# matthiasverstraete/3d_recognizer

Measured on AMD Instinct MI355X. Metric: training clouds/sec, N=40960 pts, bs=8, at 1/2/4/8 GPUs; mIoU parity, higher is better.
Workload: dtype f32 storage/accumulate, bf16x3 MFMA in the wide GEMMs

## Files before the change

3d_recognizer_amd/csrc/gemm.hip:

```cpp
#include "rl_common.h"
#include <stdlib.h>
#include <string.h>

namespace {

typedef float f32x4 __attribute__((ext_vector_type(4)));

constexpr int GM_BM = 128;
constexpr int GM_BK = 16;
constexpr int GM_AS = 20;

struct AOperand {
    const float* A;
    long lda, a_bstride;
    int a_mode;
    RlLazy lazy;
    const float* xyz;
    long xyz_bstride;
    const int32_t* nbr_idx;
    const float* nbr_d2;
    int nbr_k;
    int n;
    int K;
    long M;
// ... 150 lines not shown
                int kk, c;
                if (p.w_ns == 1) { kk = e / BN; c = e - kk * BN; }
                else             { c = e / GM_BK; kk = e - c * GM_BK; }
                float v = 0.f;
                if (k0 + kk < K && col0 + c < N) v = p.W[(long)(k0 + kk) * p.w_ks + (long)(col0 + c) * p.w_ns];
                Ws[kk * WS + c] = v;
            }
            __syncthreads();
            const int ksteps = min(4, (K - k0 + 3) >> 2);
#pragma unroll
            for (int ks = 0; ks < 4; ++ks) {
                if (ks < ksteps) {
                    const int kc = ks * 4 + lq;
                    const float a0 = As[(wave * 32 + lr) * GM_AS + kc];
                    const float a1 = As[(wave * 32 + 16 + lr) * GM_AS + kc];
#pragma unroll
                    for (int nb = 0; nb < NT; ++nb) {
                        const float bv = Ws[kc * WS + nb * 16 + lr];
                        acc[0][nb] = __builtin_amdgcn_mfma_f32_16x16x4f32(a0, bv, acc[0][nb], 0, 0, 0);
                        acc[1][nb] = __builtin_amdgcn_mfma_f32_16x16x4f32(a1, bv, acc[1][nb], 0, 0, 0);
                    }
                }
            }
        }
#pragma unroll
        for (int rb = 0; rb < 2; ++rb) {
#pragma unroll
            for (int r = 0; r < 4; ++r) {
                const long R = row0 + wave * 32 + rb * 16 + lq * 4 + r;
                if (R < M) {
                    long yoff;
                    if (p.y_contig) yoff = R * p.ldy;
                    else {
                        const int b = (int)((unsigned)R / (unsigned)p.rows_per_batch);
                        const int i = (int)(R - (long)b * p.rows_per_batch);
                        yoff = ((long)b * p.y_bstride + i) * p.ldy;
                    }
#pragma unroll
                    for (int nb = 0; nb < NT; ++nb) {
                        const int c = col0 + nb * 16 + lr;
                        if (c < N) {
                            float v = acc[rb][nb][r];
                            if (p.bias) v += p.bias[c];
                            if (p.accumulate) v += p.Y[yoff + c];
                            p.Y[yoff + c] = v;
                            const float dv = v - piv[nb];
                            ssum[nb] += dv;
                            ssq[nb] += dv * dv;
                        }
                    }
                }
            }
        }
    }
    if (p.stats) {
#pragma unroll
        for (int nb = 0; nb < NT; ++nb) {
            float s = ssum[nb], q = ssq[nb];
            s += __shfl_xor(s, 16, 64); s += __shfl_xor(s, 32, 64);
            q += __shfl_xor(q, 16, 64); q += __shfl_xor(q, 32, 64);
            if (lane < 16) {
                red[wave][0][nb * 16 + lane] = (double)s;
                red[wave][1][nb * 16 + lane] = (double)q;
            }
        }
        __syncthreads();
        if (tid < BN && col0 + tid < N) {
            const double s = red[0][0][tid] + red[1][0][tid] + red[2][0][tid] + red[3][0][tid];
            const double q = red[0][1][tid] + red[1][1][tid] + red[2][1][tid] + red[3][1][tid];
            p.stats[((long)blockIdx.x * 2 + 0) * N + col0 + tid] = s;
            p.stats[((long)blockIdx.x * 2 + 1) * N + col0 + tid] = q;
            for (long slot = blockIdx.x + gridDim.x; slot < p.stat_slots; slot += gridDim.x) {
                p.stats[(slot * 2 + 0) * N + col0 + tid] = 0.0;
                p.stats[(slot * 2 + 1) * N + col0 + tid] = 0.0;
            }
        }
    }
}

constexpr int WG_RB = 32;
constexpr int WG_T = 64;
constexpr int WG_S = 80;

struct WgradParams {
    AOperand a;
    int N;
    const float* dY;
    long lddy, dy_bstride;
    int rows_per_batch;
    int dy_contig;
    float* slab;
    long rows_per_block;
    int has_bias;
};

__global__ __launch_bounds__(256) void wgrad_kernel(const WgradParams p) {
    __shared__ __attribute__((aligned(16))) float dYs[WG_RB * WG_S];
    __shared__ __attribute__((aligned(16))) float As[WG_RB * WG_S];
    const int tid = threadIdx.x, lane = tid & 63, wave = __builtin_amdgcn_readfirstlane(tid >> 6);
    const int lr = lane & 15, lq = lane >> 4;
    const int N = p.N, K = p.a.K;
    const int n0 = blockIdx.y * WG_T, k0 = blockIdx.z * WG_T;
    const int nvalid = min(WG_T, N - n0), kvalid = min(WG_T, K - k0);
    const int nkb = (kvalid + 15) >> 4;
    const bool wave_active = wave * 16 < nvalid;
    const long r_begin = (long)blockIdx.x * p.rows_per_block;
    const long r_end = min(p.a.M, r_begin + p.rows_per_block);

    f32x4 acc[4];
#pragma unroll
    for (int kb = 0; kb < 4; ++kb) acc[kb] = (f32x4){0.f, 0.f, 0.f, 0.f};
    float bsum = 0.f;

    for (long r0 = r_begin; r0 < r_end; r0 += WG_RB) {
        __syncthreads();
        for (int e = tid; e < WG_RB * WG_T; e += 256) {
            const int r = e >> 6, c = e & 63;
            const long R = r0 + r;
            float v = 0.f;
            if (R < r_end && c < nvalid) {
                long off;
                if (p.dy_contig) off = R * p.lddy;
                else {
                    const int b = (int)((unsigned)R / (unsigned)p.rows_per_batch);
                    const int i = (int)(R - (long)b * p.rows_per_batch);
                    off = ((long)b * p.dy_bstride + i) * p.lddy;
                }
                v = p.dY[off + n0 + c];
            }
            dYs[r * WG_S + c] = v;
        }
        stage_a(p.a, r0, WG_RB, r_end, k0, nkb * 16, As, WG_S);
        __syncthreads();
        if (p.has_bias && blockIdx.z == 0 && tid < WG_T) {
#pragma unroll 8
            for (int r = 0; r < WG_RB; ++r) bsum += dYs[r * WG_S + tid];
        }
        if (wave_active) {
#pragma unroll
            for (int rs = 0; rs < WG_RB / 4; ++rs) {
                const int rr = rs * 4 + lq;
                const float av = dYs[rr * WG_S + wave * 16 + lr];
#pragma unroll
                for (int kb = 0; kb < 4; ++kb) {
                    if (kb < nkb) {
                        const float bv = As[rr * WG_S + kb * 16 + lr];
                        acc[kb] = __builtin_amdgcn_mfma_f32_16x16x4f32(av, bv, acc[kb], 0, 0, 0);
                    }
                }
            }
        }
    }
    float* out = p.slab + (long)blockIdx.x * ((long)N * K + N);
    if (wave_active) {
#pragma unroll
        for (int kb = 0; kb < 4; ++kb) {
            if (kb < nkb) {
                const int k = k0 + kb * 16 + lr;
#pragma unroll
                for (int r = 0; r < 4; ++r) {
                    const int n = n0 + wave * 16 + lq * 4 + r;
                    if (n < N && k < K) out[(long)n * K + k] = acc[kb][r];
                }
            }
        }
    }
    if (p.has_bias && blockIdx.z == 0 && tid < nvalid) out[(long)N * K + n0 + tid] = bsum;
}
// ... 1829 lines not shown
                v.w = actf(v.w * sc[i].w + sh[i].w);
            }
            float* dd = dYt + ucol[i] * PW2_S + urow[i];
            dd[0] = rd[i].x; dd[PW2_S] = rd[i].y; dd[2 * PW2_S] = rd[i].z; dd[3 * PW2_S] = rd[i].w;
            float* da = At + ucol[i] * PW2_S + urow[i];
            da[0] = v.x; da[PW2_S] = v.y; da[2 * PW2_S] = v.z; da[3 * PW2_S] = v.w;
        }
    };

    const float* n_frag = dYt + (wave * 32 + lr) * PW2_S + lq * 8;
    const float* k_frag = At + lr * PW2_S + lq * 8;
    if (r_begin < r_end) fetch(r_begin);
    for (long r0 = r_begin; r0 < r_end; r0 += PW2_RB) {
        __syncthreads();
        commit(r0);
        __syncthreads();
        if (r0 + PW2_RB < r_end) fetch(r0 + PW2_RB);
        if (p.has_bias && blockIdx.z == 0 && tid < PW2_T) {
#pragma unroll
            for (int j = 0; j < PW2_RB / 4; ++j) {
                const float4 t = *reinterpret_cast<const float4*>(dYt + tid * PW2_S + j * 4);
                bsum += (t.x + t.y) + (t.z + t.w);
            }
        }
        float4 af[2][2], bf[2][2];
#pragma unroll
        for (int h = 0; h < 2; ++h) {
            af[h][0] = *reinterpret_cast<const float4*>(n_frag + h * 4);
            af[h][1] = *reinterpret_cast<const float4*>(n_frag + 16 * PW2_S + h * 4);
        }
#pragma unroll
        for (int j = 0; j < 2; ++j) bf[0][j] = *reinterpret_cast<const float4*>(k_frag + j * 16 * PW2_S);
#pragma unroll
        for (int g = 0; g < 8; ++g) {
            const int h = g / 4, kb0 = (g % 4) * 2;
            if (g + 1 < 8) {
                const int h1 = (g + 1) / 4, kb1 = ((g + 1) % 4) * 2;
#pragma unroll
                for (int j = 0; j < 2; ++j)
                    bf[(g + 1) & 1][j] = *reinterpret_cast<const float4*>(k_frag + (kb1 + j) * 16 * PW2_S + h1 * 4);
            }
            __builtin_amdgcn_sched_barrier(0);
            const float a0[4] = {af[h][0].x, af[h][0].y, af[h][0].z, af[h][0].w};
            const float a1[4] = {af[h][1].x, af[h][1].y, af[h][1].z, af[h][1].w};
#pragma unroll
            for (int s2 = 0; s2 < 4; ++s2) {
#pragma unroll
                for (int j = 0; j < 2; ++j) {
                    const float4 b4 = bf[g & 1][j];
                    const float bv = s2 == 0 ? b4.x : s2 == 1 ? b4.y : s2 == 2 ? b4.z : b4.w;
                    acc[0][kb0 + j] = __builtin_amdgcn_mfma_f32_16x16x4f32(a0[s2], bv, acc[0][kb0 + j], 0, 0, 0);
                    acc[1][kb0 + j] = __builtin_amdgcn_mfma_f32_16x16x4f32(a1[s2], bv, acc[1][kb0 + j], 0, 0, 0);
                }
            }
        }
    }
    float* out = p.slab + (long)blockIdx.x * ((long)N * K + N);
#pragma unroll
    for (int i = 0; i < 2; ++i) {
#pragma unroll
        for (int kb = 0; kb < 8; ++kb) {
            const int k = k0 + kb * 16 + lr;
#pragma unroll
            for (int r = 0; r < 4; ++r) {
                const int n = n0 + (2 * wave + i) * 16 + lq * 4 + r;
                if (n < N && k < K) out[(long)n * K + k] = acc[i][kb][r];
            }
        }
    }
    if (p.has_bias && blockIdx.z == 0 && tid < nvalid) out[(long)N * K + n0 + tid] = bsum;
}

typedef __attribute__((ext_vector_type(4))) short s16x4g;
template <int TERMS, bool RB = false>
__device__ __forceinline__ void pwgrad128w_body(const WgradParams& p, const int bx, const int by, const int bz) {
    constexpr int RP = 144;
    constexpr int NSPL = TERMS == 3 ? 2 : 1;
    __shared__ __attribute__((aligned(16))) __bf16 lds_d[PW2_RB * RP * NSPL];
    __shared__ __attribute__((aligned(16))) __bf16 lds_a[PW2_RB * RP * NSPL];
    __bf16* Dh = lds_d;
    __bf16* Dl = Dh + PW2_RB * RP;
    __bf16* Xh = lds_a;
    __bf16* Xl = Xh + PW2_RB * RP;
    __shared__ __attribute__((aligned(16))) float lz[2][PW2_T];
    const int tid = threadIdx.x, lane = tid & 63, wave = tid >> 6;
    const int lr = lane & 15, lq = lane >> 4;
    const int N = p.N, K = p.a.K;
    const int n0 = by * PW2_T, k0 = bz * PW2_T;
    const int nvalid = min(PW2_T, N - n0), kvalid = min(PW2_T, K - k0);
    const long r_begin = (long)bx * p.rows_per_block;
    const long r_end = min(p.a.M, r_begin + p.rows_per_block);
    const bool lazy = p.a.lazy.scale != nullptr;
    const bool relu = p.a.lazy.act == RL_ACT_RELU;
    const float nslope = p.a.lazy.act == RL_ACT_NONE ? 1.f : p.a.lazy.slope;
    auto actf = [&](float z) {
        const float neg = relu ? 0.f : z * nslope;
        return z > 0.f ? z : neg;
    };
    int ucol[2], urow[2];
#pragma unroll
    for (int i = 0; i < 2; ++i) {
        const int u = i * 8 + wave;
        ucol[i] = (u & 7) * 16 + (lane & 3) * 4;
        urow[i] = (u >> 3) * 16 + (lane >> 2);
    }
    if (tid < PW2_T) {
        const bool in = lazy && tid < kvalid;
        lz[0][tid] = in ? p.a.lazy.scale[k0 + tid] : 1.f;
        lz[1][tid] = in ? p.a.lazy.shift[k0 + tid] : 0.f;
    }
    const int nh = wave >> 2, kw = wave & 3;
    f32x4 acc[4][2];
#pragma unroll
    for (int nb = 0; nb < 4; ++nb)
#pragma unroll
        for (int kb = 0; kb < 2; ++kb) acc[nb][kb] = (f32x4){0.f, 0.f, 0.f, 0.f};
    const bool want_bias = p.has_bias && bz == 0;
    f32x4 bs = {0.f, 0.f, 0.f, 0.f};
    float4 rd[2], ra[2];

    auto fetch = [&](long r0) {
#pragma unroll
        for (int i = 0; i < 2; ++i) {
            const long R = r0 + urow[i];
            rd[i] = make_float4(0.f, 0.f, 0.f, 0.f);
            ra[i] = make_float4(0.f, 0.f, 0.f, 0.f);
            if (R < r_end) {
                if (ucol[i] < nvalid) {
                    long off;
                    if (p.dy_contig) off = R * p.lddy;
                    else {
                        const int b = (int)((unsigned)R / (unsigned)p.rows_per_batch);
                        const int ii = (int)(R - (long)b * p.rows_per_batch);
                        off = ((long)b * p.dy_bstride + ii) * p.lddy;
                    }
                    rd[i] = rl_ldx4<RB>(p.dY, off + n0 + ucol[i]);
                }
                if (ucol[i] < kvalid) ra[i] = rl_ldx4<RB>(p.a.A, a_row_offset(p.a, R) + k0 + ucol[i]);
            }
        }
    };
    auto commit = [&](long r0) {
#pragma unroll
        for (int i = 0; i < 2; ++i) {
            float4 v = ra[i];
            if (lazy && r0 + urow[i] < r_end && ucol[i] < kvalid) {
                const float4 sc = *reinterpret_cast<const float4*>(&lz[0][ucol[i]]);
                const float4 sh = *reinterpret_cast<const float4*>(&lz[1][ucol[i]]);
                v.x = actf(v.x * sc.x + sh.x);
                v.y = actf(v.y * sc.y + sh.y);
                v.z = actf(v.z * sc.z + sh.z);
                v.w = actf(v.w * sc.w + sh.w);
            }
            bf16x4 dh, dl, xh, xl;
            if (want_bias) bs += (f32x4){rd[i].x, rd[i].y, rd[i].z, rd[i].w};
            split_bf16(rd[i], dh, dl);
            split_bf16(v, xh, xl);
            const int o = urow[i] * RP + ucol[i];
            *reinterpret_cast<bf16x4*>(Dh + o) = dh;
            *reinterpret_cast<bf16x4*>(Xh + o) = xh;
            if constexpr (TERMS == 3) {
                *reinterpret_cast<bf16x4*>(Dl + o) = dl;
                *reinterpret_cast<bf16x4*>(Xl + o) = xl;
            }
        }
    };

    const int tr_off = (lq * 8 + (lr >> 2)) * RP + 4 * (lr & 3);
    const __bf16* dh_frag = Dh + tr_off + nh * 64;
    const __bf16* xh_frag = Xh + tr_off + kw * 32;
    constexpr int LO = PW2_RB * RP;
    auto frag = [&](const __bf16* q) {
        const bf16x4 r0 = __builtin_bit_cast(bf16x4, __builtin_amdgcn_ds_read_tr16_b64_v4i16((__attribute__((address_space(3))) s16x4g*)q));
        const bf16x4 r1 = __builtin_bit_cast(bf16x4, __builtin_amdgcn_ds_read_tr16_b64_v4i16((__attribute__((address_space(3))) s16x4g*)(q + 4 * RP)));
        return __builtin_shufflevector(r0, r1, 0, 1, 2, 3, 4, 5, 6, 7);
    };
    if (r_begin < r_end) fetch(r_begin);
    for (long r0 = r_begin; r0 < r_end; r0 += PW2_RB) {
        __syncthreads();
        commit(r0);
        __syncthreads();
        if (r0 + PW2_RB < r_end) fetch(r0 + PW2_RB);
        bf16x8 b_h[2], b_l[2];
#pragma unroll
        for (int kb = 0; kb < 2; ++kb) {
            b_h[kb] = frag(xh_frag + kb * 16);
            if constexpr (TERMS == 3) b_l[kb] = frag(xh_frag + LO + kb * 16);
        }
#pragma unroll
        for (int nb = 0; nb < 4; ++nb) {
            bf16x8 a_h, a_l;
            a_h = frag(dh_frag + nb * 16);
            if constexpr (TERMS == 3) a_l = frag(dh_frag + LO + nb * 16);
#pragma unroll
            for (int kb = 0; kb < 2; ++kb)
                acc[nb][kb] = __builtin_amdgcn_mfma_f32_16x16x32_bf16(a_h, b_h[kb], acc[nb][kb], 0, 0, 0);
            if constexpr (TERMS == 3) {
#pragma unroll
                for (int kb = 0; kb < 2; ++kb)
                    acc[nb][kb] = __builtin_amdgcn_mfma_f32_16x16x32_bf16(a_h, b_l[kb], acc[nb][kb], 0, 0, 0);
#pragma unroll
                for (int kb = 0; kb < 2; ++kb)
                    acc[nb][kb] = __builtin_amdgcn_mfma_f32_16x16x32_bf16(a_l, b_h[kb], acc[nb][kb], 0, 0, 0);
            }
        }
    }
    float* out = p.slab + (long)bx * ((long)N * K + N);
#pragma unroll
    for (int nb = 0; nb < 4; ++nb) {
#pragma unroll
        for (int kb = 0; kb < 2; ++kb) {
            const int k = k0 + kw * 32 + kb * 16 + lr;
#pragma unroll
            for (int r = 0; r < 4; ++r) {
                const int n = n0 + nh * 64 + nb * 16 + lq * 4 + r;
                if (n < N && k < K) out[(long)n * K + k] = acc[nb][kb][r];
            }
        }
    }
    if (want_bias) {
#pragma unroll
        for (int o = 4; o < 64; o <<= 1)
#pragma unroll
            for (int j = 0; j < 4; ++j) bs[j] += __shfl_xor(bs[j], o, 64);
        if (lane < 4 && ucol[0] < nvalid) {
#pragma unroll
            for (int j = 0; j < 4; ++j) out[(long)N * K + n0 + ucol[0] + j] = bs[j];
        }
    }
}

template <int TERMS, bool RB = false>
__global__ __launch_bounds__(512, 4) void pwgrad128w_kernel(const WgradParams p) {
    pwgrad128w_body<TERMS, RB>(p, blockIdx.x, blockIdx.y, blockIdx.z);
}

struct WBItem {
    const float* A; const float* dY; const float* sc; const float* sh; float* slab;
    long lda, a_bstride, lddy, dy_bstride, rows_per_block, M;
    int N, K, n, rows_per_batch, act;
    float slope;
    int first_block;
    int nsplit;
    unsigned short gy, gz;
    unsigned char a_contig, dy_contig, has_bias, pad;
};
constexpr int WB_MAX = 24;
struct WgradBatch {
    WBItem item[WB_MAX];
    int count, pad;
};
template <int TERMS>
__global__ __launch_bounds__(512, 4) void pwgrad128w_batch_kernel(const WgradBatch b) {
    int i = 0;
    while (i + 1 < b.count && (int)blockIdx.x >= b.item[i + 1].first_block) ++i;
    const WBItem& it = b.item[i];
    const int local = (int)blockIdx.x - it.first_block;
    const int per = (int)it.gy * (int)it.gz;
    int bx, t = 0;
    if (per > 1) {
        const int grp = local / (8 * per), rem = local - grp * 8 * per;
        t = rem >> 3;
        bx = grp * 8 + (rem & 7);
    } else bx = local;
    if (bx >= it.nsplit) return;
    const int by = t / (int)it.gz, bz = t - by * (int)it.gz;
    WgradParams p;
    p.a.A = it.A; p.a.lda = it.lda; p.a.a_bstride = it.a_bstride; p.a.a_mode = 0;
    p.a.lazy.scale = it.sc; p.a.lazy.shift = it.sh; p.a.lazy.act = it.act; p.a.lazy.slope = it.slope;
    p.a.xyz = nullptr; p.a.xyz_bstride = 0; p.a.nbr_idx = nullptr; p.a.nbr_d2 = nullptr; p.a.nbr_k = 0;
    p.a.n = it.n; p.a.K = it.K; p.a.M = it.M; p.a.contig = it.a_contig; p.a.vec4 = 1; p.a.vec4p = 1;
    p.N = it.N; p.dY = it.dY; p.lddy = it.lddy; p.dy_bstride = it.dy_bstride; p.rows_per_batch = it.rows_per_batch;
    p.dy_contig = it.dy_contig; p.slab = it.slab; p.rows_per_block = it.rows_per_block; p.has_bias = it.has_bias;
    pwgrad128w_body<TERMS, false>(p, bx, by, bz);
}

__global__ __launch_bounds__(256) void swgrad_batch_kernel(const WgradBatch b) {
    __shared__ float red[4 * 4 * 4 * 64 + 8 * 64];
    int i = 0;
    while (i + 1 < b.count && (int)blockIdx.x >= b.item[i + 1].first_block) ++i;
    const WBItem& it = b.item[i];
    WgradParams p;
    p.a.A = it.A; p.a.lda = it.lda; p.a.a_bstride = it.a_bstride; p.a.a_mode = 0;
    p.a.lazy.scale = it.sc; p.a.lazy.shift = it.sh; p.a.lazy.act = it.act; p.a.lazy.slope = it.slope;
    p.a.xyz = nullptr; p.a.xyz_bstride = 0; p.a.nbr_idx = nullptr; p.a.nbr_d2 = nullptr; p.a.nbr_k = 0;
    p.a.n = it.n; p.a.K = it.K; p.a.M = it.M; p.a.contig = it.a_contig; p.a.vec4 = 0; p.a.vec4p = 0;
    p.N = it.N; p.dY = it.dY; p.lddy = it.lddy; p.dy_bstride = it.dy_bstride; p.rows_per_batch = it.rows_per_batch;
    p.dy_contig = it.dy_contig; p.slab = it.slab; p.rows_per_block = it.rows_per_block; p.has_bias = it.has_bias;
    const int bx = (int)blockIdx.x - it.first_block;
    if (bx >= it.nsplit) return;
    switch (it.gy) {
        case swgrad_body_index(1, 1): swgrad_body<1, 1>(p, bx, red); break;
        case swgrad_body_index(1, 2): swgrad_body<1, 2>(p, bx, red); break;
        case swgrad_body_index(1, 4): swgrad_body<1, 4>(p, bx, red); break;
        case swgrad_body_index(1, 8): swgrad_body<1, 8>(p, bx, red); break;
        case swgrad_body_index(2, 1): swgrad_body<2, 1>(p, bx, red); break;
        case swgrad_body_index(2, 2): swgrad_body<2, 2>(p, bx, red); break;
        case swgrad_body_index(2, 4): swgrad_body<2, 4>(p, bx, red); break;
        case swgrad_body_index(4, 1): swgrad_body<4, 1>(p, bx, red); break;
        case swgrad_body_index(4, 2): swgrad_body<4, 2>(p, bx, red); break;
        default: swgrad_body<4, 4>(p, bx, red); break;
    }
}

inline bool pwgrad_ok(const WgradParams& p) {
    if (p.a.a_mode != 0 || !p.a.vec4) return false;
    if ((p.N % 4) || (p.lddy % 4) || (((uintptr_t)p.dY) & 15)) return false;
    if (p.a.lazy.scale && ((((uintptr_t)p.a.lazy.scale) | ((uintptr_t)p.a.lazy.shift)) & 15)) return false;
    return true;
}


typedef void (*GemmFn)(const GemmParams);
typedef void (*WgradFn)(const WgradParams);
enum GemmKernel { GK_NONE, GK_SGEMM, GK_PGEMM, GK_WGEMM, GK_WGEMM2, GK_GEMM };

struct GemmFacts {
    long M; int N, K;
    bool streamable;
    bool pgemm, wgemm, wgemm2;
    bool split, stats, bnb;
    int64_t kslab_floats;
};

struct GemmPlan {
    GemmKernel kernel;
    GemmFn fn;
    int threads; dim3 grid;
    WidePlan wide;
    int gx, ny, ksplit, kchunk;
    GemmFn reduce;
    dim3 reduce_grid;
    const char* name;
    const char* refusal;
};

template <int KC, bool BNB>
GemmFn sgemm_fn(int N) {
    if constexpr (KC == 1 && !BNB) if (N > 64) return sgemm_kernel<1, 8>;
    return N <= 16 ? sgemm_kernel<KC, 1, BNB> : N <= 32 ? sgemm_kernel<KC, 2, BNB> : sgemm_kernel<KC, 4, BNB>;
}
template <int NT>
GemmFn pgemm_fn(int terms) { return terms == 0 ? pgemm_kernel<NT, 0> : terms == 1 ? pgemm_kernel<NT, 1> : pgemm_kernel<NT, 3>; }
template <int TERMS, bool STATS>
GemmFn wide_inst(bool dma, WidePlan w) {
    if (!dma) return wgemm_kernel<TERMS, STATS>;
    return w.bm == 128 ? wgemm2_kernel<TERMS, STATS, W2_AS, W2_WS, 128, 128>
         : w.bn == 128 ? wgemm2_kernel<TERMS, STATS, W2_AS, W2_WS, 64, 128> : wgemm2_kernel<TERMS, STATS, W2_AS, W2_WS, 64, 64>;
}
inline GemmFn wide_fn(bool stats, bool dma, WidePlan w) {
    if (wide_gemm_terms() == 1) return stats ? wide_inst<1, true>(dma, w) : wide_inst<1, false>(dma, w);
    return stats ? wide_inst<3, true>(dma, w) : wide_inst<3, false>(dma, w);
}

inline dim3 xcd_grid(int gx, int ny, int z) { return dim3(ny > 1 ? (unsigned)(8 * rl_cdiv(gx, 8) * ny) : (unsigned)gx, 1, z); }

inline void persistent_grid(GemmPlan& pl, long M, int ny, int z) {
    int cap = cu_count() / ny / 8 * 8;
    if (cap < 8) cap = 8;
    pl.gx = rl_cdiv(M, pl.wide.bm);
    if (pl.gx > cap) pl.gx = cap;
    pl.ny = ny;
    pl.grid = xcd_grid(pl.gx, ny, z);
}

inline void plan_wide(GemmPlan& pl, const GemmFacts& f, int z, bool splitk) {
    const bool dma = f.wgemm2;
    pl.fn = wide_fn(f.stats && pl.ksplit <= 1, dma, pl.wide);
    pl.kernel = dma ? GK_WGEMM2 : GK_WGEMM;
    pl.threads = dma ? W2_THREADS : 512;
    if (dma) persistent_grid(pl, f.M, rl_cdiv(f.N, pl.wide.bn), z);
// ... 12 lines not shown
    const bool streams = !f.split && f.streamable && stream_ok(N, K);
    if (!f.split && f.bnb && !(streams && N <= 64)) {
        pl.refusal = "rl_gemm: the BatchNorm-backward sums are a by-product of the streaming kernel only (K, N <= 64; ask rl_gemm_streams)";
        return pl;
    }
    if (streams) {
        int sg = pl.gx;
        if ((long)K * N >= 2048) sg = sg > 512 ? 512 : (sg > 256 ? 256 : sg);
        if (g_sgemm_grid_div > 1) sg = sg / g_sgemm_grid_div > 0 ? sg / g_sgemm_grid_div : 1;
        if (f.bnb) pl.fn = K <= 16 ? sgemm_fn<1, true>(N) : K <= 32 ? sgemm_fn<2, true>(N) : sgemm_fn<4, true>(N);
        else       pl.fn = K <= 16 ? sgemm_fn<1, false>(N) : K <= 32 ? sgemm_fn<2, false>(N) : sgemm_fn<4, false>(N);
        pl.kernel = GK_SGEMM;
        pl.grid = dim3(sg);
        pl.name = "sgemm_kernel";
        return pl;
    }
    if (f.pgemm) pl.wide = wide_plan(f.M, N, K, N > 64 && f.wgemm && f.wgemm2);
    const int terms = wide_gemm_terms();
    if (!f.split && f.pgemm && N > 64 && pl.wide.ksplit > 1 && f.kslab_floats >= (int64_t)pl.wide.ksplit * f.M * N) {
        pl.kchunk = ((K + pl.wide.ksplit - 1) / pl.wide.ksplit + 31) / 32 * 32;
        pl.ksplit = (K + pl.kchunk - 1) / pl.kchunk;
        const bool cb64 = (long)pl.gx * rl_cdiv(N, 64) >= 256;
        pl.reduce = cb64 ? gemm_splitk_reduce_kernel<64> : gemm_splitk_reduce_kernel<16>;
        pl.reduce_grid = dim3(pl.gx, rl_cdiv(N, cb64 ? 64 : 16));
        if (f.wgemm) {
            plan_wide(pl, f, pl.ksplit, true);
        } else {
            pl.kernel = GK_PGEMM;
            pl.fn = pgemm_fn<8>(terms);
            pl.grid = xcd_grid(pl.gx, pl.ny, pl.ksplit);
            pl.name = "pgemm_kernel<8>+splitk";
        }
    } else if (!f.split && f.pgemm && N > 16 && N <= 64 && wgemm_small_tiles() && f.wgemm && f.wgemm2) {
        pl.wide = WidePlan{64, 64, 1};
        plan_wide(pl, f, 1, false);
    } else if (!f.pgemm) {
        pl.kernel = GK_GEMM;
        pl.fn = nt == 1 ? gemm_kernel<1> : nt == 2 ? gemm_kernel<2> : nt == 4 ? gemm_kernel<4> : gemm_kernel<8>;
        pl.grid = dim3(pl.gx, pl.ny);
        pl.name = "gemm_kernel";
    } else if (N > 64 && f.wgemm) {
        plan_wide(pl, f, 1, false);
    } else {
        pl.kernel = GK_PGEMM;
        pl.fn = nt == 1 ? pgemm_fn<1>(terms) : nt == 2 ? pgemm_fn<2>(terms) : nt == 4 ? pgemm_fn<4>(terms) : pgemm_fn<8>(terms);
        pl.grid = xcd_grid(pl.gx, pl.ny, 1);
        pl.name = N > 64 ? "pgemm_kernel<8>" : f.split ? "pgemm_kernel" : nt == 1 ? "pgemm_kernel<1>" : nt == 2 ? "pgemm_kernel<2>" : "pgemm_kernel<4>";
    }
    return pl;
}

inline GemmFacts aligned_facts(long M, int N, int K, bool dma) {
    return GemmFacts{M, N, K, true, true, wide_gemm_terms() != 0 && K % 8 == 0,
                     dma && wgemm_staging() == 1 && K % PG_BK == 0 && K <= W2_KMAX, false, true, false, 0};
}

int launch_gemm(const GemmPlan& pl, hipStream_t st, GemmParams p, const char* who) {
    p.gx = pl.gx; p.ny = pl.ny; p.ksplit = pl.ksplit; p.kchunk = pl.kchunk;
    hipLaunchKernelGGL(pl.fn, pl.grid, dim3(pl.threads), 0, st, p);
    rl_note_kernel(pl.name);
    RL_LAUNCH_CHECK(who);
    if (!pl.reduce) return RL_OK;
    hipLaunchKernelGGL(pl.reduce, pl.reduce_grid, dim3(256), 0, st, p);
    RL_LAUNCH_CHECK("rl_gemm(split-K reduce)");
    return RL_OK;
}

struct WgradPlan {
    WgradFn fn;
    int threads; dim3 grid;
    int nsplit; long rows_per_block;
    int batch;
    int body;
    const char* name;
    const char* refusal;
};

template <int KT>
WgradFn swgrad_fn(int N) {
    if constexpr (KT == 1) if (N > 64) return swgrad_kernel<1, 8>;
    return N <= 16 ? swgrad_kernel<KT, 1> : N <= 32 ? swgrad_kernel<KT, 2> : swgrad_kernel<KT, 4>;
}

WgradPlan plan_wgrad(long M, int N, int K, int a_mode, bool pwgrad, bool rows_bf16) {
    WgradPlan pl{};
    pl.threads = 256;
    const int terms = wide_gemm_terms();
    if (stream_ok(N, K)) {
        swgrad_split(M, &pl.nsplit, &pl.rows_per_block);
        if (!rows_bf16) pl.fn = K <= 16 ? swgrad_fn<1>(N) : K <= 32 ? swgrad_fn<2>(N) : swgrad_fn<4>(N);
        pl.refusal = "rl_wgrad: bf16 rows are supported by the wide weight-gradient kernel only";
        pl.grid = dim3(pl.nsplit);
        pl.batch = a_mode == 0 && !rows_bf16 ? 2 : 0;
        pl.body = swgrad_body_index(K <= 16 ? 1 : K <= 32 ? 2 : 4, N <= 16 ? 1 : N <= 32 ? 2 : N <= 64 ? 4 : 8);
        pl.name = "swgrad_kernel";
        return pl;
    }
    wgrad_split(M, N, K, &pl.nsplit, &pl.rows_per_block);
    const int T = pwgrad ? wgrad_tile(N, K) : WG_T;
    const bool wide = pwgrad && T == 128;
    pl.grid = dim3(pl.nsplit, rl_cdiv(N, T), rl_cdiv(K, T));
    if (rows_bf16)  pl.fn = wide && terms != 0 ? pwgrad128w_kernel<1, true> : nullptr;
    else if (wide)  pl.fn = terms == 0 ? pwgrad128_kernel : terms == 1 ? pwgrad128w_kernel<1> : pwgrad128w_kernel<3>;
    else            pl.fn = pwgrad ? pwgrad_kernel : wgrad_kernel;
    pl.threads = wide && terms != 0 ? 512 : 256;
    pl.refusal = "rl_wgrad: bf16 rows are supported by the wide (128 x 128 tile) weight-gradient kernel only";
    pl.batch = !rows_bf16 && wide && terms != 0 && rl_cdiv(N, 128) < 65536 && rl_cdiv(K, 128) < 65536 ? 1 : 0;
    pl.name = wide ? (terms != 0 ? "pwgrad128w_kernel" : "pwgrad128_kernel") : pwgrad ? "pwgrad_kernel" : "wgrad_kernel";
    return pl;
}

void launch_wgrad_batch(int batch, long blocks, hipStream_t st, const WgradBatch& b) {
    if (batch == 2)                   hipLaunchKernelGGL(swgrad_batch_kernel, dim3((unsigned)blocks), dim3(256), 0, st, b);
    else if (wide_gemm_terms() == 1)  hipLaunchKernelGGL(pwgrad128w_batch_kernel<1>, dim3((unsigned)blocks), dim3(512), 0, st, b);
    else                              hipLaunchKernelGGL(pwgrad128w_batch_kernel<3>, dim3((unsigned)blocks), dim3(512), 0, st, b);
}

}

int rl_wide_terms() { return wide_gemm_terms(); }

extern "C" int rl_set_wide_gemm(const char* mode) {
    const int t = parse_wide(mode);
    RL_REQUIRE(mode != nullptr && t >= 0, RL_ERR_ARGS, "rl_set_wide_gemm: mode must be \"fp32\", \"bf16x3\" or \"bf16\"");
    g_wide_terms = t;
    return RL_OK;
}
extern "C" int rl_set_wgemm_staging(const char* how) {
    RL_REQUIRE(how != nullptr && (!strcmp(how, "registers") || !strcmp(how, "dma")), RL_ERR_ARGS,
               "rl_set_wgemm_staging: \"registers\" or \"dma\"");
    g_wgemm_staging = !strcmp(how, "dma");
    return RL_OK;
}
extern "C" int rl_set_wgemm_tile(const char* how) {
    RL_REQUIRE(how && (!strcmp(how, "auto") || !strcmp(how, "128") || !strcmp(how, "64x128") || !strcmp(how, "64x64")), RL_ERR_ARGS,
               "rl_set_wgemm_tile: expected auto | 128 | 64x128 | 64x64");
    g_wgemm_force = !strcmp(how, "64x128") ? 1 : !strcmp(how, "64x64") ? 2 : 0;
    g_wgemm_small = strcmp(how, "128") ? 1 : 0;
    return RL_OK;
}
extern "C" int rl_set_gemm_ksplit(int enable) {
    g_gemm_no_ksplit = enable ? 0 : 1;
    return RL_OK;
}
extern "C" int rl_set_sgemm_grid_div(int div) {
    RL_REQUIRE(div >= 1 && div <= 64, RL_ERR_ARGS, "rl_set_sgemm_grid_div: 1 .. 64");
    g_sgemm_grid_div = div;
    return RL_OK;
}
extern "C" const char* rl_get_wide_gemm(void) {
    const int t = wide_gemm_terms();
    return t == 0 ? "fp32" : t == 1 ? "bf16" : "bf16x3";
}

extern "C" int rl_gemm(const rl_gemm_desc* d, void* stream) {
    RL_REQUIRE(d != nullptr, RL_ERR_ARGS, "rl_gemm: null descriptor");
    GemmParams p{};
    int rc = fill_a(&p.a, "rl_gemm", d->A, d->lda, d->a_bstride, d->a_mode, d->in_act, d->in_slope,
                    d->in_scale, d->in_shift, d->xyz, d->xyz_bstride, d->nbr_idx, d->nbr_d2, d->nbr_k,
                    d->B, d->n, d->K);
    if (rc) return rc;
    RL_REQUIRE(d->N > 0 && d->W && d->Y && d->ldy > 0, RL_ERR_ARGS, "rl_gemm: bad W/Y");
    p.N = d->N; p.W = d->W; p.w_ks = d->w_ks; p.w_ns = d->w_ns; p.bias = d->bias;
    p.Y = d->Y; p.ldy = d->ldy; p.y_bstride = d->y_bstride;
    p.rows_per_batch = (d->a_mode == 1) ? d->n * d->nbr_k : d->n;
    RL_REQUIRE(d->y_bstride >= p.rows_per_batch, RL_ERR_ARGS, "rl_gemm: y_bstride smaller than rows per cloud");
    p.y_contig = (d->y_bstride == p.rows_per_batch);
// ... 39 lines not shown
static bool gemm_pair_fits(const rl_gemm_desc* a, const rl_gemm_desc* b) {
    if (!a || !b) return false;
    if (a->A != b->A || a->lda != b->lda || a->a_bstride != b->a_bstride || a->a_mode != 0 || b->a_mode != 0) return false;
    if (a->B != b->B || a->n != b->n || a->K != b->K) return false;
    if (a->in_scale != b->in_scale || a->in_shift != b->in_shift || a->in_act != b->in_act || a->in_slope != b->in_slope) return false;
    if (!a->W_split || !b->W_split || wide_gemm_terms() == 0 || wgemm_staging() != 1) return false;
    if (a->K % PG_BK || a->K > W2_KMAX || a->N <= 0 || b->N <= 0) return false;
    if ((a->K <= 64 && a->N <= 64) || (b->K <= 64 && b->N <= 64)) return false;
    if (a->bias || b->bias || a->accumulate || b->accumulate || a->addend || b->addend || a->out2 || b->out2) return false;
    if ((a->stats == nullptr) != (b->stats == nullptr)) return false;
    if (a->ldy != a->N || b->ldy != b->N || a->y_bstride != a->n || b->y_bstride != b->n || !a->Y || !b->Y) return false;
    if ((((uintptr_t)a->A | (uintptr_t)(a->lda * 4) | (uintptr_t)a->W_split | (uintptr_t)b->W_split | (uintptr_t)a->Y | (uintptr_t)b->Y) & 15) != 0)
        return false;
    if (a->N % 4 || b->N % 4) return false;
    return true;
}
extern "C" int rl_gemm_pair_supported(const rl_gemm_desc* a, const rl_gemm_desc* b) { return gemm_pair_fits(a, b) ? 1 : 0; }
extern "C" int rl_gemm_pair(const rl_gemm_desc* a, const rl_gemm_desc* b, void* stream) {
    RL_REQUIRE(gemm_pair_fits(a, b), RL_ERR_UNSUPPORTED,
               "rl_gemm_pair: needs one plain A' (K %% 32 == 0, K <= 1024) for both, pre-split weights in a bf16 arithmetic mode, the "
               "dense outputs, statistics for both or none, no bias / accumulate / split epilogue");
    GemmParams p{};
    int rc = fill_a(&p.a, "rl_gemm_pair", a->A, a->lda, a->a_bstride, 0, a->in_act, a->in_slope, a->in_scale, a->in_shift,
                    nullptr, 0, nullptr, nullptr, 0, a->B, a->n, a->K);
    if (rc) return rc;
    p.N = a->N; p.W = a->W; p.w_ks = a->w_ks; p.w_ns = a->w_ns; p.bias = nullptr;
    p.Y = a->Y; p.ldy = a->ldy; p.y_bstride = a->y_bstride; p.rows_per_batch = a->n; p.y_contig = 1;
    p.accumulate = 0; p.stats = a->stats;
    p.piv_mean = a->stats ? a->stats_pivot_mean : nullptr; p.piv_bias = a->stats ? a->stats_pivot_bias : nullptr;
    p.split_col = a->N; p.wsplit = reinterpret_cast<const __bf16*>(a->W_split);
    p.stat_slots = rl_row_blocks_host(p.a.M, GM_BM);
    p.N2 = b->N; p.Y2 = b->Y; p.stats2 = b->stats; p.wsplit2 = reinterpret_cast<const __bf16*>(b->W_split);
    p.piv_mean2 = b->stats ? b->stats_pivot_mean : nullptr; p.piv_bias2 = b->stats ? b->stats_pivot_bias : nullptr;
    p.pair_ny1 = rl_cdiv(a->N, 128);
    RL_REQUIRE(wgemm2_usable(p), RL_ERR_UNSUPPORTED, "rl_gemm_pair: the LDS-DMA kernel does not take this operand");
    GemmPlan pl{};
    pl.kernel = GK_WGEMM2; pl.wide = WidePlan{128, 128, 1}; pl.threads = W2_THREADS; pl.ksplit = 1; pl.name = "wgemm2_kernel";
    pl.fn = wide_fn(p.stats != nullptr, true, pl.wide);
    persistent_grid(pl, p.a.M, p.pair_ny1 + rl_cdiv(b->N, 128), 1);
    return launch_gemm(pl, (hipStream_t)stream, p, "rl_gemm_pair");
}

extern "C" int rl_split_weights(const rl_wsplit_item* items, int count, void* stream) {
    RL_REQUIRE(items != nullptr && count >= 0, RL_ERR_ARGS, "rl_split_weights: bad arguments");
    hipStream_t st = (hipStream_t)stream;
    for (int base = 0; base < count; base += WS_MAX) {
        SplitBatch b;
        b.count = count - base < WS_MAX ? count - base : WS_MAX;
        long blocks = 0;
        for (int i = 0; i < b.count; ++i) {
            const rl_wsplit_item& it = items[base + i];
            RL_REQUIRE(it.W && it.out && it.K > 0 && it.N > 0, RL_ERR_ARGS, "rl_split_weights: bad item %d", base + i);
            RL_REQUIRE(((uintptr_t)it.out & 15) == 0, RL_ERR_ARGS, "rl_split_weights: item %d: out must be 16-byte aligned", base + i);
            RL_REQUIRE(it.K % 8 == 0 && (long)it.N * it.K < (1l << 31), RL_ERR_ARGS, "rl_split_weights: item %d: K %% 8 == 0, N * K < 2^31", base + i);
            b.item[i] = it;
            b.first_block[i] = (int)blocks;
            blocks += rl_cdiv((long)it.N * (it.K / 8), 256);
        }
        b.first_block[b.count] = (int)blocks;
        if (blocks > 0) hipLaunchKernelGGL(split_weights_kernel, dim3((unsigned)blocks), dim3(256), 0, st, b);
        RL_LAUNCH_CHECK("rl_split_weights");
    }
    rl_note_kernel("split_weights_kernel");
    return RL_OK;
}

extern "C" int64_t rl_gemm_stat_slots(int64_t M, int N, int K) {
    const GemmPlan pl = plan_gemm(aligned_facts(M, N, K, true));
    return rl_row_blocks_host(M, pl.kernel == GK_WGEMM2 ? pl.wide.bm : GM_BM);
}

extern "C" int64_t rl_gemm_kslab_floats(int64_t M, int N, int K) {
    const int ks = plan_gemm(aligned_facts(M, N, K, false)).wide.ksplit;
    return ks > 1 ? (int64_t)ks * M * N : 0;
}

extern "C" int64_t rl_wgrad_slab_floats(int64_t M, int N, int K) {
    return (int64_t)plan_wgrad(M, N, K, 0, true, false).nsplit * ((int64_t)N * K + N);
}

static int wgrad_fill(const rl_wgrad_desc* d, WgradParams* pp, WgradPlan* plan) {
    RL_REQUIRE(d != nullptr, RL_ERR_ARGS, "rl_wgrad: null descriptor");
    WgradParams& p = *pp;
    int rc = fill_a(&p.a, "rl_wgrad", d->A, d->lda, d->a_bstride, d->a_mode, d->in_act, d->in_slope,
                    d->in_scale, d->in_shift, d->xyz, d->xyz_bstride, d->nbr_idx, d->nbr_d2, d->nbr_k,
                    d->B, d->n, d->K);
    if (rc) return rc;
    RL_REQUIRE(d->N > 0 && d->dY && d->dW && d->slab && d->lddy >= d->N, RL_ERR_ARGS, "rl_wgrad: bad dY/dW/slab");
    p.N = d->N; p.dY = d->dY; p.lddy = d->lddy; p.dy_bstride = d->dy_bstride;
    p.rows_per_batch = (d->a_mode == 1) ? d->n * d->nbr_k : d->n;
    RL_REQUIRE(d->dy_bstride >= p.rows_per_batch, RL_ERR_ARGS, "rl_wgrad: dy_bstride smaller than rows per cloud");
    p.dy_contig = (d->dy_bstride == p.rows_per_batch);
    p.slab = d->slab; p.has_bias = d->dbias != nullptr;
    const WgradPlan pl = plan_wgrad(p.a.M, d->N, d->K, d->a_mode, pwgrad_ok(p), d->rows_bf16 != 0);
    RL_REQUIRE(pl.fn != nullptr, RL_ERR_UNSUPPORTED, "%s", pl.refusal);
    RL_REQUIRE(d->slab_floats >= (int64_t)pl.nsplit * ((int64_t)d->N * d->K + d->N), RL_ERR_ARGS,
               "rl_wgrad: slab too small (%ld floats)", (long)d->slab_floats);
    RL_REQUIRE(!d->rows_bf16 || (d->lda % 4 == 0 && d->lddy % 4 == 0), RL_ERR_ARGS,
               "rl_wgrad: bf16 rows need leading dimensions that are multiples of 4");
    p.rows_per_block = pl.rows_per_block;
    *plan = pl;
    return RL_OK;
}

extern "C" int rl_wgrad_batchable(const rl_wgrad_desc* d) {
    WgradParams p;
    WgradPlan pl;
    return wgrad_fill(d, &p, &pl) == RL_OK ? pl.batch : 0;
}

extern "C" int rl_wgrad_batch(const rl_wgrad_desc* descs, int count, void* stream) {
    RL_REQUIRE(descs != nullptr && count >= 0, RL_ERR_ARGS, "rl_wgrad_batch: bad arguments");
    hipStream_t st = (hipStream_t)stream;
    bool any[3] = {false, false, false};
    for (int kind = 1; kind <= 2; ++kind) {
        WgradBatch b;
        b.count = 0; b.pad = 0;
        long blocks = 0;
        auto flush = [&]() -> int {
            if (b.count == 0 || blocks == 0) { b.count = 0; blocks = 0; return RL_OK; }
            launch_wgrad_batch(kind, blocks, st, b);
            RL_LAUNCH_CHECK("rl_wgrad_batch");
            b.count = 0; blocks = 0;
            return RL_OK;
        };
        for (int i = 0; i < count; ++i) {
            const rl_wgrad_desc* d = descs + i;
            WgradParams p;
            WgradPlan pl;
            int rc = wgrad_fill(d, &p, &pl);
            if (rc) return rc;
            RL_REQUIRE(pl.batch != 0, RL_ERR_UNSUPPORTED,
                       "rl_wgrad_batch: layer %d (N = %d, K = %d) cannot join a grouped launch - check rl_wgrad_batchable first", i, d->N, d->K);
            RL_REQUIRE(d->defer_reduce, RL_ERR_ARGS, "rl_wgrad_batch: the layers' slabs are summed by rl_wgrad_reduce_batch (defer_reduce must be set)");
            if (pl.batch != kind) continue;
            any[kind] = true;
            WBItem& it = b.item[b.count];
            it.A = p.a.A; it.dY = p.dY; it.sc = p.a.lazy.scale; it.sh = p.a.lazy.shift; it.slab = p.slab;
            it.lda = p.a.lda; it.a_bstride = p.a.a_bstride; it.lddy = p.lddy; it.dy_bstride = p.dy_bstride;
            it.rows_per_block = p.rows_per_block; it.M = p.a.M;
            it.N = p.N; it.K = p.a.K; it.n = p.a.n; it.rows_per_batch = p.rows_per_batch; it.act = p.a.lazy.act; it.slope = p.a.lazy.slope;
            it.nsplit = pl.nsplit;
            if (kind == 2) {
                it.gy = (unsigned short)pl.body; it.gz = 1;
                it.first_block = (int)blocks;
                blocks += pl.nsplit;
            } else {
                it.gy = (unsigned short)pl.grid.y; it.gz = (unsigned short)pl.grid.z;
                const int per = (int)it.gy * (int)it.gz;
                if (per > 1) blocks = (blocks + 7) / 8 * 8;
                it.first_block = (int)blocks;
                blocks += per > 1 ? (long)((pl.nsplit + 7) / 8 * 8) * per : (long)pl.nsplit;
            }
            it.a_contig = (unsigned char)p.a.contig; it.dy_contig = (unsigned char)p.dy_contig; it.has_bias = (unsigned char)p.has_bias; it.pad = 0;
            RL_REQUIRE(blocks < (1l << 30), RL_ERR_ARGS, "rl_wgrad_batch: too many workgroups");
            if (++b.count == WB_MAX) {
                rc = flush();
                if (rc) return rc;
            }
        }
        const int rc = flush();
        if (rc) return rc;
    }
    rl_note_kernel(any[2] && !any[1] ? "swgrad_batch_kernel" : "pwgrad128w_batch_kernel");
    return RL_OK;
}

extern "C" int rl_wgrad(const rl_wgrad_desc* d, void* stream) {
    WgradParams p;
    WgradPlan pl;
    int rc = wgrad_fill(d, &p, &pl);
    if (rc) return rc;
    hipStream_t st = (hipStream_t)stream;
    hipLaunchKernelGGL(pl.fn, pl.grid, dim3(pl.threads), 0, st, p);
    rl_note_kernel(pl.name);
    RL_LAUNCH_CHECK("rl_wgrad");
    if (d->defer_reduce) return RL_OK;
    const long per = (long)d->N * d->K + d->N;
    hipLaunchKernelGGL(wgrad_reduce_kernel, dim3(rl_cdiv(per, WR_E)), dim3(256), 0, st, d->slab, pl.nsplit,
                       d->N, d->K, d->dW, (long)d->w_ks, (long)d->w_ns, d->dbias);
    RL_LAUNCH_CHECK("rl_wgrad_reduce");
    return RL_OK;
}

extern "C" int rl_wgrad_nsplit(int64_t M, int N, int K) { return plan_wgrad(M, N, K, 0, true, false).nsplit; }

extern "C" int rl_wgrad_reduce_batch(const rl_wgrad_reduce_item* items, int count, void* stream) {
    RL_REQUIRE(items != nullptr && count >= 0, RL_ERR_ARGS, "rl_wgrad_reduce_batch: bad arguments");
    hipStream_t st = (hipStream_t)stream;
    for (int base = 0; base < count; base += RB_MAX) {
        ReduceBatch b;
        b.count = count - base < RB_MAX ? count - base : RB_MAX;
        long tiles = 0;
        for (int i = 0; i < b.count; ++i) {
            const rl_wgrad_reduce_item& it = items[base + i];
            RL_REQUIRE(it.slab && it.dW && it.nsplit > 0 && it.N > 0 && it.K > 0, RL_ERR_ARGS,
                       "rl_wgrad_reduce_batch: bad item %d", base + i);
            b.item[i] = it;
            b.first_tile[i] = (int)tiles;
            tiles += rl_cdiv((long)it.N * it.K + it.N, WR_E);
            RL_REQUIRE(tiles < (1l << 30), RL_ERR_ARGS, "rl_wgrad_reduce_batch: too many tiles");
        }
        b.first_tile[b.count] = (int)tiles;
        hipLaunchKernelGGL(wgrad_reduce_batch_kernel, dim3((unsigned)tiles), dim3(256), 0, st, b);
        RL_LAUNCH_CHECK("rl_wgrad_reduce_batch");
    }
    rl_note_kernel("wgrad_reduce_batch_kernel");
    return RL_OK;
}
```

3d_recognizer_amd/csrc/pool.hip:

```cpp
#include "rl_common.h"
#include <stdlib.h>

namespace {

#ifdef RL_POOL_PLAIN_STORES
#define RL_ST1 rl_stx
#define RL_ST4 rl_stx4
#else
#define RL_ST1 rl_stx_nt
#define RL_ST4 rl_stx4_nt
#endif

typedef float f32x4 __attribute__((ext_vector_type(4)));
typedef __attribute__((ext_vector_type(4))) __bf16 bf16x4;
typedef __attribute__((ext_vector_type(8))) __bf16 bf16x8;
typedef __attribute__((ext_vector_type(4))) short s16x4;

typedef float f32x2 __attribute__((ext_vector_type(2)));
typedef __attribute__((ext_vector_type(2))) __bf16 bf16x2;
__device__ __forceinline__ void split2(const f32x2 x, unsigned& hi, unsigned& lo) {
    const unsigned hb = __builtin_bit_cast(unsigned, __builtin_convertvector(x, bf16x2));
    const f32x2 hf = {__uint_as_float(hb << 16), __uint_as_float(hb & 0xffff0000u)};
    const f32x2 l = x - hf;
    lo = __builtin_bit_cast(unsigned, __builtin_convertvector(l, bf16x2));
    hi = hb;
}
__device__ __forceinline__ void split4(const float4 v, bf16x4& hi, bf16x4& lo) {
    unsigned h0, h1, l0, l1;
    split2((f32x2){v.x, v.y}, h0, l0);
    split2((f32x2){v.z, v.w}, h1, l1);
    typedef unsigned u2 __attribute__((ext_vector_type(2)));
    hi = __builtin_bit_cast(bf16x4, (u2){h0, h1});
    lo = __builtin_bit_cast(bf16x4, (u2){l0, l1});
}
__device__ __forceinline__ bf16x8 cat8(const bf16x4 a, const bf16x4 b) {
    bf16x8 r;
#pragma unroll
    for (int i = 0; i < 4; ++i) { r[i] = a[i]; r[4 + i] = b[i]; }
    return r;
}
__device__ __forceinline__ f32x4 mfma16(const bf16x4 a, const bf16x4 b, const f32x4 c) {
    return __builtin_amdgcn_mfma_f32_16x16x16bf16_1k(__builtin_bit_cast(s16x4, a), __builtin_bit_cast(s16x4, b), c, 0, 0, 0);
}

__device__ __forceinline__ void loads_issued() { __builtin_amdgcn_sched_barrier(0); }
__device__ __forceinline__ void loads_landed() {
    asm volatile("" ::: "memory");
    __builtin_amdgcn_s_waitcnt(0x0F70);
    asm volatile("" ::: "memory");
}
__device__ __forceinline__ f32x4 splat(float v) { return (f32x4){v, v, v, v}; }
__device__ __forceinline__ f32x4 v4(const float4 a) { return (f32x4){a.x, a.y, a.z, a.w}; }
__device__ __forceinline__ float4 f4(const f32x4 a) { return make_float4(a[0], a[1], a[2], a[3]); }
__device__ __forceinline__ float sum4(const f32x4 a) { return (a[0] + a[1]) + (a[2] + a[3]); }
__device__ __forceinline__ f32x4 vbn(const f32x4 raw, float s, float h) { return __builtin_elementwise_fma(raw, splat(s), splat(h)); }
__device__ __forceinline__ f32x4 vrelu(const f32x4 z) { return __builtin_elementwise_max(z, splat(0.f)); }
__device__ __forceinline__ float eff_slope(const RlLazy& t) {
    if (t.scale == nullptr || t.act == RL_ACT_NONE) return 1.f;
    return t.act == RL_ACT_RELU ? 0.f : t.slope;
}
__device__ __forceinline__ f32x4 vact(const f32x4 z, float e) { return __builtin_elementwise_max(z, z * splat(e)); }

struct PoolParams {
    const float* U;
    RlLazy ulazy;
    const float* G;
    long g_bstride;
    RlLazy glazy;
    const int32_t* idx;
    const float* W;
    long P;
    int n;
    int d;
    float* Pout;
    const float* dP;
    float* GU;
    int gu_accumulate;
    float* DG;
    float* slab;
    long slab_stride;
    float* X_out;
    float* dS_out;
    int src;
    const float* xyz;
    long xyz_bstride;
    int xyz_w;
    const float* nbr_d2;
    const float* W1; const float* b1; const float* sc1; const float* sh1;
    const float* W2; const float* b2; const float* sc2; const float* sh2;
    const float* mu1; const float* is1; const float* mu2; const float* is2;
    const float* piv1; const float* piv2;
    double* fstats2;
    double* bstats;
    int xcd_chunk;
};

template <int DT>
struct Tile {
    static constexpr int D = 16 * DT;
    static constexpr int H = D / 2;
    static constexpr int XS = D + 4;
    static constexpr int XSB = D + 8;
};

template <int DT>
__device__ __forceinline__ void lane_lazy(const PoolParams& p, int lj, f32x4 (&sc)[DT], f32x4 (&sh)[DT]) {
    constexpr int H = Tile<DT>::H;
#pragma unroll
    for (int c = 0; c < DT; ++c)
#pragma unroll
        for (int s = 0; s < 4; ++s) {
            const int k = 16 * c + 4 * lj + s;
            if (k < H) {
                sc[c][s] = p.ulazy.scale ? p.ulazy.scale[k] : 1.f;
                sh[c][s] = p.ulazy.scale ? p.ulazy.shift[k] : 0.f;
            } else {
                sc[c][s] = p.glazy.scale ? p.glazy.scale[k - H] : 1.f;
                sh[c][s] = p.glazy.scale ? p.glazy.shift[k - H] : 0.f;
            }
        }
}
template <int DT>
__device__ __forceinline__ float chunk_slope(int c, int lj, float es_u, float es_g) {
    if constexpr (DT == 1) return lj < 2 ? es_u : es_g;
    else return 16 * c < Tile<DT>::H ? es_u : es_g;
}

template <int DT>
struct LFold {
    static constexpr int D = 16 * DT;
    static constexpr bool INLDS = DT >= 8;
    static constexpr int LDS_FLOATS = INLDS ? 2 * D : 4;
    f32x4 rsc[INLDS ? 1 : DT], rsh[INLDS ? 1 : DT];
    const float* lds;
    __device__ __forceinline__ void init(const PoolParams& p, int lj, float* mem) {
        if constexpr (INLDS) {
            constexpr int H = D / 2;
            for (int k = threadIdx.x; k < D; k += blockDim.x) {
                const RlLazy& t = k < H ? p.ulazy : p.glazy;
                mem[k] = t.scale ? t.scale[k < H ? k : k - H] : 1.f;
                mem[D + k] = t.scale ? t.shift[k < H ? k : k - H] : 0.f;
            }
            lds = mem + 4 * lj;
        } else lane_lazy<DT>(p, lj, rsc, rsh);
    }
    __device__ __forceinline__ f32x4 sc(int c) const {
        if constexpr (INLDS) return *reinterpret_cast<const f32x4*>(lds + 16 * c);
        else return rsc[c];
    }
    __device__ __forceinline__ f32x4 sh(int c) const {
        if constexpr (INLDS) return *reinterpret_cast<const f32x4*>(lds + D + 16 * c);
        else return rsh[c];
    }
};

struct Cursor {
    long pt;
    int b, i;
    __device__ __forceinline__ void start(long pt0, int n) {
        pt = pt0;
        b = (int)((unsigned)pt0 / (unsigned)n);
        i = (int)(pt0 - (long)b * n);
    }
    __device__ __forceinline__ Cursor next(long pstep, int n) const {
        Cursor c;
        c.pt = pt + pstep;
        c.b = b;
        c.i = i + (int)pstep;
        while (c.i >= n) { c.i -= n; ++c.b; }
        return c;
    }
};

struct PointSpan { int first, step, end; };
template <int NW>
__device__ __forceinline__ PointSpan point_span(const PoolParams& p, int wave) {
    PointSpan s;
    if (p.xcd_chunk > 0) {
        const int x = (int)blockIdx.x & 7, slot = (int)blockIdx.x >> 3;
        const int lo = x * p.xcd_chunk, hi = lo + p.xcd_chunk;
        s.end = hi < (int)p.P ? hi : (int)p.P;
        s.first = lo + slot * NW + wave;
        s.step = ((int)gridDim.x >> 3) * NW;
    } else {
        s.end = (int)p.P;
        s.first = (int)blockIdx.x * NW + wave;
        s.step = (int)gridDim.x * NW;
    }
    return s;
}

template <int DT>
__device__ __forceinline__ void fetch_x(const PoolParams& p, const Cursor& cu, int li, int lj, int my_idx, float4 (&raw)[DT]) {
    constexpr int H = Tile<DT>::H;
    const long row = cu.pt * 16 + li;
    const long b = cu.b;
#pragma unroll
    for (int c = 0; c < DT; ++c) {
        const int k = 16 * c + 4 * lj;
        if (k < H) {
            if (p.src == 0) raw[c] = *reinterpret_cast<const float4*>(p.U + row * H + k);
        } else raw[c] = *reinterpret_cast<const float4*>(p.G + (b * p.g_bstride + my_idx) * H + (k - H));
    }
}
template <int DT>
__device__ __forceinline__ void finish_x(const PoolParams& p, int li, int lj, const float4 (&raw)[DT],
                                         const LFold<DT>& lf, float4 (&xa)[DT], float* Xs) {
    constexpr int XS = Tile<DT>::XS;
    const float es_u = eff_slope(p.ulazy), es_g = eff_slope(p.glazy);
#pragma unroll
    for (int c = 0; c < DT; ++c) {
        const int k = 16 * c + 4 * lj;
        const float4 v = f4(vact(v4(raw[c]) * lf.sc(c) + lf.sh(c), chunk_slope<DT>(c, lj, es_u, es_g)));
        xa[c] = v;
        *reinterpret_cast<float4*>(Xs + li * XS + k) = v;
    }
}

template <int DT>
__device__ __forceinline__ void tile_gemm(const float4 (&a)[DT], const float* Bt, int li, int lj, f32x4 (&acc)[DT]) {
    constexpr int XS = Tile<DT>::XS;
    const float* base = Bt + li * XS + 4 * lj;
#pragma unroll
    for (int c = 0; c < DT; ++c) {
        float4 b[DT];
#pragma unroll
        for (int nb = 0; nb < DT; ++nb) b[nb] = *reinterpret_cast<const float4*>(base + nb * 16 * XS + 16 * c);
        const float av[4] = {a[c].x, a[c].y, a[c].z, a[c].w};
#pragma unroll
        for (int s = 0; s < 4; ++s) {
#pragma unroll
            for (int nb = 0; nb < DT; ++nb) {
                const float bv = s == 0 ? b[nb].x : s == 1 ? b[nb].y : s == 2 ? b[nb].z : b[nb].w;
                acc[nb] = __builtin_amdgcn_mfma_f32_16x16x4f32(av[s], bv, acc[nb], 0, 0, 0);
            }
        }
    }
}

template <int DT>
__device__ __forceinline__ void tile_gemm_bf(const float4 (&a)[DT], const __bf16* Bh, const __bf16* Bl, int li, int lj,
                                             f32x4 (&acc)[DT]) {
    constexpr int XSB = Tile<DT>::XSB;
    const int off = li * XSB + 4 * lj;
    if constexpr (DT == 1) {
        bf16x4 ah, al;
        split4(a[0], ah, al);
        const bf16x4 bh = *reinterpret_cast<const bf16x4*>(Bh + off);
        const bf16x4 bl = *reinterpret_cast<const bf16x4*>(Bl + off);
        acc[0] = mfma16(ah, bh, acc[0]);
        acc[0] = mfma16(ah, bl, acc[0]);
        acc[0] = mfma16(al, bh, acc[0]);
    } else {
#pragma unroll
        for (int b = 0; b < DT / 2; ++b) {
            bf16x4 h0, l0, h1, l1;
            split4(a[2 * b], h0, l0);
            split4(a[2 * b + 1], h1, l1);
            const bf16x8 ah = cat8(h0, h1), al = cat8(l0, l1);
            constexpr int NG = DT < 4 ? DT : 4;
#pragma unroll
            for (int n0 = 0; n0 < DT; n0 += NG) {
                bf16x8 bh[NG], bl[NG];
#pragma unroll
                for (int j = 0; j < NG; ++j) {
                    const int o = off + (n0 + j) * 16 * XSB + 32 * b;
                    bh[j] = cat8(*reinterpret_cast<const bf16x4*>(Bh + o), *reinterpret_cast<const bf16x4*>(Bh + o + 16));
                    bl[j] = cat8(*reinterpret_cast<const bf16x4*>(Bl + o), *reinterpret_cast<const bf16x4*>(Bl + o + 16));
                }
#pragma unroll
                for (int j = 0; j < NG; ++j) acc[n0 + j] = __builtin_amdgcn_mfma_f32_16x16x32_bf16(ah, bh[j], acc[n0 + j], 0, 0, 0);
#pragma unroll
                for (int j = 0; j < NG; ++j) acc[n0 + j] = __builtin_amdgcn_mfma_f32_16x16x32_bf16(ah, bl[j], acc[n0 + j], 0, 0, 0);
#pragma unroll
                for (int j = 0; j < NG; ++j) acc[n0 + j] = __builtin_amdgcn_mfma_f32_16x16x32_bf16(al, bh[j], acc[n0 + j], 0, 0, 0);
            }
        }
    }
}


typedef unsigned u32x2 __attribute__((ext_vector_type(2)));
__device__ __forceinline__ float vsqrt(float x) { return __builtin_amdgcn_sqrtf(x); }

__device__ __forceinline__ float lg_sum(float v) {
    u32x2 r = __builtin_amdgcn_permlane16_swap(__float_as_uint(v), __float_as_uint(v), false, false);
    v = __uint_as_float(r[0]) + __uint_as_float(r[1]);
    r = __builtin_amdgcn_permlane32_swap(__float_as_uint(v), __float_as_uint(v), false, false);
    return __uint_as_float(r[0]) + __uint_as_float(r[1]);
}
__device__ __forceinline__ void lg_sum2(float& a, float& b) {
    u32x2 r = __builtin_amdgcn_permlane32_swap(__float_as_uint(a), __float_as_uint(b), false, false);
    float z = __uint_as_float(r[0]) + __uint_as_float(r[1]);
    r = __builtin_amdgcn_permlane16_swap(__float_as_uint(z), __float_as_uint(z), false, false);
    z = __uint_as_float(r[0]) + __uint_as_float(r[1]);
    r = __builtin_amdgcn_permlane32_swap(__float_as_uint(z), __float_as_uint(z), false, false);
// ... 230 lines not shown
                v.x = Xs[(4 * lj + 0) * XS + kb * 16 + li]; v.y = Xs[(4 * lj + 1) * XS + kb * 16 + li];
                v.z = Xs[(4 * lj + 2) * XS + kb * 16 + li]; v.w = Xs[(4 * lj + 3) * XS + kb * 16 + li];
                split4(v, xh[kb], xl[kb]);
            }
#pragma unroll
            for (int nb = 0; nb < DT; ++nb) {
                bf16x4 dh, dl;
                split4(f4(dsr[nb]), dh, dl);
#pragma unroll
                for (int kb = 0; kb < DT; ++kb) accw[nb][kb] = mfma16(dh, xh[kb], accw[nb][kb]);
#pragma unroll
                for (int kb = 0; kb < DT; ++kb) accw[nb][kb] = mfma16(dh, xl[kb], accw[nb][kb]);
#pragma unroll
                for (int kb = 0; kb < DT; ++kb) accw[nb][kb] = mfma16(dl, xh[kb], accw[nb][kb]);
            }
        }
        loads_landed();
#pragma unroll
        for (int r = 0; r < 4; ++r) {
            const int rowi = lj * 4 + r;
#pragma unroll
            for (int nb = 0; nb < DT; ++nb) {
                const int col = nb * 16 + li;
                float v = dx[nb][r];
                if (col < H) {
                    if (nb < NGU) v += gacc[nb][r];
                }
                if constexpr (DT <= 2) Ds[rowi * XS + col] = v;
                else {
                    const long urow = (pt * 16 + rowi) * H;
                    if (col < H) RL_ST1<GUB>(p.GU, urow + col, v);
                    else RL_ST1<GB>(p.DG, urow + (col - H), v);
                }
            }
        }
        if constexpr (DT <= 2) {
            __builtin_amdgcn_wave_barrier();
            const long orow = (pt * 16 + li) * H;
#pragma unroll
            for (int c = 0; c < DT; ++c) {
                const int k = 16 * c + 4 * lj;
                const float4 v = *reinterpret_cast<const float4*>(Ds + li * XS + k);
                if (k < H) RL_ST4<GUB>(p.GU, orow + k, v);
                else RL_ST4<GB>(p.DG, orow + (k - H), v);
            }
        }
#pragma unroll
        for (int nb = 0; nb < DT; ++nb) gp[nb] = gp_nxt[nb];
        __builtin_amdgcn_wave_barrier();
    }
    __syncthreads();
    float* red = Wmem;
    for (int w = 1; w < NW; ++w) {
        __syncthreads();
        if (wave == w) {
#pragma unroll
            for (int nb = 0; nb < DT; ++nb)
#pragma unroll
                for (int kb = 0; kb < DT; ++kb)
#pragma unroll
                    for (int r = 0; r < 4; ++r) red[((nb * DT + kb) * 4 + r) * 64 + lane] = accw[nb][kb][r];
        }
        __syncthreads();
        if (wave == 0) {
#pragma unroll
            for (int nb = 0; nb < DT; ++nb)
#pragma unroll
                for (int kb = 0; kb < DT; ++kb)
#pragma unroll
                    for (int r = 0; r < 4; ++r) accw[nb][kb][r] += red[((nb * DT + kb) * 4 + r) * 64 + lane];
        }
    }
    if (wave == 0) {
        float* out = p.slab + (long)blockIdx.x * p.slab_stride;
#pragma unroll
        for (int nb = 0; nb < DT; ++nb)
#pragma unroll
            for (int kb = 0; kb < DT; ++kb)
#pragma unroll
                for (int r = 0; r < 4; ++r) out[(long)(nb * 16 + lj * 4 + r) * D + kb * 16 + li] = accw[nb][kb][r];
    }
}

template <bool GB>
__global__ __launch_bounds__(512) void pool128_bwd_kernel(const PoolParams p) {
    __shared__ __attribute__((aligned(16))) float lfm[LFold<8>::LDS_FLOATS];
    constexpr int NW = 8;
    constexpr int TERMS = 3;
    constexpr int DT = 8, D = 128, H = 64, XS = Tile<DT>::XS, XSB = Tile<DT>::XSB;
    __shared__ __attribute__((aligned(16))) __bf16 Wh[D * XSB];
    __shared__ __attribute__((aligned(16))) __bf16 Wl[D * XSB];
    __shared__ __attribute__((aligned(16))) float Tiles[NW][16 * XS];
    const int lane = threadIdx.x & 63, wave = __builtin_amdgcn_readfirstlane(threadIdx.x >> 6);
    const int li = lane & 15, lj = lane >> 4;
    for (int e = threadIdx.x; e < D * D; e += 64 * NW) {
        const int o = e / D, i = e - o * D;
        const float w = p.W[e];
        const __bf16 h = (__bf16)w;
        Wh[o * XSB + i] = h;
        if constexpr (TERMS == 3) Wl[o * XSB + i] = (__bf16)(w - (float)h);
    }
    LFold<DT> lf;
    lf.init(p, lj, lfm);
    __syncthreads();
    float* Xs = Tiles[wave];
    float* Ds = Tiles[wave];

    const PointSpan span = point_span<NW>(p, wave);
    const long pstep = span.step, Pend = span.end;
    long pt = span.first;
    int idx_cur = pt < Pend ? p.idx[pt * 16 + li] : 0;
    int idx_nxt = pt + pstep < Pend ? p.idx[(pt + pstep) * 16 + li] : 0;
    float4 raw[DT];
    Cursor cu;
    cu.start(pt, p.n);
    float gp[DT], gp_nxt[DT];
#pragma unroll
    for (int nb = 0; nb < DT; ++nb) gp[nb] = gp_nxt[nb] = 0.f;
    if (pt < Pend) {
        fetch_x<DT>(p, cu, li, lj, idx_cur, raw);
#pragma unroll
        for (int nb = 0; nb < DT; ++nb) gp[nb] = p.dP[pt * D + nb * 16 + li];
    }
    loads_landed();
    for (; pt < Pend; pt += pstep) {
        const Cursor cn = cu.next(pstep, p.n);
        float4 xa[DT];
        finish_x<DT>(p, li, lj, raw, lf, xa, Xs);
        const int idx_n2 = pt + 2 * pstep < Pend ? p.idx[(pt + 2 * pstep) * 16 + li] : 0;
        const Cursor cf = pt + pstep < Pend ? cn : cu;
        fetch_x<DT>(p, cf, li, lj, pt + pstep < Pend ? idx_nxt : idx_cur, raw);
#pragma unroll
        for (int nb = 0; nb < DT; ++nb) gp_nxt[nb] = p.dP[cf.pt * D + nb * 16 + li];
        loads_issued();
        cu = cn;
        idx_cur = idx_nxt; idx_nxt = idx_n2;
#pragma unroll
        for (int c = 0; c < DT; ++c) rl_stx4<GB>(p.X_out, (pt * 16 + li) * D + 16 * c + 4 * lj, xa[c]);
        f32x4 a[DT];
#pragma unroll
        for (int nb = 0; nb < DT; ++nb) a[nb] = (f32x4){0.f, 0.f, 0.f, 0.f};
        tile_gemm_bf<DT>(xa, Wh, Wl, li, lj, a);
        softmax_rows<DT>(a);
        __builtin_amdgcn_wave_barrier();
        f32x4 dx[DT];
#pragma unroll
        for (int nb = 0; nb < DT; ++nb) {
            const int col = nb * 16 + li;
            f32x4 xc;
#pragma unroll
            for (int r = 0; r < 4; ++r) xc[r] = Xs[(lj * 4 + r) * XS + col];
            float pool = sum4(a[nb] * xc);
            pool = lg_sum(pool);
            dx[nb] = a[nb] * splat(gp[nb]);
            const f32x4 ds = dx[nb] * (xc - splat(pool));
#pragma unroll
            for (int r = 0; r < 4; ++r) Ds[(lj * 4 + r) * XS + col] = ds[r];
        }
        __builtin_amdgcn_wave_barrier();
#pragma unroll
        for (int c = 0; c < DT; ++c) {
            const float4 da = *reinterpret_cast<const float4*>(Ds + li * XS + 16 * c + 4 * lj);
            rl_stx4<GB>(p.dS_out, (pt * 16 + li) * D + 16 * c + 4 * lj, da);
            bf16x4 ah, al;
            split4(da, ah, al);
            const int tq = li >> 2, tp = li & 3;
            const __bf16* trh = Wh + (16 * c + 4 * lj + tq) * XSB + 4 * tp;
            const __bf16* trl = Wl + (16 * c + 4 * lj + tq) * XSB + 4 * tp;
#pragma unroll
            for (int n0 = 0; n0 < DT; n0 += 4) {
                bf16x4 bh[4], bl[4];
#pragma unroll
                for (int j4 = 0; j4 < 4; ++j4) {
                    bh[j4] = __builtin_bit_cast(bf16x4, __builtin_amdgcn_ds_read_tr16_b64_v4i16(
                        (__attribute__((address_space(3))) s16x4*)(trh + (n0 + j4) * 16)));
                    if constexpr (TERMS == 3)
                        bl[j4] = __builtin_bit_cast(bf16x4, __builtin_amdgcn_ds_read_tr16_b64_v4i16(
                            (__attribute__((address_space(3))) s16x4*)(trl + (n0 + j4) * 16)));
                }
#pragma unroll
                for (int j4 = 0; j4 < 4; ++j4) dx[n0 + j4] = mfma16(ah, bh[j4], dx[n0 + j4]);
                if constexpr (TERMS == 3) {
#pragma unroll
                    for (int j4 = 0; j4 < 4; ++j4) dx[n0 + j4] = mfma16(ah, bl[j4], dx[n0 + j4]);
#pragma unroll
                    for (int j4 = 0; j4 < 4; ++j4) dx[n0 + j4] = mfma16(al, bh[j4], dx[n0 + j4]);
                }
            }
        }
        loads_landed();
        __builtin_amdgcn_wave_barrier();
#pragma unroll
        for (int nb = 0; nb < DT; ++nb)
#pragma unroll
            for (int r = 0; r < 4; ++r) Ds[(lj * 4 + r) * XS + nb * 16 + li] = dx[nb][r];
        __builtin_amdgcn_wave_barrier();
        const long orow = (pt * 16 + li) * H;
        float4 gold[DT / 2];
        if (p.gu_accumulate) {
#pragma unroll
            for (int c = 0; c < DT / 2; ++c) gold[c] = *reinterpret_cast<const float4*>(p.GU + orow + 16 * c + 4 * lj);
        }
#pragma unroll
        for (int c = DT / 2; c < DT; ++c)
            rl_stx4<GB>(p.DG, orow + 16 * c + 4 * lj - H, *reinterpret_cast<const float4*>(Ds + li * XS + 16 * c + 4 * lj));
#pragma unroll
        for (int c = 0; c < DT / 2; ++c) {
            f32x4 v = *reinterpret_cast<const f32x4*>(Ds + li * XS + 16 * c + 4 * lj);
            if (p.gu_accumulate) v += v4(gold[c]);
            *reinterpret_cast<float4*>(p.GU + orow + 16 * c + 4 * lj) = f4(v);
        }
#pragma unroll
        for (int nb = 0; nb < DT; ++nb) gp[nb] = gp_nxt[nb];
        __builtin_amdgcn_wave_barrier();
    }
}

struct RpeBwdParams {
    PoolParams pp;
    const float* G;
    double* stats;
    const float* coef;
    float* slab;
    float* GU1;
    int g_bf16;
// ... 1354 lines not shown
        __syncthreads();
        if (wave == 0) {
#pragma unroll
            for (int nb = 0; nb < NCH; ++nb)
#pragma unroll
                for (int kb = 0; kb < KB; ++kb)
#pragma unroll
                    for (int r = 0; r < 4; ++r) accw[nb][kb][r] += red[((nb * KB + kb) * 4 + r) * 64 + lane];
        }
    }
    __syncthreads();
    float* out = q.slab + (long)blockIdx.x * ((long)H * Kin + H);
    if (wave == 0) {
#pragma unroll
        for (int nb = 0; nb < NCH; ++nb) {
            if constexpr (SRC == 1) {
#pragma unroll
                for (int r = 0; r < 4; ++r) {
                    const int n = nb * 16 + lj * 4 + r;
                    const float v = accw[nb][0][r], o = __shfl_xor(v, 1, 64);
                    const int c = li >> 1;
                    if (n < H && li < 8) {
                        if ((li & 1) == 0) {
                            if (c < 3) { out[(long)n * 10 + c] = v; out[(long)n * 10 + 3 + c] = v - o; }
                        } else {
                            out[(long)n * 10 + (c < 3 ? 6 + c : 9)] = v;
                        }
                    }
                }
            } else {
#pragma unroll
                for (int kb = 0; kb < KB; ++kb) {
                    const int k = kb * 16 + li;
#pragma unroll
                    for (int r = 0; r < 4; ++r) {
                        const int n = nb * 16 + lj * 4 + r;
                        if (n < H && k < Kin) out[(long)n * Kin + k] = accw[nb][kb][r];
                    }
                }
            }
        }
    }
    if (threadIdx.x < H) {
        const int n = threadIdx.x;
        out[(long)H * Kin + n] = ((rb[0 * HP + n] + rb[1 * HP + n]) + rb[2 * HP + n]) + rb[3 * HP + n];
    }
}

__global__ __launch_bounds__(256) void pool_dw_reduce_kernel(const float* __restrict__ slab, int nsplit, int count,
                                                             float* __restrict__ dW) {
    __shared__ float red[16][17];
    const int ex = threadIdx.x & 15, sy = threadIdx.x >> 4;
    const int e = blockIdx.x * 16 + ex;
    float s0 = 0.f, s1 = 0.f, s2 = 0.f, s3 = 0.f;
    if (e < count) {
        const float* src = slab + e;
        int i = sy;
        for (; i + 48 < nsplit; i += 64) {
            s0 += src[(long)i * count];
            s1 += src[(long)(i + 16) * count];
            s2 += src[(long)(i + 32) * count];
            s3 += src[(long)(i + 48) * count];
        }
        for (; i < nsplit; i += 16) s0 += src[(long)i * count];
    }
    red[sy][ex] = (s0 + s1) + (s2 + s3);
    __syncthreads();
    if (sy == 0 && e < count) {
        float t = 0.f;
#pragma unroll
        for (int j = 0; j < 16; ++j) t += red[j][ex];
        dW[e] = t;
    }
}

enum PoolEntry { PE_FWD, PE_BWD, PE_STATS, PE_BN_REDUCE, PE_WGRAD };

struct PoolFacts {
    PoolEntry entry;
    int d, stage;
    int terms;
    bool rows_bf16, gu_accumulate, fwd_stats2;
    long points;
};

typedef void (*PoolFn)();
struct PoolPlan {
    PoolFn fn;
    int grid, threads;
    int xcd_chunk;
    int dw_count;
    const char* name;
    const char* refusal;
};

constexpr int pool_wavefronts(bool virtual_bwd, int d) { return d == 128 || (virtual_bwd && d == 64) ? 8 : 4; }

template <template <int, int> class Pick, class... A>
PoolFn by_width(int d, int terms, A... a) {
    if (terms == 0) return d == 16 ? Pick<1, 0>::fn(a...) : d == 32 ? Pick<2, 0>::fn(a...) : Pick<4, 0>::fn(a...);
    return d == 16 ? Pick<1, 3>::fn(a...) : d == 32 ? Pick<2, 3>::fn(a...) : Pick<4, 3>::fn(a...);
}
template <int DT, int T> struct PoolFwd { static PoolFn fn() { return (PoolFn)pool_fwd_kernel<DT, T>; } };
template <int DT, int T> struct PoolBwd {
    static PoolFn fn(bool gb) {
        if constexpr (T == 3) if (gb) return (PoolFn)pool_bwd_kernel<DT, 3, false, 4, true>;
        return (PoolFn)pool_bwd_kernel<DT, T>;
    }
};
template <int DT, int T> struct VPoolFwd {
    static PoolFn fn(bool s2, bool fst) {
        return s2 ? (PoolFn)vpool_fwd_kernel<DT, T, 2, false> : fst ? (PoolFn)vpool_fwd_kernel<DT, T, 1, true> : (PoolFn)vpool_fwd_kernel<DT, T, 1, false>;
    }
};
template <int DT, int T> struct VPoolBwd {
    template <int SRC, bool GB> static PoolFn at(bool acc) {
        constexpr int NW = pool_wavefronts(true, 16 * DT);
        return acc ? (PoolFn)vpool_bwd_kernel<DT, T, SRC, NW, GB, true> : (PoolFn)vpool_bwd_kernel<DT, T, SRC, NW, GB, false>;
    }
    static PoolFn fn(bool s2, bool gb, bool acc) {
        if constexpr (T == 3) if (gb) return s2 ? at<2, true>(acc) : at<1, true>(acc);
        return s2 ? at<2, false>(acc) : at<1, false>(acc);
    }
};
template <int DT, int T> struct RpeStats { static PoolFn fn(bool s2) { return s2 ? (PoolFn)vrpe_stats_kernel<DT, T, 2> : (PoolFn)vrpe_stats_kernel<DT, T, 1>; } };
template <int DT, int T> struct RpeBwd {
    template <int SRC, bool GB> static PoolFn at(bool wgrad) { return wgrad ? (PoolFn)vrpe_wgrad_kernel<DT, T, SRC, GB> : (PoolFn)vrpe_bn_reduce_kernel<DT, T, SRC, GB>; }
    static PoolFn fn(bool s2, bool gb, bool wgrad) {
        if constexpr (T == 3) if (gb) return s2 ? at<2, true>(wgrad) : at<1, true>(wgrad);
        return s2 ? at<2, false>(wgrad) : at<1, false>(wgrad);
    }
};

PoolPlan plan_pool(const PoolFacts& f) {
    const bool rpe = f.entry >= PE_STATS, fwd = f.entry == PE_FWD, virt = f.stage > 0, s2 = f.stage == 2;
    const int d = f.d, nw = rpe ? 4 : pool_wavefronts(f.entry == PE_BWD && virt, d);
    PoolPlan pl{};
    pl.threads = 64 * nw;
    const long per = 4 * nw;
    const long cap = rpe ? RL_MAX_SLOTS : nw == 8 ? 256 : (fwd && d <= 16) ? 1280 : (fwd && d == 64) ? 768 : 1024;
    const long g = (f.points + per - 1) / per;
    pl.grid = (int)(g < 1 ? 1 : g < cap ? g : cap);
    if (((fwd && virt) || f.entry == PE_STATS) && pl.grid >= 8 && pl.grid % 8 == 0 && f.points < (1l << 30))
        pl.xcd_chunk = (int)((f.points + 7) / 8);

    if (!(d == 16 || d == 32 || d == 64 || (d == 128 && !virt && !rpe && f.terms != 0))) {
        pl.refusal = "d must be 16, 32 or 64, or 128 with a stored U outside the fp32 arithmetic mode";
        return pl;
    }
    const bool gb = f.rows_bf16 && !fwd && f.entry != PE_STATS;
    if (gb && f.terms != 3 && d != 128) { pl.refusal = "bf16 gradient rows need the bf16x3 arithmetic mode"; return pl; }
    switch (f.entry) {
    case PE_FWD:
        pl.name = virt ? "vpool_fwd_kernel" : d == 16 ? "pool_fwd_kernel<1>" : d == 32 ? "pool_fwd_kernel<2>" : d == 64 ? "pool_fwd_kernel<4>" : "pool_fwd_kernel<8>";
        pl.fn = virt ? by_width<VPoolFwd>(d, f.terms, s2, f.fwd_stats2)
              : d == 128 ? (PoolFn)pool_fwd_kernel<8, 3, pool_wavefronts(false, 128)> : by_width<PoolFwd>(d, f.terms);
        break;
    case PE_BWD:
        pl.name = virt ? "vpool_bwd_kernel" : d == 16 ? "pool_bwd_kernel<1>" : d == 32 ? "pool_bwd_kernel<2>" : d == 64 ? "pool_bwd_kernel<4>" : "pool128_bwd_kernel";
        pl.fn = virt ? by_width<VPoolBwd>(d, f.terms, s2, gb, f.gu_accumulate)
              : d == 128 ? (gb ? (PoolFn)pool128_bwd_kernel<true> : (PoolFn)pool128_bwd_kernel<false>) : by_width<PoolBwd>(d, f.terms, gb);
        pl.dw_count = d == 128 ? 0 : d * d;
        break;
    case PE_STATS:
        pl.name = "vrpe_stats_kernel";
        pl.fn = by_width<RpeStats>(d, f.terms, s2);
        break;
    case PE_BN_REDUCE:
    case PE_WGRAD:
        pl.name = f.entry == PE_WGRAD ? "vrpe_wgrad_kernel" : "vrpe_bn_reduce_kernel";
        pl.fn = by_width<RpeBwd>(d, f.terms, s2, gb, f.entry == PE_WGRAD);
        break;
    }
    return pl;
}

template <class... Args>
int launch_pool(const PoolPlan& pl, const char* who, void* stream, const float* slab, float* dW, Args... args) {
    hipStream_t st = (hipStream_t)stream;
    void (*fn)(Args...) = (void (*)(Args...))pl.fn;
    hipLaunchKernelGGL(fn, dim3(pl.grid), dim3(pl.threads), 0, st, args...);
    rl_note_kernel(pl.name);
    RL_LAUNCH_CHECK(who);
    if (dW) {
        hipLaunchKernelGGL(pool_dw_reduce_kernel, dim3(rl_cdiv(pl.dw_count, 16)), dim3(256), 0, st, slab, pl.grid, pl.dw_count, dW);
        RL_LAUNCH_CHECK(who);
    }
    return RL_OK;
}

enum BnNeed {
    BN_BELOW,
    BN_FOLDED,
    BN_FOLDED_SAVED,
    BN_ALL
};

int fill_branch(PoolParams* p, const rl_pool_desc* d, const char* who, BnNeed need) {
    RL_REQUIRE(d && d->idx && d->points > 0 && d->n > 0 && d->points % d->n == 0, RL_ERR_ARGS, "%s: bad descriptor (null, idx, points, n)", who);
    RL_REQUIRE(d->nbr_k == 16, RL_ERR_UNSUPPORTED, "%s: the fused kernels need 16 neighbours (got %d)", who, d->nbr_k);
    RL_REQUIRE((int64_t)d->points * 16 < (1l << 31), RL_ERR_ARGS, "%s: too many neighbourhood rows", who);
    const int s = d->u_source;
    RL_REQUIRE(s >= 0 && s <= 2, RL_ERR_ARGS, "%s: u_source must be 0, 1 or 2", who);
    *p = PoolParams{};
    p->idx = d->idx; p->P = d->points; p->n = d->n; p->d = d->d; p->src = s;
    p->xyz = d->xyz; p->xyz_bstride = d->xyz_bstride; p->nbr_d2 = d->nbr_d2;
    p->xyz_w = d->xyz_width == 4 ? 4 : 3;
    p->W1 = d->W1; p->b1 = d->b1; p->sc1 = d->scale1; p->sh1 = d->shift1;
    p->W2 = d->W2; p->b2 = d->b2; p->sc2 = d->scale2; p->sh2 = d->shift2;
    p->mu1 = d->mean1; p->is1 = d->invstd1; p->mu2 = d->mean2; p->is2 = d->invstd2;
    p->piv1 = d->pivot_mean1; p->piv2 = d->pivot_mean2;
    if (s == 0) return RL_OK;
    RL_REQUIRE(d->xyz && d->nbr_d2 && d->xyz_bstride >= d->n && d->W1 && d->b1, RL_ERR_ARGS, "%s: incomplete virtual rpe branch (xyz, nbr_d2, xyz_bstride, W1, b1)", who);
    RL_REQUIRE(s < 2 || (d->W2 && d->b2 && d->scale1 && d->shift1), RL_ERR_ARGS, "%s: stage 2 needs W2 / b2 and BatchNorm 1", who);
    const int64_t B = d->points / d->n, h = d->d / 2, lim = (int64_t)1 << 31;
    RL_REQUIRE(d->n < (1 << 24), RL_ERR_UNSUPPORTED, "%s: a virtual rpe branch needs fewer than 2^24 points per cloud", who);
    RL_REQUIRE((int64_t)d->points * 16 * h * 4 < lim && (int64_t)d->points * d->d * 4 < lim, RL_ERR_UNSUPPORTED,
               "%s: a virtual rpe branch needs (points*16) x d/2 row tensors below 2 GB", who);
    RL_REQUIRE(B * d->xyz_bstride * 16 < lim && (d->g_bstride == 0 || B * d->g_bstride * h * 4 < lim), RL_ERR_UNSUPPORTED,
               "%s: a virtual rpe branch needs coordinate / feature tables below 2 GB", who);
    RL_REQUIRE(d->xyz_width == 0 || d->xyz_width == 3 || d->xyz_width == 4, RL_ERR_ARGS, "%s: xyz_width must be 3 or 4", who);
    RL_REQUIRE(d->xyz_width != 4 || ((uintptr_t)d->xyz & 15) == 0, RL_ERR_ARGS, "%s: padded xyz must be 16-byte aligned", who);
    RL_REQUIRE(need == BN_BELOW || (d->scale1 && d->shift1 && (s < 2 || (d->scale2 && d->shift2))), RL_ERR_ARGS,
               "%s: the virtual rpe branch needs its folded BatchNorm(s)", who);
    RL_REQUIRE(need != BN_ALL || (d->mean1 && d->invstd1 && (s < 2 || (d->mean2 && d->invstd2))), RL_ERR_ARGS,
               "%s: the backward of a virtual stage needs the saved mean / invstd up to it", who);
    RL_REQUIRE(need != BN_FOLDED_SAVED || (s == 1 ? (d->mean1 && d->invstd1) : (d->mean2 && d->invstd2)), RL_ERR_ARGS,
               "%s: bn_bwd_stats needs the stage's saved mean / invstd", who);
    return RL_OK;
}

int fill(PoolParams* p, const rl_pool_desc* d, const char* who, bool backward) {
    int rc = fill_branch(p, d, who, backward && d && d->bn_bwd_stats ? BN_FOLDED_SAVED : BN_FOLDED);
    if (rc) return rc;
    RL_REQUIRE(d->G && d->W && (p->src > 0 || d->U) && d->g_bstride >= d->n, RL_ERR_ARGS, "%s: null G / W / U, or g_bstride < n", who);
    RL_REQUIRE((p->src > 0 || ((uintptr_t)d->U & 15) == 0) && ((uintptr_t)d->G & 15) == 0, RL_ERR_ARGS, "%s: U/G must be 16-byte aligned", who);
    RL_REQUIRE((d->u_scale == nullptr) == (d->u_shift == nullptr) && (d->g_scale == nullptr) == (d->g_shift == nullptr),
               RL_ERR_ARGS, "%s: scale/shift must come together", who);
    p->U = d->U; p->ulazy.scale = d->u_scale; p->ulazy.shift = d->u_shift; p->ulazy.act = d->u_act; p->ulazy.slope = d->u_slope;
    p->G = d->G; p->g_bstride = d->g_bstride;
    p->glazy.scale = d->g_scale; p->glazy.shift = d->g_shift; p->glazy.act = d->g_act; p->glazy.slope = d->g_slope;
    p->W = d->W;
    p->Pout = d->Pout; p->dP = d->dP; p->GU = d->GU; p->gu_accumulate = d->gu_accumulate; p->DG = d->DG; p->slab = d->slab;
    p->slab_stride = (long)d->d * d->d + (d->dW ? 0 : d->d);
    if (backward) p->piv1 = p->piv2 = nullptr;
    p->fstats2 = backward ? nullptr : d->bn_fwd_stats2;
    RL_REQUIRE(!p->fstats2 || (p->src == 1 && d->W2 && d->b2), RL_ERR_ARGS, "%s: bn_fwd_stats2 needs virtual stage 1 and W2 / b2", who);
    p->bstats = backward ? d->bn_bwd_stats : nullptr;
    RL_REQUIRE(!p->bstats || p->src > 0, RL_ERR_ARGS, "%s: bn_bwd_stats needs a virtual rpe stage", who);
    RL_REQUIRE(backward ? (d->dP && d->GU && d->DG) : d->Pout != nullptr, RL_ERR_ARGS, "%s: null output / gradient buffers", who);
    return RL_OK;
}

int plan_grid(PoolEntry entry, int64_t points, int d, int stage) { return plan_pool({entry, d, stage, rl_wide_terms(), false, false, false, points}).grid; }

}

extern "C" int rl_pool_supported(int d, int nbr_k) { return nbr_k == 16 && !plan_pool({PE_FWD, d, 0, rl_wide_terms(), false, false, false, 1}).refusal; }

extern "C" int64_t rl_pool_slab_floats(int64_t points, int d) {
    const int stored = plan_grid(PE_BWD, points, d, 0), virt = plan_grid(PE_BWD, points, d, 1);
    return (int64_t)(stored > virt ? stored : virt) * (d * d + d);
}
extern "C" int rl_pool_bwd_slots(int64_t points, int d) { return plan_grid(PE_BWD, points, d, 1); }
extern "C" int rl_pool_bwd_grid(int64_t points, int d, int virt) { return plan_grid(PE_BWD, points, d, virt != 0); }
extern "C" int rl_pool_fwd_slots(int64_t points, int d) { return plan_grid(PE_FWD, points, d, 0); }
extern "C" int rl_rpe_stats_slots(int64_t points) { return plan_grid(PE_STATS, points, 16, 1); }
extern "C" int64_t rl_rpe_wgrad_slab_floats(int64_t points, int d, int stage) {
    const int h = d / 2;
    return (int64_t)plan_grid(PE_WGRAD, points, d, stage) * ((int64_t)h * (stage == 1 ? 10 : h) + h);
}

extern "C" int rl_pool_fwd(const rl_pool_desc* d, void* stream) {
    PoolParams p;
    int rc = fill(&p, d, "rl_pool_fwd", false);
    if (rc) return rc;
    const PoolPlan pl = plan_pool({PE_FWD, p.d, p.src, rl_wide_terms(), false, false, p.fstats2 != nullptr, p.P});
    RL_REQUIRE(!pl.refusal, RL_ERR_UNSUPPORTED, "rl_pool_fwd: %s (d %d, u_source %d)", pl.refusal, p.d, p.src);
    p.xcd_chunk = pl.xcd_chunk;
    return launch_pool(pl, "rl_pool_fwd", stream, nullptr, nullptr, p);
}

extern "C" int rl_pool_bwd(const rl_pool_desc* d, void* stream) {
    PoolParams p;
    int rc = fill(&p, d, "rl_pool_bwd", true);
    if (rc) return rc;
    const PoolPlan pl = plan_pool({PE_BWD, p.d, p.src, rl_wide_terms(), d->rows_bf16 != 0, p.gu_accumulate != 0, false, p.P});
    RL_REQUIRE(!pl.refusal, RL_ERR_UNSUPPORTED, "rl_pool_bwd: %s (d %d, u_source %d)", pl.refusal, p.d, p.src);
    if (p.d == 128) {
        RL_REQUIRE(d->X_out && d->dS_out, RL_ERR_ARGS, "rl_pool_bwd: d = 128 needs X_out and dS_out");
        RL_REQUIRE((((uintptr_t)d->X_out | (uintptr_t)d->dS_out) & 15) == 0, RL_ERR_ARGS, "rl_pool_bwd: X_out / dS_out must be 16-byte aligned");
        p.X_out = d->X_out; p.dS_out = d->dS_out;
        return launch_pool(pl, "rl_pool_bwd", stream, nullptr, nullptr, p);
    }
    RL_REQUIRE(d->slab, RL_ERR_ARGS, "rl_pool_bwd: null gradient buffers");
    RL_REQUIRE(d->slab_floats >= (int64_t)pl.grid * p.slab_stride, RL_ERR_ARGS, "rl_pool_bwd: slab too small");
    return launch_pool(pl, "rl_pool_bwd", stream, p.slab, d->dW, p);
}

extern "C" int rl_rpe_stats(const rl_pool_desc* d, double* stats, void* stream) {
    PoolParams p;
    int rc = fill_branch(&p, d, "rl_rpe_stats", BN_BELOW);
    if (rc) return rc;
    RL_REQUIRE(p.src > 0 && stats, RL_ERR_ARGS, "rl_rpe_stats: needs u_source 1 or 2 and a stats buffer");
    const PoolPlan pl = plan_pool({PE_STATS, p.d, p.src, rl_wide_terms(), false, false, false, p.P});
    RL_REQUIRE(!pl.refusal, RL_ERR_UNSUPPORTED, "rl_rpe_stats: %s (d %d, u_source %d)", pl.refusal, p.d, p.src);
    p.xcd_chunk = pl.xcd_chunk;
    return launch_pool(pl, "rl_rpe_stats", stream, nullptr, nullptr, p, stats);
}

static int rpe_bwd_plan(RpeBwdParams* q, PoolPlan* pl, PoolEntry entry, const rl_pool_desc* d, const float* G, const char* who) {
    int rc = fill_branch(&q->pp, d, who, BN_ALL);
    if (rc) return rc;
    RL_REQUIRE(q->pp.src > 0 && G, RL_ERR_ARGS, "%s: needs u_source 1 or 2 and the stage's gradient G", who);
    q->pp.piv1 = q->pp.piv2 = nullptr;
    q->G = G; q->stats = nullptr; q->coef = nullptr; q->slab = nullptr; q->GU1 = nullptr;
    q->g_bf16 = d->rows_bf16 ? 1 : 0;
    *pl = plan_pool({entry, d->d, d->u_source, rl_wide_terms(), d->rows_bf16 != 0, false, false, d->points});
    RL_REQUIRE(!pl->refusal, RL_ERR_UNSUPPORTED, "%s: %s (d %d, u_source %d)", who, pl->refusal, d->d, d->u_source);
    return RL_OK;
}

extern "C" int rl_rpe_bn_reduce(const rl_pool_desc* d, const float* G, double* stats, void* stream) {
    RpeBwdParams q;
    PoolPlan pl;
    int rc = rpe_bwd_plan(&q, &pl, PE_BN_REDUCE, d, G, "rl_rpe_bn_reduce");
    if (rc) return rc;
    RL_REQUIRE(stats, RL_ERR_ARGS, "rl_rpe_bn_reduce: null stats");
    q.stats = stats;
    return launch_pool(pl, "rl_rpe_bn_reduce", stream, nullptr, nullptr, q);
}

extern "C" int rl_rpe_wgrad(const rl_pool_desc* d, const float* G, const float* coef, float* slab, int64_t slab_floats,
                            float* GU1, void* stream) {
    RpeBwdParams q;
    PoolPlan pl;
    int rc = rpe_bwd_plan(&q, &pl, PE_WGRAD, d, G, "rl_rpe_wgrad");
    if (rc) return rc;
    RL_REQUIRE(coef && slab, RL_ERR_ARGS, "rl_rpe_wgrad: null coef / slab");
    RL_REQUIRE(slab_floats >= rl_rpe_wgrad_slab_floats(d->points, d->d, d->u_source), RL_ERR_ARGS, "rl_rpe_wgrad: slab too small");
    RL_REQUIRE(d->u_source == 1 || GU1, RL_ERR_ARGS, "rl_rpe_wgrad: stage 2 needs the stage-1 gradient output");
    q.coef = coef; q.slab = slab; q.GU1 = GU1;
    return launch_pool(pl, "rl_rpe_wgrad", stream, nullptr, nullptr, q);
}
```

3d_recognizer_amd/csrc/rl_common.h:

```cpp
#pragma once
#include <hip/hip_runtime.h>
#include <stdarg.h>
#include <stdint.h>
#include <stdio.h>

#include "../../include/rl_randlanet.h"

void rl_set_error(const char* fmt, ...);
void rl_note_kernel(const char* name);

#define RL_REQUIRE(cond, code, ...)      \
    do {                                 \
        if (!(cond)) {                   \
            rl_set_error(__VA_ARGS__);   \
            return (code);               \
        }                                \
    } while (0)

#define RL_LAUNCH_CHECK(name)                                                        \
    do {                                                                             \
        hipError_t e_ = hipGetLastError();                                           \
        if (e_ != hipSuccess) {                                                      \
            rl_set_error("%s: launch failed: %s", name, hipGetErrorString(e_));      \
            return RL_ERR_LAUNCH;                                                    \
        }                                                                            \
    } while (0)

void rl_count_launch();
#undef hipLaunchKernelGGL
#define hipLaunchKernelGGL(kernelName, numBlocks, numThreads, memPerBlock, streamId, ...)                         \
    do {                                                                                                         \
        rl_count_launch();                                                                                       \
        kernelName<<<(numBlocks), (numThreads), (memPerBlock), (streamId)>>>(__VA_ARGS__);                       \
    } while (0)

int rl_wide_terms();

static inline int rl_cdiv(long a, long b) { return (int)((a + b - 1) / b); }

#include <stdlib.h>
static inline bool rl_float_atomics_allowed() {
    const char* e = getenv("RL_ALLOW_FLOAT_ATOMICS");
    return e && e[0] == '1';
}

static inline int rl_row_blocks_host(long rows, int rows_per_tile) {
    long tiles = (rows + rows_per_tile - 1) / rows_per_tile;
    if (tiles < 1) tiles = 1;
    return (int)(tiles < RL_MAX_SLOTS ? tiles : RL_MAX_SLOTS);
}

constexpr size_t al256(size_t x) { return (x + 255) & ~(size_t)255; }

struct RlCarve {
    size_t at = 0;
    size_t take(size_t bytes) {
        const size_t off = at;
        at += al256(bytes);
        return off;
    }
};

template <class T>
static inline T* rl_at(const void* ws, size_t off) { return (T*)((char*)ws + off); }

static inline int rl_ws_check(const char* who, const void* ws, int64_t ws_bytes, int64_t need) {
    RL_REQUIRE(ws_bytes >= need, RL_ERR_ARGS, "%s: workspace of %lld bytes, %lld needed", who, (long long)ws_bytes,
               (long long)need);
    RL_REQUIRE(ws, RL_ERR_ARGS, "%s: null pointer", who);
    RL_REQUIRE(((uintptr_t)ws & 255) == 0, RL_ERR_ARGS, "%s: workspace not 256-byte aligned", who);
    return RL_OK;
}

static inline int rl_bits_of(int64_t x) {
    int b = 0;
    while (x > 0) ++b, x >>= 1;
    return b < 1 ? 1 : b;
}

#define RL_ACT_NONE 0
#define RL_ACT_RELU 1
#define RL_ACT_LRELU 2

__device__ __forceinline__ float rl_act(float z, int act, float slope) {
    if (act == RL_ACT_RELU) return z > 0.f ? z : 0.f;
    if (act == RL_ACT_LRELU) return z > 0.f ? z : z * slope;
    return z;
}
__device__ __forceinline__ float rl_act_grad(float z, int act, float slope) {
    if (act == RL_ACT_RELU) return z > 0.f ? 1.f : 0.f;
    if (act == RL_ACT_LRELU) return z > 0.f ? 1.f : slope;
    return 1.f;
}

struct RlLazy {
    const float* scale;
    const float* shift;
    int act;
    float slope;
};
__device__ __forceinline__ float rl_lazy(const RlLazy& t, float raw, int c) {
    if (t.scale == nullptr) return raw;
    return rl_act(raw * t.scale[c] + t.shift[c], t.act, t.slope);
}

typedef __bf16 rl_bf16x4 __attribute__((ext_vector_type(4)));
template <bool BF>
__device__ __forceinline__ float rl_ldx(const float* p, long i) {
    if constexpr (BF) return (float)reinterpret_cast<const __bf16*>(p)[i];
    else return p[i];
}
template <bool BF>
__device__ __forceinline__ void rl_stx(float* p, long i, float v) {
    if constexpr (BF) reinterpret_cast<__bf16*>(p)[i] = (__bf16)v;
    else p[i] = v;
}
template <bool BF>
__device__ __forceinline__ float4 rl_ldx4(const float* p, long i) {
    if constexpr (BF) {
        const rl_bf16x4 h = *reinterpret_cast<const rl_bf16x4*>(reinterpret_cast<const __bf16*>(p) + i);
        return make_float4((float)h[0], (float)h[1], (float)h[2], (float)h[3]);
    } else return *reinterpret_cast<const float4*>(p + i);
}
template <bool BF>
__device__ __forceinline__ void rl_stx4(float* p, long i, const float4 v) {
    if constexpr (BF) {
        rl_bf16x4 h;
        h[0] = (__bf16)v.x; h[1] = (__bf16)v.y; h[2] = (__bf16)v.z; h[3] = (__bf16)v.w;
        *reinterpret_cast<rl_bf16x4*>(reinterpret_cast<__bf16*>(p) + i) = h;
    } else *reinterpret_cast<float4*>(p + i) = v;
}
template <bool BF>
__device__ __forceinline__ void rl_stx_nt(float* p, long i, float v) {
    if constexpr (BF) __builtin_nontemporal_store((__bf16)v, reinterpret_cast<__bf16*>(p) + i);
    else __builtin_nontemporal_store(v, p + i);
}
template <bool BF>
__device__ __forceinline__ void rl_stx4_nt(float* p, long i, const float4 v) {
    typedef float rl_f32x4 __attribute__((ext_vector_type(4)));
    if constexpr (BF) {
        rl_bf16x4 h;
        h[0] = (__bf16)v.x; h[1] = (__bf16)v.y; h[2] = (__bf16)v.z; h[3] = (__bf16)v.w;
        __builtin_nontemporal_store(h, reinterpret_cast<rl_bf16x4*>(reinterpret_cast<__bf16*>(p) + i));
    } else {
        const rl_f32x4 w = {v.x, v.y, v.z, v.w};
        __builtin_nontemporal_store(w, reinterpret_cast<rl_f32x4*>(p + i));
    }
}
__device__ __forceinline__ float4 rl_ld4(const float* p, long i, int bf) { return bf ? rl_ldx4<true>(p, i) : rl_ldx4<false>(p, i); }
__device__ __forceinline__ float rl_ld1(const float* p, long i, int bf) { return bf ? rl_ldx<true>(p, i) : rl_ldx<false>(p, i); }
__device__ __forceinline__ void rl_st4(float* p, long i, const float4 v, int bf) {
    if (bf) rl_stx4<true>(p, i, v);
    else rl_stx4<false>(p, i, v);
}
__device__ __forceinline__ void rl_st1(float* p, long i, float v, int bf) {
    if (bf) rl_stx<true>(p, i, v);
    else rl_stx<false>(p, i, v);
}

__device__ __forceinline__ double rl_wave_sum(double v) {
#pragma unroll
    for (int o = 32; o > 0; o >>= 1) v += __shfl_xor(v, o, 64);
    return v;
}
__device__ __forceinline__ float rl_wave_sum(float v) {
#pragma unroll
    for (int o = 32; o > 0; o >>= 1) v += __shfl_xor(v, o, 64);
    return v;
}
```

3d_recognizer_amd/randlanet/_hip.py:

```python
import ctypes as C
import os
from typing import Optional

import torch

_LIB: Optional[C.CDLL] = None
_LIB_PATH = os.path.join(os.path.dirname(os.path.dirname(os.path.abspath(__file__))), "csrc",
                         "librandla_hip.so")
_LIB_PATH = os.environ.get("RL_HIP_LIB", _LIB_PATH)

ABI_VERSION = 110
MAX_SLOTS = 1024
KNN_MAX_K = 64
ACT_NONE, ACT_RELU, ACT_LRELU = 0, 1, 2

ERR_ARGS, ERR_FEW_SUPPORT, ERR_LAUNCH, ERR_UNSUPPORTED = -1, -2, -3, -4


class HipKernelError(RuntimeError):
    pass


class GemmDesc(C.Structure):
    _fields_ = [
        ("A", C.c_void_p), ("lda", C.c_int64), ("a_bstride", C.c_int64),
        ("a_mode", C.c_int32), ("in_act", C.c_int32), ("in_slope", C.c_float),
        ("in_scale", C.c_void_p), ("in_shift", C.c_void_p),
        ("xyz", C.c_void_p), ("xyz_bstride", C.c_int64),
        ("nbr_idx", C.c_void_p), ("nbr_d2", C.c_void_p), ("nbr_k", C.c_int32),
        ("B", C.c_int32), ("n", C.c_int32), ("N", C.c_int32), ("K", C.c_int32),
        ("W", C.c_void_p), ("w_ks", C.c_int64), ("w_ns", C.c_int64),
        ("bias", C.c_void_p),
        ("Y", C.c_void_p), ("ldy", C.c_int64), ("y_bstride", C.c_int64),
        ("accumulate", C.c_int32),
        ("stats", C.c_void_p),
        ("kslab", C.c_void_p), ("kslab_floats", C.c_int64),
        ("addend", C.c_void_p), ("out2", C.c_void_p), ("out2_index", C.c_void_p), ("out2_bstride", C.c_int64),
        ("split_col", C.c_int32),
        ("W_split", C.c_void_p),
        ("stats_pivot_mean", C.c_void_p), ("stats_pivot_bias", C.c_void_p),
        ("bnb_Y", C.c_void_p), ("bnb_scale", C.c_void_p), ("bnb_shift", C.c_void_p), ("bnb_mean", C.c_void_p),
        ("bnb_invstd", C.c_void_p), ("bnb_act", C.c_int32), ("bnb_slope", C.c_float),
    ]


class WsplitItem(C.Structure):
    _fields_ = [("W", C.c_void_p), ("w_ks", C.c_int64), ("w_ns", C.c_int64), ("K", C.c_int32), ("N", C.c_int32),
                ("out", C.c_void_p)]


class WgradDesc(C.Structure):
    _fields_ = [
        ("A", C.c_void_p), ("lda", C.c_int64), ("a_bstride", C.c_int64),
        ("a_mode", C.c_int32), ("in_act", C.c_int32), ("in_slope", C.c_float),
        ("in_scale", C.c_void_p), ("in_shift", C.c_void_p),
        ("xyz", C.c_void_p), ("xyz_bstride", C.c_int64),
        ("nbr_idx", C.c_void_p), ("nbr_d2", C.c_void_p), ("nbr_k", C.c_int32),
        ("B", C.c_int32), ("n", C.c_int32), ("N", C.c_int32), ("K", C.c_int32),
        ("dY", C.c_void_p), ("lddy", C.c_int64), ("dy_bstride", C.c_int64),
        ("dW", C.c_void_p), ("w_ks", C.c_int64), ("w_ns", C.c_int64),
        ("dbias", C.c_void_p),
        ("slab", C.c_void_p), ("slab_floats", C.c_int64),
        ("defer_reduce", C.c_int32), ("rows_bf16", C.c_int32),
    ]


class WgradReduceItem(C.Structure):
    _fields_ = [
        ("slab", C.c_void_p), ("dW", C.c_void_p), ("dbias", C.c_void_p),
        ("w_ks", C.c_int64), ("w_ns", C.c_int64),
        ("nsplit", C.c_int32), ("N", C.c_int32), ("K", C.c_int32), ("reserved", C.c_int32),
    ]


class CloudJob(C.Structure):
    _fields_ = [
        ("xyz", C.c_void_p), ("features", C.c_void_p), ("labels", C.c_void_p), ("n_points", C.c_int64),
        ("xyz_f64", C.c_int32), ("normalization", C.c_int32), ("augment", C.c_int32), ("normal_col", C.c_int32),
        ("jitter_variance", C.c_double), ("jitter_limit", C.c_double), ("scale", C.c_double),
        ("R", C.c_double * 9), ("shift", C.c_double * 3),
    ]


class HeadDesc(C.Structure):
    _fields_ = [
        ("X", C.c_void_p), ("scale", C.c_void_p), ("shift", C.c_void_p), ("act", C.c_int32), ("slope", C.c_float),
        ("mean", C.c_void_p), ("invstd", C.c_void_p), ("W", C.c_void_p), ("bias", C.c_void_p),
        ("perm", C.c_void_p), ("labels", C.c_void_p), ("B", C.c_int32), ("N", C.c_int32), ("C", C.c_int32),
        ("loss_kind", C.c_int32), ("alpha", C.c_float), ("gamma", C.c_float), ("neglect_background", C.c_int32),
        ("drop_p", C.c_float), ("drop_key", C.c_void_p), ("drop_seed", C.c_uint64), ("drop_first_row", C.c_int64),
        ("work", C.c_void_p), ("G", C.c_void_p), ("bn_bwd_stats", C.c_void_p), ("slab", C.c_void_p),
        ("slab_floats", C.c_int64), ("grad_scale", C.c_float), ("reserved", C.c_int32), ("drop_mask", C.c_void_p), ("perm_bstride", C.c_int64),
        ("class_weight", C.c_void_p), ("masked", C.c_int32),
    ]


class BnBwdDesc(C.Structure):
    _fields_ = [
        ("G", C.c_void_p), ("Y", C.c_void_p), ("ld", C.c_int64), ("bstride", C.c_int64),
        ("B", C.c_int32), ("n", C.c_int32), ("C", C.c_int32), ("act", C.c_int32),
        ("slope", C.c_float),
        ("scale", C.c_void_p), ("shift", C.c_void_p), ("mean", C.c_void_p), ("invstd", C.c_void_p),
        ("stats", C.c_void_p), ("coef", C.c_void_p),
    ]


class KnnTask(C.Structure):
    _fields_ = [
        ("support", C.c_void_p), ("support_bstride", C.c_int64), ("query", C.c_void_p), ("query_bstride", C.c_int64),
        ("Ns", C.c_int32), ("Nq", C.c_int32), ("k", C.c_int32),
        ("idx_out", C.c_void_p), ("d2_out", C.c_void_p),
    ]


KNN_MAX_TASKS = 8


class PoolDesc(C.Structure):
    _fields_ = [
        ("U", C.c_void_p), ("u_scale", C.c_void_p), ("u_shift", C.c_void_p), ("u_act", C.c_int32),
        ("u_slope", C.c_float),
        ("G", C.c_void_p), ("g_bstride", C.c_int64), ("g_scale", C.c_void_p), ("g_shift", C.c_void_p),
        ("g_act", C.c_int32), ("g_slope", C.c_float),
        ("idx", C.c_void_p), ("W", C.c_void_p), ("points", C.c_int64),
        ("n", C.c_int32), ("d", C.c_int32), ("nbr_k", C.c_int32),
        ("Pout", C.c_void_p), ("dP", C.c_void_p), ("GU", C.c_void_p), ("gu_accumulate", C.c_int32),
        ("DG", C.c_void_p), ("dW", C.c_void_p), ("slab", C.c_void_p), ("slab_floats", C.c_int64),
        ("X_out", C.c_void_p), ("dS_out", C.c_void_p),
        ("u_source", C.c_int32), ("xyz", C.c_void_p), ("xyz_bstride", C.c_int64), ("nbr_d2", C.c_void_p),
        ("W1", C.c_void_p), ("b1", C.c_void_p), ("scale1", C.c_void_p), ("shift1", C.c_void_p),
        ("W2", C.c_void_p), ("b2", C.c_void_p), ("scale2", C.c_void_p), ("shift2", C.c_void_p),
        ("mean1", C.c_void_p), ("invstd1", C.c_void_p), ("mean2", C.c_void_p), ("invstd2", C.c_void_p),
        ("xyz_width", C.c_int32), ("bn_bwd_stats", C.c_void_p), ("bn_fwd_stats2", C.c_void_p),
        ("rows_bf16", C.c_int32),
        ("pivot_mean1", C.c_void_p), ("pivot_mean2", C.c_void_p),
    ]


class ResidBnBwdDesc(C.Structure):
    _fields_ = [
        ("G", C.c_void_p), ("G2", C.c_void_p), ("O", C.c_void_p), ("slope", C.c_float), ("rows", C.c_int64), ("C", C.c_int32),
        ("Y1", C.c_void_p), ("scale1", C.c_void_p), ("mean1", C.c_void_p), ("invstd1", C.c_void_p),
        ("Y2", C.c_void_p), ("scale2", C.c_void_p), ("mean2", C.c_void_p), ("invstd2", C.c_void_p),
        ("stats1", C.c_void_p), ("stats2", C.c_void_p), ("coef1", C.c_void_p), ("coef2", C.c_void_p),
    ]


class CsrTask(C.Structure):
    _fields_ = [
        ("idx", C.c_void_p), ("n_src", C.c_int32), ("k", C.c_int32), ("n_dst", C.c_int32),
        ("offsets", C.c_void_p), ("entries", C.c_void_p),
    ]


CSR_MAX_TASKS = 8


class BnFinalizeItem(C.Structure):
    _fields_ = [
        ("stats", C.c_void_p), ("count", C.c_int64), ("gamma", C.c_void_p), ("beta", C.c_void_p),
        ("running_mean", C.c_void_p), ("running_var", C.c_void_p), ("num_batches_tracked", C.c_void_p),
        ("scale", C.c_void_p), ("shift", C.c_void_p), ("save_mean", C.c_void_p), ("save_invstd", C.c_void_p),
        ("folded_bias", C.c_void_p), ("nslots", C.c_int32), ("C", C.c_int32), ("training", C.c_int32),
        ("momentum", C.c_float), ("eps", C.c_float), ("pivoted", C.c_int32), ("pivot", C.c_void_p),
    ]


class BnBwdFinalizeItem(C.Structure):
    _fields_ = [
        ("stats", C.c_void_p), ("count", C.c_int64), ("dgamma", C.c_void_p), ("dbeta", C.c_void_p), ("coef", C.c_void_p),
        ("nslots", C.c_int32), ("C", C.c_int32),
    ]


class SegsumDesc(C.Structure):
    _fields_ = [
        ("src", C.c_void_p), ("lds", C.c_int64), ("src_bstride", C.c_int64),
        ("dst", C.c_void_p), ("ldd", C.c_int64), ("dst_bstride", C.c_int64),
        ("offsets", C.c_void_p), ("entries", C.c_void_p), ("entries_per_cloud", C.c_int64),
        ("B", C.c_int32), ("n_dst", C.c_int32), ("C", C.c_int32), ("accumulate", C.c_int32),
        ("src_bf16", C.c_int32),
    ]


class RowsDesc(C.Structure):
    _fields_ = [
        ("src", C.c_void_p), ("lds", C.c_int64), ("src_bstride", C.c_int64),
        ("dst", C.c_void_p), ("ldd", C.c_int64),
        ("rows", C.c_int64), ("rows_per_batch", C.c_int64),
        ("C", C.c_int32),
        ("index32", C.c_void_p), ("index64", C.c_void_p),
        ("index_shared", C.c_int32), ("accumulate", C.c_int32), ("act", C.c_int32),
        ("slope", C.c_float),
        ("scale", C.c_void_p), ("shift", C.c_void_p),
    ]


_vp, _i, _l, _f = C.c_void_p, C.c_int, C.c_int64, C.c_float
_SIGNATURES = {
    "rl_last_error": (C.c_char_p, []),
    "rl_last_kernel": (C.c_char_p, []),
    "rl_version": (_i, []),
    "rl_spin_us": (_i, [_i, _vp]),
    "rl_launch_count": (_l, []),
    "rl_row_blocks": (_i, [_l, _i]),
    "rl_knn_workspace_bytes": (_l, [_i, _i, _i, _i]),
    "rl_knn_f32": (_i, [_vp, _vp, _i, _i, _i, _i, _vp, _vp, _vp, _l, _vp]),
    "rl_knn_f32_cpu": (_i, [_vp, _vp, _i, _i, _i, _i, _vp, _vp]),
    "rl_knn_i32": (_i, [_vp, _l, _vp, _l, _i, _i, _i, _i, _vp, _vp, _vp, _l, _vp]),
    "rl_knn_multi_workspace_bytes": (_l, [C.POINTER(KnnTask), _i, _i]),
    "rl_knn_multi": (_i, [C.POINTER(KnnTask), _i, _i, _vp, _l, _vp]),
    "rl_gemm_streams": (_i, [C.POINTER(GemmDesc)]),
    "rl_gemm_pair_supported": (_i, [C.POINTER(GemmDesc), C.POINTER(GemmDesc)]),
    "rl_gemm_pair": (_i, [C.POINTER(GemmDesc), C.POINTER(GemmDesc), _vp]),
    "rl_gemm_kslab_floats": (_l, [_l, _i, _i]),
    "rl_gemm_stat_slots": (_l, [_l, _i, _i]),
    "rl_gemm": (_i, [C.POINTER(GemmDesc), _vp]),
    "rl_split_weights": (_i, [C.POINTER(WsplitItem), _i, _vp]),
    "rl_wgrad_slab_floats": (_l, [_l, _i, _i]),
    "rl_set_wide_gemm": (_i, [C.c_char_p]),
    "rl_get_wide_gemm": (C.c_char_p, []),
    "rl_set_wgemm_staging": (_i, [C.c_char_p]),
    "rl_set_wgemm_tile": (_i, [C.c_char_p]),
    "rl_set_gemm_ksplit": (_i, [_i]),
    "rl_set_sgemm_grid_div": (_i, [_i]),
    "rl_wgrad": (_i, [C.POINTER(WgradDesc), _vp]),
    "rl_wgrad_nsplit": (_i, [_l, _i, _i]),
    "rl_wgrad_batchable": (_i, [C.POINTER(WgradDesc)]),
    "rl_wgrad_batch": (_i, [C.POINTER(WgradDesc), _i, _vp]),
    "rl_wgrad_reduce_batch": (_i, [C.POINTER(WgradReduceItem), _i, _vp]),
    "rl_bn_finalize": (_i, [_vp, _i, _l, _i, _vp, _vp, _vp, _vp, _vp, _f, _f, _i, _vp, _vp, _vp, _vp, _vp, _i, _vp, _vp]),
    "rl_bn_finalize_batch": (_i, [C.POINTER(BnFinalizeItem), _i, _vp]),
    "rl_bn_bwd_finalize_batch": (_i, [C.POINTER(BnBwdFinalizeItem), _i, _vp]),
    "rl_head_supported": (_i, [_i, _i]),
    "rl_head_grid": (_i, [_l]),
    "rl_head_fwd": (_i, [C.POINTER(HeadDesc), _vp, _vp]),
    "rl_head_bwd": (_i, [C.POINTER(HeadDesc), _vp]),
    "rl_bn_bwd_finalize_pair": (_i, [_vp, _vp, _i, _l, _i, _vp, _vp, _vp, _vp, _vp, _vp, _vp]),
    "rl_bn_reduce_slots": (_i, [_vp, _i, _i, _vp, _vp]),
    "rl_bn_bwd_slots": (_i, [_l]),
    "rl_bn_bwd_reduce": (_i, [C.POINTER(BnBwdDesc), _vp]),
    "rl_bn_bwd_finalize": (_i, [_vp, _i, _l, _i, _vp, _vp, _vp, _vp]),
    "rl_bn_bwd_apply": (_i, [C.POINTER(BnBwdDesc), _vp]),
    "rl_bn_bwd_fused_supported": (_i, [_l, _i, _l]),
    "rl_bn_bwd_fused": (_i, [C.POINTER(BnBwdDesc), _l, _vp, _vp, _vp, _vp]),
    "rl_resid_bn_bwd_supported": (_i, [_l, _i]),
    "rl_resid_bn_bwd_reduce": (_i, [C.POINTER(ResidBnBwdDesc), _vp]),
    "rl_resid_bn_bwd_apply": (_i, [C.POINTER(ResidBnBwdDesc), _vp]),
    "rl_resid_bn_bwd_fused_supported": (_i, [_l, _i]),
    "rl_resid_bn_bwd_fused": (_i, [C.POINTER(ResidBnBwdDesc), _vp, _vp, _vp, _vp, _vp]),
    "rl_copy_rows": (_i, [C.POINTER(RowsDesc), _vp]),
    "rl_copy_rows_pair": (_i, [C.POINTER(RowsDesc), C.POINTER(RowsDesc), _vp]),
    "rl_scatter_add_rows": (_i, [C.POINTER(RowsDesc), _vp]),
    "rl_csr_workspace_bytes": (_l, [C.POINTER(CsrTask), _i, _i]),
    "rl_csr_build": (_i, [C.POINTER(CsrTask), _i, _i, _vp, _l, _vp]),
    "rl_segment_sum_rows": (_i, [C.POINTER(SegsumDesc), _vp]),
    "rl_pool_supported": (_i, [_i, _i]),
    "rl_pool_slab_floats": (_l, [_l, _i]),
    "rl_pool_bwd_slots": (_i, [_l, _i]),
    "rl_pool_bwd_grid": (_i, [_l, _i, _i]),
    "rl_pool_fwd_slots": (_i, [_l, _i]),
    "rl_pool_fwd": (_i, [C.POINTER(PoolDesc), _vp]),
    "rl_rpe_stats_slots": (_i, [_l]),
    "rl_rpe_stats": (_i, [C.POINTER(PoolDesc), _vp, _vp]),
    "rl_rpe_bn_reduce": (_i, [C.POINTER(PoolDesc), _vp, _vp, _vp]),
    "rl_rpe_wgrad_slab_floats": (_l, [_l, _i, _i]),
    "rl_rpe_wgrad": (_i, [C.POINTER(PoolDesc), _vp, _vp, _vp, _l, _vp, _vp]),
    "rl_pool_bwd": (_i, [C.POINTER(PoolDesc), _vp]),
    "rl_attpool_fwd": (_i, [_vp, _vp, _l, _i, _i, _vp, _vp]),
    "rl_attpool_bwd": (_i, [_vp, _vp, _vp, _vp, _l, _i, _i, _vp, _vp, _vp]),
    "rl_add_act_fwd": (_i, [_vp, _vp, _vp, _vp, _vp, _vp, _l, _i, _f, _vp, _vp]),
    "rl_add_act_bwd": (_i, [_vp, _vp, _l, _i, _f, _vp]),
    "rl_rpe_build": (_i, [_vp, _l, _vp, _vp, _i, _i, _i, _vp, _vp]),
    "rl_rpe_build_dist": (_i, [_vp, _l, _vp, _vp, _i, _i, _i, _vp, _vp]),
    "rl_batch_assemble": (_i, [_vp, _i, _i, _i, _vp, _vp, _vp, _vp, _vp, _vp]),
    "rl_batch_assemble_scratch_doubles": (_l, [_i, _i]),
    "rl_batch_assemble_flag_u32": (_l, [_i, _i, _i]),
    "rl_batch_draw": (_i, [_vp, _i, _i, C.c_uint64, _vp, _vp, _vp]),
    "rl_scale_mask": (_i, [_vp, _vp, _f, _l, _vp]),
    "rl_dropout_tick": (_i, [_vp, _vp, _vp]),
    "rl_dropout_fwd": (_i, [_vp, _vp, _vp, _i, _f, _vp, _l, _l, _i, _vp, C.c_uint64, _f, _vp]),
    "rl_dropout_bwd": (_i, [_vp, _l, _l, _i, _vp, C.c_uint64, _f, _vp]),
    "rl_upsample_cf": (_i, [_vp, _vp, _vp, _i, _i, _i, _i, _i, _i, _vp, _vp]),
    "rl_logits_unpermute": (_i, [_vp, _vp, _i, _i, _i, _vp, _vp]),
    "rl_logits_permute_grad": (_i, [_vp, _vp, _i, _i, _i, _vp, _vp]),
    "rl_logits_unpermute_b": (_i, [_vp, _vp, C.c_int64, _i, _i, _i, _vp, _vp]),
    "rl_logits_permute_grad_b": (_i, [_vp, _vp, C.c_int64, _i, _i, _i, _vp, _vp]),
    "rl_band_sort_workspace_bytes": (C.c_int64, [_i, _i, _vp, _i]),
    "rl_band_sort": (_i, [_vp, C.c_int64, _vp, _i, _i, _vp, _i, _vp, _vp, C.c_int64, _vp]),
    "rl_loss_max_classes": (_i, []),
    "rl_loss_work_doubles": (_l, [_l, _i]),
    "rl_loss_forward": (_i, [_vp, _vp, _i, _i, _i, _i, _f, _f, _i, _vp, _vp, _vp]),
    "rl_loss_backward": (_i, [_vp, _vp, _i, _i, _i, _i, _f, _f, _i, _vp, _f, _vp, _vp]),
    "rl_loss_forward_masked": (_i, [_vp, _vp, _i, _i, _i, _i, _f, _f, _i, _vp, _i, _vp, _vp, _vp]),
    "rl_loss_backward_masked": (_i, [_vp, _vp, _i, _i, _i, _i, _f, _f, _i, _vp, _f, _vp, _i, _vp, _vp]),
    "rl_loss_partials": (_i, [_vp, _vp, _i, _i, _i, _i, _f, _vp, _vp]),
    "rl_loss_totals_offset": (_l, [_i]),
    "rl_loss_from_totals": (_i, [_l, _i, _i, _f, _f, _i, _vp, _vp, _vp]),
    "rl_loss_backward_global": (_i, [_vp, _vp, _i, _i, _i, _i, _f, _f, _i, _vp, _f, _l, _vp, _vp]),
    "rl_lovasz_workspace_bytes": (_l, [_i, _i, _i]),
    "rl_lovasz_coef_offset": (_l, [_i, _i, _i]),
    "rl_lovasz_forward": (_i, [_vp, _vp, _i, _i, _i, _i, _vp, _vp, _l, _vp, _vp]),
    "rl_lovasz_backward": (_i, [_vp, _vp, _i, _i, _i, _i, _vp, _vp, _l, _f, _vp, _vp]),
    "rl_softmax_cf": (_i, [_vp, _i, _i, _i, _vp, _vp]),
    "rl_adam_step": (_i, [_vp, _vp, _vp, _vp, _l, _vp, _f, _f, _f, _f, _vp, _vp]),
    "rl_scene_workspace_bytes": (_l, [_l, _i]),
    "rl_scene_crop": (_i, [_vp, _l, _i, _vp, _i, _vp, _l, _vp, _vp, _l, _vp]),
    "rl_scene_accumulate": (_i, [_vp, _i, _i, _vp, _f, _f, _vp, _vp, _l, _vp]),
    "rl_scene_min_count": (_i, [_vp, _l, _vp, _vp, _vp]),
    "rl_scene_crop_padded": (_i, [_vp, _l, _i, _vp, _i, _vp, _l, _vp, _vp, _l, _vp]),
    "rl_scene_accumulate_first": (_i, [_vp, _i, _i, _vp, _f, _f, _vp, _vp, _l, _l, _i, _vp]),
    "rl_scenes_workspace_bytes": (_l, [_i, _l, _i]),
    "rl_scenes_init": (_i, [_vp, _i, _l, _vp, _vp, _l, _vp]),
    "rl_scenes_crop": (_i, [_vp, _i, _i, _l, _vp, _i, _i, _vp, _vp, _vp, _vp, _l, _vp]),
    "rl_scenes_crop_padded": (_i, [_vp, _i, _i, _l, _vp, _i, _i, _vp, _vp, _vp, _vp, _l, _vp]),
    "rl_scenes_vote_crop": (_i, [_vp, _i, _i, _l, _vp, _vp, _vp, _i, _i, _i, _i, _vp, _l, _l, _vp, _vp, _vp, _vp, _vp, _l, _vp]),
    "rl_scenes_vote_accumulate": (_i, [_vp, _i, _i, _l, _l, _i, _vp, _vp, _f, _f, _vp, _l, _vp]),
    "rl_grid_workspace_bytes": (_l, [_l, _i]),
    "rl_grid_bounds": (_i, [_vp, _l, _i, _f, _vp, _vp, _l, _vp]),
    "rl_grid_sort": (_i, [_vp, _l, _i, _i, _vp, _l, _vp]),
    "rl_grid_heads": (_i, [_l, _i, _vp, _vp, _vp, _l, _vp]),
    "rl_grid_reduce": (_i, [_vp, _l, _i, _vp, _i, _l, _vp, _vp, _vp, _vp, _l, _vp]),
    "rl_scene_confusion": (_i, [_vp, _l, _i, _vp, _l, _vp, _vp, _vp]),
    "rl_cluster_workspace_bytes": (_l, [_l]),
    "rl_cluster_cells": (_i, [_vp, _l, _f, _vp, _vp, _l, _vp]),
    "rl_cluster_union": (_i, [_vp, _vp, _l, _f, _vp, _i, _i, _l, _vp, _vp, _vp, _l, _vp]),
    "rl_cluster_smooth_workspace_bytes": (_l, [_l]),
    "rl_cluster_union_smooth": (_i, [_vp, _vp, _l, _f, _vp, _i, _i, _l, _vp, _vp, _f, _f, _vp, _vp, _vp, _l, _vp]),
    "rl_cluster_reduce": (_i, [_vp, _vp, _vp, _l, _l, _vp, _vp, _vp, _vp, _vp, _vp, _vp, _l, _vp]),
    "rl_scene_labels": (_i, [_vp, _l, _i, _f, _vp, _vp, _vp]),
    "rl_keypoints_workspace_bytes": (_l, [_l]),
    "rl_keypoints_cells": (_i, [_vp, _l, _f, _vp, _vp, _l, _vp]),
    "rl_keypoints_sort": (_i, [_vp, _vp, _vp, _l, _f, _vp, _i, _i, _vp, _l, _vp]),
    "rl_keypoints_support": (_i, [_vp, _l, _f, _vp, _l, _vp]),
    "rl_keypoints_peaks": (_i, [_vp, _l, _f, _l, _vp, _vp, _l, _vp]),
    "rl_keypoints_refine": (_i, [_vp, _l, _l, _f, _l, _vp, _vp, _vp, _vp, _vp, _vp, _vp, _l, _vp]),
    "rl_normals": (_i, [_vp, _l, _vp, _l, _l, _i, _vp, _vp, _vp, _vp, _vp]),
    "rl_pairs_workspace_bytes": (_l, [_l]),
    "rl_pairs_sort": (_i, [_vp, _i, _vp, _i, _l, _l, _l, _vp, _vp, _l, _vp]),
    "rl_pairs_write": (_i, [_l, _l, _l, _l, _vp, _vp, _vp, _vp, _l, _vp]),
    "rl_boxes_workspace_bytes": (_l, [_l, _l]),
    "rl_boxes_sort": (_i, [_vp, _i, _l, _l, _vp, _l, _vp]),
    "rl_boxes_moments": (_i, [_vp, _l, _l, _vp, _vp, _vp, _l, _vp]),
    "rl_boxes_fit": (_i, [_vp, _l, _l, _vp, _vp, _vp, _vp, _vp, _vp, _vp, _vp, _l, _vp]),
}
EXPORTS = tuple(_SIGNATURES)
MAX_LOSS_CLASSES = 256


def library_path() -> str:
    return _LIB_PATH
# ... 51 lines not shown
```

3d_recognizer_amd/randlanet/_ops.py:

```python
import contextlib
import ctypes as C
import os
from dataclasses import dataclass
from typing import Optional, Tuple

import torch

from . import _hip as H

F32 = torch.float32
BF16 = torch.bfloat16

_STORAGE = os.environ.get("RL_STORAGE", "f32")


def set_storage(mode: str) -> None:
    global _STORAGE
    if mode not in ("f32", "bf16"):
        raise ValueError(f"storage must be 'f32' or 'bf16', got {mode!r}")
    if mode == "bf16" and get_wide_gemm() == "fp32":
        raise H.HipKernelError("bf16 storage needs the bf16x3 / bf16 arithmetic mode (RL_WIDE_GEMM)")
    _STORAGE = mode


# ... 144 lines not shown
    B, N, _ = xyz.shape
    out = []
    for c0 in range(0, len(tasks), H.KNN_MAX_TASKS):
        chunk = tasks[c0:c0 + H.KNN_MAX_TASKS]
        arr = (H.KnnTask * len(chunk))()
        res = []
        nbytes_io = 0
        for t, (Ns, Nq, k) in zip(arr, chunk):
            assert 0 < k <= Ns <= N and 0 < Nq <= N and k <= H.KNN_MAX_K
            idx = torch.empty((B, Nq, k), dtype=torch.int32, device=xyz.device)
            d2 = torch.empty((B, Nq, k), dtype=F32, device=xyz.device)
            t.support, t.support_bstride, t.query, t.query_bstride = xyz.data_ptr(), N, xyz.data_ptr(), N
            t.Ns, t.Nq, t.k, t.idx_out, t.d2_out = Ns, Nq, k, idx.data_ptr(), d2.data_ptr()
            res.append((idx, d2))
            nbytes_io += B * (12 * (Ns + Nq) + 8 * Nq * k)
        nbytes = H.lib().rl_knn_multi_workspace_bytes(arr, len(chunk), B)
        ws = torch.empty(max(nbytes, 256), dtype=torch.uint8, device=xyz.device)
        with _rec("knn_multi", tuple(chunk), nbytes_io, sum(8 * B * a * b for a, b, _ in chunk)):
            H.check(H.lib().rl_knn_multi(arr, len(chunk), B, ws.data_ptr(), ws.numel(), _st()), "rl_knn_multi")
        out.extend(res)
    return out


def knn_f32(support: torch.Tensor, query: torch.Tensor, k: int, brute: bool = False
            ) -> Tuple[torch.Tensor, torch.Tensor]:
    _dev_check(support, query)
    B, Ns, _ = support.shape
    Nq = query.shape[1]
    idx = torch.empty((B, Nq, k), dtype=torch.int64, device=support.device)
    d2 = torch.empty((B, Nq, k), dtype=F32, device=support.device)
    ws, nbytes = _knn_workspace(support.device, B, Ns, Nq, k, brute)
    with _rec("knn", (B, Ns, Nq, k), B * (12 * (Ns + Nq) + 12 * Nq * k), 8 * B * Ns * Nq):
        H.check(H.lib().rl_knn_f32(support.data_ptr(), query.data_ptr(), B, Ns, Nq, k, idx.data_ptr(),
                                   d2.data_ptr(), H.ptr(ws), nbytes, _st()), "rl_knn_f32")
    return idx, d2


@dataclass
class Rpe:
    xyz: torch.Tensor
    idx: torch.Tensor
    d2: torch.Tensor
    B: int
    n: int
    K: int

    @property
    def rows(self) -> int:
        return self.B * self.n * self.K


def set_wide_gemm(mode: str) -> None:
    H.check(H.lib().rl_set_wide_gemm(mode.encode()), "rl_set_wide_gemm")


def get_wide_gemm() -> str:
    return H.lib().rl_get_wide_gemm().decode()


def set_wgemm_staging(how: str) -> None:
    H.check(H.lib().rl_set_wgemm_staging(how.encode()), "rl_set_wgemm_staging")


def set_wgemm_tile(how: str) -> None:
    H.check(H.lib().rl_set_wgemm_tile(how.encode()), "rl_set_wgemm_tile")


def set_gemm_ksplit(enable: bool) -> None:
    H.check(H.lib().rl_set_gemm_ksplit(int(bool(enable))), "rl_set_gemm_ksplit")


def rpe_build(a: "Rpe", distances: bool = False) -> Lazy:
    _dev_check(a.xyz, a.idx, a.d2)
    assert a.idx.dtype == torch.int32 and a.idx.shape == (a.B, a.n, a.K) and a.d2.shape == a.idx.shape
    assert a.xyz.shape[0] == a.B and a.xyz.shape[1] >= a.n and a.xyz.shape[2] == 3
    out = torch.empty((a.rows, 12), dtype=F32, device=a.xyz.device)
    with _rec("rpe_build", (a.rows,), (48 + 8) * a.rows, 0):
        fn = H.lib().rl_rpe_build_dist if distances else H.lib().rl_rpe_build
        H.check(fn(a.xyz.data_ptr(), a.xyz.shape[1], a.idx.data_ptr(), a.d2.data_ptr(), a.B, a.n, a.K,
                   out.data_ptr(), _st()), "rl_rpe_build")
    return Lazy(out, a.B, a.n * a.K, a.n * a.K, 10)


def _fill_a(d, a):
    if isinstance(a, Rpe):
        _dev_check(a.xyz, a.idx, a.d2)
        assert a.idx.dtype == torch.int32 and a.idx.shape == (a.B, a.n, a.K) and a.d2.shape == a.idx.shape
        assert a.xyz.shape[0] == a.B and a.xyz.shape[1] >= a.n and a.xyz.shape[2] == 3
        d.a_mode = 1
        d.xyz, d.xyz_bstride = a.xyz.data_ptr(), a.xyz.shape[1]
        d.nbr_idx, d.nbr_d2, d.nbr_k = a.idx.data_ptr(), a.d2.data_ptr(), a.K
        d.B, d.n, d.K = a.B, a.n, 10
        return a.rows, 10
    _dev_check(a.raw, a.scale, a.shift)
    assert a.raw.dtype in (F32, BF16) and a.raw.dim() == 2 and a.raw.shape[1] >= a.C
    assert a.raw.shape[0] >= (a.B - 1) * a.bstride + a.n, "A operand rows out of range"
    d.a_mode = 0
    d.A, d.lda, d.a_bstride = a.raw.data_ptr(), a.raw.shape[1], a.bstride
    if a.scale is not None:
        assert a.scale.numel() == a.C and a.shift.numel() == a.C
        d.in_scale, d.in_shift, d.in_act, d.in_slope = a.scale.data_ptr(), a.shift.data_ptr(), a.act, a.slope
    d.B, d.n, d.K = a.B, a.n, a.C
    return a.rows, a.C


def weight_strides(W: torch.Tensor, transposed: bool, K: int, N: int) -> Tuple[int, int]:
    if transposed:
        assert W.shape[0] == K and W.shape[1] == N, (tuple(W.shape), K, N)
        return N, 1
    assert W.shape[0] == N and W.shape[1] == K, (tuple(W.shape), K, N)
    return 1, K




def split_weights(entries) -> dict:
    out_map = {}
    if get_wide_gemm() == "fp32" or not entries:
        return out_map
    entries = [e[:5] for e in entries if e[3] % 8 == 0 and (e[4] > 64 or e[3] > 64 or len(e) > 5)]
    if not entries:
        return out_map
    total = sum(2 * K * N + 8 for _, _, _, K, N in entries)
    buf = torch.empty(total, dtype=torch.bfloat16, device=entries[0][0].device)
    arr = (H.WsplitItem * len(entries))()
    off = 0
    for it, (W, ks, ns, K, N) in zip(arr, entries):
        _dev_check(W)
        assert W.dtype == F32 and W.numel() == K * N
        out = buf[off:off + 2 * K * N]
        it.W, it.w_ks, it.w_ns, it.K, it.N, it.out = W.data_ptr(), ks, ns, K, N, out.data_ptr()
        out_map[(W.data_ptr(), ks, ns, K, N)] = out
        off += (2 * K * N + 7) // 8 * 8
    with _rec("split_weights", (len(entries),), 6 * sum(K * N for _, _, _, K, N in entries), 0):
        H.check(H.lib().rl_split_weights(arr, len(entries), _st()), "rl_split_weights")
    return out_map


def gemm_stat_slots(M: int, N: int, K: int) -> int:
    return int(H.lib().rl_gemm_stat_slots(M, N, K))


def gemm(a, W: torch.Tensor, w_ks: int, w_ns: int, N: int, bias: Optional[torch.Tensor] = None, *,
         out: Optional[torch.Tensor] = None, out_bstride: Optional[int] = None,
         accumulate: bool = False, stats: Optional[torch.Tensor] = None,
         addend: Optional[torch.Tensor] = None, out2: Optional[torch.Tensor] = None,
         out2_index: Optional[torch.Tensor] = None, out2_bstride: int = 0, split_col: int = 0,
         wsplit: Optional[dict] = None, pivot: Optional[tuple] = None, bnb: Optional[Lazy] = None):
    d = H.GemmDesc()
    M, K = _fill_a(d, a)
    assert isinstance(a, Rpe) or a.raw.dtype == F32, "rl_gemm reads fp32 rows"
    rows_per_batch = a.n * a.K if isinstance(a, Rpe) else a.n
    _dev_check(W, bias, out, stats)
    assert W.dtype == F32 and W.numel() == K * N
    if out is None:
        out = torch.empty((M, N), dtype=F32, device=W.device)
        out_bstride = rows_per_batch
    else:
        assert out.dtype == F32 and out.dim() == 2 and out.shape[1] >= (split_col if out2 is not None else N)
        out_bstride = rows_per_batch if out_bstride is None else out_bstride
        assert out.shape[0] >= (d.B - 1) * out_bstride + rows_per_batch, "Y rows out of range"
    if bias is not None:
        assert bias.numel() == N
    if stats is not None:
        assert stats.dtype == torch.float64 and stats.numel() >= gemm_stat_slots(M, N, K) * 2 * N
    d.N, d.W, d.w_ks, d.w_ns, d.bias = N, W.data_ptr(), w_ks, w_ns, H.ptr(bias)
    planes = wsplit.get((W.data_ptr(), w_ks, w_ns, K, N)) if wsplit else None
# ... 14 lines not shown
                assert out2.shape[0] >= M
            else:
                assert out2_index.dtype == torch.int32 and out2_index.numel() == M
                assert out2.shape[0] >= (d.B - 1) * out2_bstride + 1
        d.addend, d.out2, d.out2_index = H.ptr(addend), H.ptr(out2), H.ptr(out2_index)
        d.out2_bstride, d.split_col = out2_bstride, split_col
    bnb_pre = None
    if bnb is not None:
        if (stats is None and pivot is None and bnb.mean is not None and bnb.scale is not None and bnb.raw.dtype == F32
                and bnb.raw.shape[1] == out.shape[1] and bnb.bstride == out_bstride and bnb.C == N
                and 4 * M * N <= BNB_MAX_BYTES and H.lib().rl_gemm_streams(C.byref(d))):
            _dev_check(bnb.raw, bnb.scale, bnb.shift, bnb.mean, bnb.invstd)
            st_b = new_stats(W.device, N)
            d.stats = st_b.data_ptr()
            d.bnb_Y, d.bnb_scale, d.bnb_shift = bnb.raw.data_ptr(), bnb.scale.data_ptr(), bnb.shift.data_ptr()
            d.bnb_mean, d.bnb_invstd, d.bnb_act, d.bnb_slope = bnb.mean.data_ptr(), bnb.invstd.data_ptr(), bnb.act, bnb.slope
            bnb_pre = (st_b, gemm_stat_slots(M, N, K))
    kfloats = H.lib().rl_gemm_kslab_floats(M, N, K) if (N > 64 and not isinstance(a, Rpe) and out2 is None and addend is None) else 0
    if kfloats > 0:
        kslab = _slab(W.device, kfloats)
        d.kslab, d.kslab_floats = kslab.data_ptr(), kslab.numel()
    with _rec("gemm_rpe" if isinstance(a, Rpe) else "gemm", (M, K, N), 4 * (M * (K if not isinstance(a, Rpe) else 6) + M * N * (2 if accumulate else 1) + K * N), 2 * M * K * N):
        H.check(H.lib().rl_gemm(C.byref(d), _st()), "rl_gemm")
    return (out, bnb_pre) if bnb is not None else out


BNB_MAX_BYTES = 32 << 20


def gemm_pair(a, first: tuple, second: tuple, wsplit: Optional[dict]):
    if not wsplit or isinstance(a, Rpe) or a.raw.dtype != F32:
        return None
    descs, outs = [], []
    M = K = None
    for (W, w_ks, w_ns, N, stats, pivot) in (first, second):
        d = H.GemmDesc()
        M, K = _fill_a(d, a)
        planes = wsplit.get((W.data_ptr(), w_ks, w_ns, K, N))
        if planes is None:
            return None
        _dev_check(W, stats)
        out = torch.empty((M, N), dtype=F32, device=W.device)
        d.N, d.W, d.w_ks, d.w_ns, d.W_split = N, W.data_ptr(), w_ks, w_ns, planes.data_ptr()
        d.Y, d.ldy, d.y_bstride = out.data_ptr(), N, a.n
        if stats is not None:
            assert stats.dtype == torch.float64 and stats.numel() >= H.row_blocks(M, 128) * 2 * N
            d.stats = stats.data_ptr()
            if pivot is not None:
                _dev_check(*pivot)
                d.stats_pivot_mean, d.stats_pivot_bias = pivot[0].data_ptr(), H.ptr(pivot[1])
        descs.append(d)
        outs.append(out)
    if not H.lib().rl_gemm_pair_supported(C.byref(descs[0]), C.byref(descs[1])):
        return None
    N1, N2 = first[3], second[3]
    with _rec("gemm", (M, K, N1 + N2), 4 * (M * K + M * (N1 + N2) + K * (N1 + N2)), 2 * M * K * (N1 + N2)):
        H.check(H.lib().rl_gemm_pair(C.byref(descs[0]), C.byref(descs[1]), _st()), "rl_gemm_pair")
    return outs[0], outs[1]


_SLAB = {}


def _slab(device, floats: int) -> torch.Tensor:
    key = (device, torch.cuda.current_stream(device).cuda_stream)
    buf = _SLAB.get(key)
    if buf is None or buf.numel() < floats:
        buf = torch.empty(max(floats, 1 << 20), dtype=F32, device=device)
        _SLAB[key] = buf
    return buf


WGRAD_BATCH_BYTES = 3 << 30


def wgrad(a, dY: torch.Tensor, dy_bstride: int, N: int, dW: torch.Tensor, w_ks: int, w_ns: int,
          dbias: Optional[torch.Tensor] = None, pending: Optional[list] = None, batch: Optional[list] = None) -> None:
    d = H.WgradDesc()
    M, K = _fill_a(d, a)
    rows_per_batch = a.n * a.K if isinstance(a, Rpe) else a.n
    _dev_check(dY, dW, dbias)
    rows_bf16 = dY.dtype == BF16
    assert dY.dtype in (F32, BF16) and dY.dim() == 2 and dY.shape[1] >= N
    assert isinstance(a, Rpe) or a.raw.dtype == dY.dtype, "A and dY must share their storage type"
    d.rows_bf16 = int(rows_bf16)
    assert dY.shape[0] >= (d.B - 1) * dy_bstride + rows_per_batch
    assert dW.numel() == K * N and (dbias is None or dbias.numel() == N)
    floats = H.lib().rl_wgrad_slab_floats(M, N, K)
    slab = _slab(dY.device, floats) if pending is None else torch.empty(floats, dtype=F32, device=dY.device)
    d.N, d.dY, d.lddy, d.dy_bstride = N, dY.data_ptr(), dY.shape[1], dy_bstride
    d.dW, d.w_ks, d.w_ns, d.dbias = dW.data_ptr(), w_ks, w_ns, H.ptr(dbias)
    d.slab, d.slab_floats = slab.data_ptr(), slab.numel()
    d.defer_reduce = 0 if pending is None else 1
    es = 2 if rows_bf16 else 4
    nbytes, flops = es * (M * (K if not isinstance(a, Rpe) else 6) + M * N) + 4 * K * N, 2 * M * K * N
    kind = H.lib().rl_wgrad_batchable(C.byref(d)) if (batch is not None and pending is not None) else 0
    if kind:
        batch.append((d, nbytes, flops, a, dY, slab, kind))
        if sum(b[1] for b in batch) > WGRAD_BATCH_BYTES:
            wgrad_batch_flush(batch)
    else:
        with _rec("wgrad_rpe" if isinstance(a, Rpe) else "wgrad", (M, K, N), nbytes, flops):
            H.check(H.lib().rl_wgrad(C.byref(d), _st()), "rl_wgrad")
    if pending is not None:
        it = H.WgradReduceItem()
        it.slab, it.dW, it.dbias, it.w_ks, it.w_ns = slab.data_ptr(), dW.data_ptr(), H.ptr(dbias), w_ks, w_ns
        it.nsplit, it.N, it.K = H.lib().rl_wgrad_nsplit(M, N, K), N, K
        pending.append((it, slab, dW, dbias))


def wgrad_batch_flush(batch: list) -> None:
    for kind, name in ((1, "wgrad_batch"), (2, "swgrad_batch")):
        part = [b for b in batch if b[6] == kind]
        if not part:
            continue
        arr = (H.WgradDesc * len(part))(*[b[0] for b in part])
        with _rec(name, (len(part),), sum(b[1] for b in part), sum(b[2] for b in part)):
            H.check(H.lib().rl_wgrad_batch(arr, len(part), _st()), "rl_wgrad_batch")
    batch.clear()


def wgrad_flush(pending: list) -> None:
    if not pending:
        return
    arr = (H.WgradReduceItem * len(pending))(*[p[0] for p in pending])
    nbytes = sum(4 * p[1].numel() for p in pending)
    with _rec("wgrad_reduce_batch", (len(pending),), nbytes, 0):
        H.check(H.lib().rl_wgrad_reduce_batch(arr, len(pending), _st()), "rl_wgrad_reduce_batch")
    pending.clear()


def new_stats(device, C: int) -> torch.Tensor:
    return torch.empty((H.MAX_SLOTS, 2, C), dtype=torch.float64, device=device)


class SyncGroup:

    def __init__(self, world: int, group=None, staged: bool = False):
        self.world, self.group, self.staged = world, group, staged
        self.local_clouds, self.global_clouds, self.cloud_offset = 1, world, 0

    def set_shard(self, local_clouds: int, rank: Optional[int] = None) -> None:
        import torch.distributed as dist
        if self.world <= 1 or not (dist.is_available() and dist.is_initialized()):
            self.local_clouds, self.global_clouds, self.cloud_offset = local_clouds, local_clouds * self.world, 0
            return
        rank = dist.get_rank(self.group) if rank is None else rank
        counts = torch.zeros(self.world, dtype=torch.int64)
        counts[rank] = local_clouds
        if dist.get_backend(self.group) == "nccl":
            dev_counts = counts.cuda()
            dist.all_reduce(dev_counts, op=dist.ReduceOp.SUM, group=self.group)
            counts = dev_counts.cpu()
        else:
            dist.all_reduce(counts, op=dist.ReduceOp.SUM, group=self.group)
        self.local_clouds, self.global_clouds = local_clouds, int(counts.sum())
        self.cloud_offset = int(counts[:rank].sum())

    def global_rows(self, rows: int) -> int:
        assert rows % self.local_clouds == 0, (rows, self.local_clouds)
        return rows // self.local_clouds * self.global_clouds

    def allreduce(self, t: torch.Tensor) -> None:
        import torch.distributed as dist
        if self.staged:
            h = t.cpu()
            dist.all_reduce(h, op=dist.ReduceOp.SUM, group=self.group)
            t.copy_(h)
        else:
            dist.all_reduce(t, op=dist.ReduceOp.SUM, group=self.group)


def _stats_totals(stats: torch.Tensor, nslots: int, C: int) -> torch.Tensor:
    out = torch.empty((1, 2, C), dtype=torch.float64, device=stats.device)
    H.check(H.lib().rl_bn_reduce_slots(stats.data_ptr(), nslots, C, out.data_ptr(), _st()), "rl_bn_reduce_slots")
    return out


def bn_finalize(stats, rows: int, tile: int, C: int, gamma, beta, rmean, rvar, nbt, momentum: float,
                eps: float, training: bool, sync: Optional[SyncGroup] = None, nslots: Optional[int] = None,
                folded_bias: Optional[torch.Tensor] = None, defer: Optional[list] = None, pivoted: bool = False,
                pivot: Optional[torch.Tensor] = None):
    dev = gamma.device
    nslots = H.row_blocks(rows, tile) if nslots is None else nslots
    if training and sync is not None:
        stats = _stats_totals(stats, nslots, C)
        if pivoted:
            m = pivot if pivot is not None else rmean
            c = (m - folded_bias if folded_bias is not None else m).to(torch.float64)
            S, Q = stats[0, 0].clone(), stats[0, 1].clone()
            stats[0, 0] = S + rows * c
# ... 342 lines not shown
    pd.rows_bf16 = int(G.dtype == BF16)
    es = G.element_size()
    floats = H.lib().rl_rpe_wgrad_slab_floats(v.B * v.n, 2 * v.h, stage)
    slab = torch.empty(floats, dtype=F32, device=G.device)
    with _rec("rpe_wgrad", (v.rows, Kin, v.h), es * v.rows * v.h * (2 if stage == 2 else 1) + 8 * v.rows, 2 * v.rows * v.h * (Kin + (v.h if stage == 2 else 0))):
        H.check(H.lib().rl_rpe_wgrad(C.byref(pd), G.data_ptr(), coef.data_ptr(), slab.data_ptr(), slab.numel(), H.ptr(GU1), _st()),
                "rl_rpe_wgrad")
    it = H.WgradReduceItem()
    it.slab, it.dW, it.dbias, it.w_ks, it.w_ns = slab.data_ptr(), dW.data_ptr(), dbias.data_ptr(), 1, Kin
    it.nsplit, it.N, it.K = H.lib().rl_rpe_stats_slots(v.B * v.n), v.h, Kin
    pending.append((it, slab, dW, dbias))


def pool_supported(d: int, K: int) -> bool:
    return bool(H.lib().rl_pool_supported(d, K))


def _pool_desc(u, g: Lazy, idx: torch.Tensor, W: torch.Tensor, n: int, d: int, stage: int = 0) -> H.PoolDesc:
    _dev_check(g.raw, idx, W, g.scale, g.shift)
    h = d // 2
    B = u.B
    assert idx.dtype == torch.int32 and idx.shape == (B, n, 16)
    assert g.raw.shape[1] == h and g.C == h and g.n == n and g.raw.shape[0] >= (B - 1) * g.bstride + n
    assert W.numel() == d * d
    pd = H.PoolDesc()
    if isinstance(u, VirtualRpe):
        assert stage in (1, 2) and u.h == h and u.n == n and u.bn1 is not None and (stage == 1 or u.bn2 is not None)
        _fill_virtual(pd, u, stage)
    else:
        _dev_check(u.raw, u.scale, u.shift)
        assert u.raw.shape == (B * n * 16, h) and u.bstride == u.n == n * 16 and u.C == h
        pd.U, pd.u_scale, pd.u_shift, pd.u_act, pd.u_slope = u.raw.data_ptr(), H.ptr(u.scale), H.ptr(u.shift), u.act, u.slope
    pd.G, pd.g_bstride = g.raw.data_ptr(), g.bstride
    pd.g_scale, pd.g_shift, pd.g_act, pd.g_slope = H.ptr(g.scale), H.ptr(g.shift), g.act, g.slope
    pd.idx, pd.W, pd.points, pd.n, pd.d, pd.nbr_k = idx.data_ptr(), W.data_ptr(), B * n, n, d, 16
    return pd


def pool_fwd(u, g: Lazy, idx: torch.Tensor, W: torch.Tensor, n: int, d: int, stage: int = 0, next_stats: bool = False):
    pd = _pool_desc(u, g, idx, W, n, d, stage)
    stats2 = None
    if next_stats:
        assert stage == 1
        ns = H.lib().rl_pool_fwd_slots(u.B * n, d)
        stats2 = torch.empty((ns, 2, d // 2), dtype=torch.float64, device=W.device)
        pd.bn_fwd_stats2 = stats2.data_ptr()
    out = torch.empty((u.B * n, d), dtype=F32, device=W.device)
    pd.Pout = out.data_ptr()
    P = u.B * n
    virt = isinstance(u, VirtualRpe)
    fbytes = P * (4 * (32 + d) + 16 * (16 + 4 * (d // 2))) if virt else 4 * (2 * P * 16 * (d // 2) + P * 16 + P * d)
    with _rec("pool_fwd_virtual" if virt else "pool_fwd", (P, 16, d), fbytes, 2 * P * 16 * d * d):
        H.check(H.lib().rl_pool_fwd(C.byref(pd), _st()), "rl_pool_fwd")
    if next_stats:
        return out, stats2, ns
    return out


def pool_bwd(u, g: Lazy, idx: torch.Tensor, W: torch.Tensor, n: int, d: int, dP: torch.Tensor,
             GU: torch.Tensor, gu_accumulate: bool, dW: torch.Tensor, pending: Optional[list] = None,
             stage: int = 0, bn_bwd_stats: Optional[torch.Tensor] = None, batch: Optional[list] = None) -> torch.Tensor:
    pd = _pool_desc(u, g, idx, W, n, d, stage)
    _dev_check(dP, GU, dW)
    P = u.B * n
    assert dP.shape == (P, d) and GU.shape == (P * 16, d // 2) and dW.numel() == d * d
    rdt = row_dtype()
    virt = isinstance(u, VirtualRpe)
    assert GU.dtype == (rdt if virt else F32), "GU: the row storage type under a virtual rpe branch, fp32 for a real U tensor"
    pd.rows_bf16 = int(rdt == BF16)
    es = 2 if rdt == BF16 else 4
    DG = torch.empty((P * 16, d // 2), dtype=rdt, device=W.device)
    if bn_bwd_stats is not None:
        _dev_check(bn_bwd_stats)
        assert stage > 0 and bn_bwd_stats.dtype == torch.float64
        assert bn_bwd_stats.numel() >= H.lib().rl_pool_bwd_slots(P, d) * d
        pd.bn_bwd_stats = bn_bwd_stats.data_ptr()
    pd.dP, pd.GU, pd.gu_accumulate, pd.DG, pd.dW = dP.data_ptr(), GU.data_ptr(), int(gu_accumulate), DG.data_ptr(), dW.data_ptr()
    h = d // 2
    if virt:
        nbytes = P * (4 * (32 + d) + 16 * (16 + 4 * h) + 4 * d + es * 16 * h * (2 + int(gu_accumulate)))
    else:
        nbytes = (4 * (2 * P * 16 * h + P * 16 + 2 * P * d) + es * P * 16 * h + 4 * P * 16 * h * (1 + int(gu_accumulate)))
    if d == 128:
        X = torch.empty((P * 16, d), dtype=rdt, device=W.device)
        dS = torch.empty((P * 16, d), dtype=rdt, device=W.device)
        pd.X_out, pd.dS_out = X.data_ptr(), dS.data_ptr()
        with _rec("pool_bwd", (P, 16, d), nbytes + 2 * es * P * 16 * d, 4 * P * 16 * d * d):
            H.check(H.lib().rl_pool_bwd(C.byref(pd), _st()), "rl_pool_bwd")
        wgrad(plain(X, u.B, n * 16), dS, n * 16, d, dW, 1, d, None, pending=pending, batch=batch)
        return DG
    floats = H.lib().rl_pool_slab_floats(P, d)
    if pending is not None:
        slab = torch.empty(floats, dtype=F32, device=W.device)
        pd.dW = None
    else:
        slab = _slab(W.device, floats)
    pd.slab, pd.slab_floats = slab.data_ptr(), slab.numel()
    with _rec("pool_bwd", (P, 16, d), nbytes, 6 * P * 16 * d * d):
        H.check(H.lib().rl_pool_bwd(C.byref(pd), _st()), "rl_pool_bwd")
    if pending is not None:
        it = H.WgradReduceItem()
        it.slab, it.dW, it.dbias, it.w_ks, it.w_ns = slab.data_ptr(), dW.data_ptr(), None, 1, d
        it.nsplit, it.N, it.K = H.lib().rl_pool_bwd_grid(P, d, int(virt)), d, d
        pending.append((it, slab, dW, None))
    return DG


def attpool_fwd(X: torch.Tensor, S: torch.Tensor, P: int, K: int) -> torch.Tensor:
    _dev_check(X, S)
    Cc = X.shape[1]
    assert X.shape == S.shape == (P * K, Cc)
    out = torch.empty((P, Cc), dtype=F32, device=X.device)
    with _rec("attpool_fwd", (P, K, Cc), 4 * (2 * P * K * Cc + P * Cc), 0):
        H.check(H.lib().rl_attpool_fwd(X.data_ptr(), S.data_ptr(), P, K, Cc, out.data_ptr(), _st()), "rl_attpool_fwd")
    return out


def attpool_bwd(X, S, Pout, dP, P: int, K: int):
    _dev_check(X, S, Pout, dP)
    Cc = X.shape[1]
    assert X.shape == S.shape == (P * K, Cc) and Pout.shape == dP.shape == (P, Cc)
    dS = torch.empty_like(S)
    dXa = torch.empty_like(X)
    with _rec("attpool_bwd", (P, K, Cc), 4 * (4 * P * K * Cc + 2 * P * Cc), 0):
        H.check(H.lib().rl_attpool_bwd(X.data_ptr(), S.data_ptr(), Pout.data_ptr(), dP.data_ptr(), P, K, Cc,
                                       dS.data_ptr(), dXa.data_ptr(), _st()), "rl_attpool_bwd")
    return dS, dXa


def add_act_fwd(y1: Lazy, y2: Lazy, slope: float) -> torch.Tensor:
    assert y1.rows == y2.rows and y1.C == y2.C and y1.bstride == y1.n and y2.bstride == y2.n
    out = torch.empty((y1.rows, y1.C), dtype=F32, device=y1.raw.device)
    with _rec("add_act", (y1.rows, y1.C), 12 * y1.rows * y1.C, 0):
        H.check(H.lib().rl_add_act_fwd(y1.raw.data_ptr(), y1.scale.data_ptr(), y1.shift.data_ptr(), y2.raw.data_ptr(),
                                       y2.scale.data_ptr(), y2.shift.data_ptr(), y1.rows, y1.C, slope, out.data_ptr(),
                                       _st()), "rl_add_act_fwd")
    return out


def add_act_bwd(G: torch.Tensor, O: torch.Tensor, slope: float) -> None:
    assert G.shape == O.shape and G.is_contiguous() and O.is_contiguous()
    with _rec("add_act", (G.shape[0], G.shape[1]), 12 * G.numel(), 0):
        H.check(H.lib().rl_add_act_bwd(G.data_ptr(), O.data_ptr(), G.shape[0], G.shape[1], slope, _st()), "rl_add_act_bwd")


def scale_mask(x: torch.Tensor, mask: torch.Tensor, scale: float) -> None:
    _dev_check(x, mask)
    assert mask.dtype == torch.uint8 and mask.numel() == x.numel() and x.dtype == F32
    H.check(H.lib().rl_scale_mask(x.data_ptr(), mask.data_ptr(), scale, x.numel(), _st()), "rl_scale_mask")


def dropout_tick(counter: torch.Tensor) -> torch.Tensor:
    _dev_check(counter)
    assert counter.dtype == torch.int64 and counter.numel() == 1
    key = torch.empty(1, dtype=torch.int64, device=counter.device)
    H.check(H.lib().rl_dropout_tick(counter.data_ptr(), key.data_ptr(), _st()), "rl_dropout_tick")
    return key


def dropout_fwd(x: Lazy, key: torch.Tensor, seed: int, p: float, first_row: int = 0) -> torch.Tensor:
    _dev_check(x.raw, x.scale, x.shift, key)
    assert x.bstride == x.n and x.raw.shape == (x.rows, x.C) and x.C % 4 == 0
    out = torch.empty_like(x.raw)
    with _rec("dropout", (x.rows, x.C), 8 * x.rows * x.C, 0):
        H.check(H.lib().rl_dropout_fwd(x.raw.data_ptr(), H.ptr(x.scale), H.ptr(x.shift), x.act, x.slope, out.data_ptr(),
                                       x.rows, first_row, x.C, key.data_ptr(), seed & 0xFFFFFFFFFFFFFFFF, p, _st()), "rl_dropout_fwd")
    return out


def dropout_bwd(G: torch.Tensor, key: torch.Tensor, seed: int, p: float, first_row: int = 0) -> None:
    _dev_check(G, key)
    assert G.dim() == 2 and G.shape[1] % 4 == 0
# ... 708 lines not shown
```

include/rl_randlanet.h:

```cpp
#ifndef RL_RANDLANET_H
#define RL_RANDLANET_H

#include <stdint.h>

#ifdef __cplusplus
extern "C" {
#endif

#define RL_VERSION 110

#define RL_OK 0
#define RL_ERR_ARGS (-1)
#define RL_ERR_FEW_SUPPORT (-2)
#define RL_ERR_LAUNCH (-3)
#define RL_ERR_UNSUPPORTED (-4)

#define RL_MAX_SLOTS 1024
#define RL_KNN_MAX_K 64
#define RL_MAX_CLASSES 256

const char* rl_last_error(void);
const char* rl_last_kernel(void);
int rl_version(void);
int64_t rl_launch_count(void);
// ... 34 lines not shown
    int32_t in_act;
    float in_slope;
    const float* in_scale;
    const float* in_shift;
    const float* xyz;
    int64_t xyz_bstride;
    const int32_t* nbr_idx;
    const float* nbr_d2;
    int32_t nbr_k;
    int32_t B, n, N, K;
    const float* W;
    int64_t w_ks, w_ns;
    const float* bias;
    float* Y;
    int64_t ldy, y_bstride;
    int32_t accumulate;
    double* stats;
    float* kslab;
    int64_t kslab_floats;
    const float* addend;
    float* out2;
    const int32_t* out2_index;
    int64_t out2_bstride;
    int32_t split_col;
    const void* W_split;
    const float* stats_pivot_mean;
    const float* stats_pivot_bias;
    const float* bnb_Y;
    const float* bnb_scale;
    const float* bnb_shift;
    const float* bnb_mean;
    const float* bnb_invstd;
    int32_t bnb_act;
    float bnb_slope;
} rl_gemm_desc;

int rl_gemm_streams(const rl_gemm_desc* d);
int rl_gemm_pair_supported(const rl_gemm_desc* a, const rl_gemm_desc* b);
int rl_gemm_pair(const rl_gemm_desc* a, const rl_gemm_desc* b, void* stream);

typedef struct rl_wsplit_item {
    const float* W;
    int64_t w_ks, w_ns;
    int32_t K, N;
    void* out;
} rl_wsplit_item;

int rl_split_weights(const rl_wsplit_item* items, int count, void* stream);

int64_t rl_gemm_kslab_floats(int64_t M, int N, int K);
int64_t rl_gemm_stat_slots(int64_t M, int N, int K);

int rl_set_wide_gemm(const char* mode);
const char* rl_get_wide_gemm(void);
int rl_set_wgemm_staging(const char* how);
int rl_set_wgemm_tile(const char* how);
int rl_set_gemm_ksplit(int enable);
int rl_set_sgemm_grid_div(int div);
int rl_gemm(const rl_gemm_desc* d, void* stream);

typedef struct rl_wgrad_desc {
    const float* A;
    int64_t lda, a_bstride;
    int32_t a_mode;
    int32_t in_act;
    float in_slope;
    const float* in_scale;
    const float* in_shift;
    const float* xyz;
    int64_t xyz_bstride;
    const int32_t* nbr_idx;
    const float* nbr_d2;
    int32_t nbr_k;
    int32_t B, n, N, K;
    const float* dY;
    int64_t lddy, dy_bstride;
    float* dW;
    int64_t w_ks, w_ns;
    float* dbias;
    float* slab;
    int64_t slab_floats;
    int32_t defer_reduce;
    int32_t rows_bf16;
} rl_wgrad_desc;

int64_t rl_wgrad_slab_floats(int64_t M, int N, int K);
int rl_wgrad(const rl_wgrad_desc* d, void* stream);

typedef struct rl_wgrad_reduce_item {
    const float* slab;
    float* dW;
    float* dbias;
    int64_t w_ks, w_ns;
    int32_t nsplit, N, K;
    int32_t reserved;
} rl_wgrad_reduce_item;

int rl_wgrad_nsplit(int64_t M, int N, int K);
int rl_wgrad_batchable(const rl_wgrad_desc* d);
int rl_wgrad_batch(const rl_wgrad_desc* descs, int count, void* stream);
int rl_wgrad_reduce_batch(const rl_wgrad_reduce_item* items, int count, void* stream);

int rl_bn_finalize(const double* stats, int nslots, int64_t count, int C, const float* gamma,
                   const float* beta, float* running_mean, float* running_var, int64_t* nbt,
                   float momentum, float eps, int training, float* scale, float* shift,
                   float* save_mean, float* save_invstd, const float* folded_bias, int pivoted, float* pivot, void* stream);

typedef struct rl_bn_finalize_item {
    const double* stats;
    int64_t count;
    const float* gamma;
    const float* beta;
    float* running_mean;
    float* running_var;
    int64_t* num_batches_tracked;
    float* scale;
    float* shift;
    float* save_mean;
    float* save_invstd;
    const float* folded_bias;
    int32_t nslots, C, training;
    float momentum, eps;
    int32_t pivoted;
    float* pivot;
} rl_bn_finalize_item;
int rl_bn_finalize_batch(const rl_bn_finalize_item* items, int count, void* stream);

typedef struct rl_bn_bwd_desc {
    float* G;
    const float* Y;
    int64_t ld, bstride;
    int32_t B, n, C;
    int32_t act;
    float slope;
    const float* scale;
    const float* shift;
    const float* mean;
    const float* invstd;
    double* stats;
    const float* coef;
} rl_bn_bwd_desc;

int rl_bn_reduce_slots(const double* stats, int nslots, int C, double* out, void* stream);
int rl_bn_bwd_slots(int64_t rows);
int rl_bn_bwd_reduce(const rl_bn_bwd_desc* d, void* stream);
int rl_bn_bwd_finalize(const double* stats, int nslots, int64_t count, int C, float* dgamma,
                       float* dbeta, float* coef, void* stream);
int rl_bn_bwd_finalize_pair(const double* stats0, const double* stats1, int nslots, int64_t count, int C, float* dgamma0,
                            float* dbeta0, float* coef0, float* dgamma1, float* dbeta1, float* coef1, void* stream);
typedef struct rl_bn_bwd_finalize_item {
    const double* stats;
    int64_t count;
    float* dgamma;
    float* dbeta;
    float* coef;
    int32_t nslots, C;
} rl_bn_bwd_finalize_item;
int rl_bn_bwd_finalize_batch(const rl_bn_bwd_finalize_item* items, int count, void* stream);
int rl_bn_bwd_apply(const rl_bn_bwd_desc* d, void* stream);
int rl_bn_bwd_fused_supported(int64_t rows, int C, int64_t ld);
int rl_bn_bwd_fused(const rl_bn_bwd_desc* d, int64_t count, float* dgamma, float* dbeta, float* coef_out, void* stream);

typedef struct rl_resid_bn_bwd_desc {
    float* G;
    float* G2;
    const float* O;
    float slope;
    int64_t rows;
    int32_t C;
    const float* Y1; const float* scale1; const float* mean1; const float* invstd1;
// ... 29 lines not shown
int rl_copy_rows_pair(const rl_rows_desc* d0, const rl_rows_desc* d1, void* stream);

int rl_scatter_add_rows(const rl_rows_desc* d, void* stream);

typedef struct rl_csr_task {
    const int32_t* idx;
    int32_t n_src, k, n_dst;
    int32_t* offsets;
    int32_t* entries;
} rl_csr_task;

int64_t rl_csr_workspace_bytes(const rl_csr_task* tasks, int ntasks, int B);
int rl_csr_build(const rl_csr_task* tasks, int ntasks, int B, void* workspace, int64_t workspace_bytes,
                 void* stream);

typedef struct rl_segsum_desc {
    const float* src;
    int64_t lds, src_bstride;
    float* dst;
    int64_t ldd, dst_bstride;
    const int32_t* offsets;
    const int32_t* entries;
    int64_t entries_per_cloud;
    int32_t B, n_dst, C;
    int32_t accumulate;
    int32_t src_bf16;
} rl_segsum_desc;

int rl_segment_sum_rows(const rl_segsum_desc* d, void* stream);

int rl_attpool_fwd(const float* X, const float* S, int64_t P, int K, int C, float* Pout,
                   void* stream);
int rl_attpool_bwd(const float* X, const float* S, const float* Pout, const float* dP, int64_t P,
                   int K, int C, float* dS, float* dXa, void* stream);

typedef struct rl_pool_desc {
    const float* U;
    const float* u_scale;
    const float* u_shift;
    int32_t u_act;
    float u_slope;
    const float* G;
    int64_t g_bstride;
    const float* g_scale;
    const float* g_shift;
    int32_t g_act;
    float g_slope;
    const int32_t* idx;
    const float* W;
    int64_t points;
    int32_t n, d, nbr_k;
    float* Pout;
    const float* dP;
    float* GU;
    int32_t gu_accumulate;
    float* DG;
    float* dW;
    float* slab;
    int64_t slab_floats;
    float* X_out;
    float* dS_out;
    int32_t u_source;
    const float* xyz;
    int64_t xyz_bstride;
    const float* nbr_d2;
    const float* W1;
    const float* b1;
    const float* scale1;
    const float* shift1;
    const float* W2;
    const float* b2;
    const float* scale2;
    const float* shift2;
    const float* mean1;
    const float* invstd1;
    const float* mean2;
    const float* invstd2;
    int32_t xyz_width;
    double* bn_bwd_stats;
    double* bn_fwd_stats2;
    int32_t rows_bf16;
    const float* pivot_mean1;
    const float* pivot_mean2;
} rl_pool_desc;

int rl_pool_supported(int d, int nbr_k);
int64_t rl_pool_slab_floats(int64_t points, int d);
int rl_pool_bwd_slots(int64_t points, int d);
int rl_pool_bwd_grid(int64_t points, int d, int virtual_stage);
int rl_pool_fwd_slots(int64_t points, int d);
int rl_pool_fwd(const rl_pool_desc* d, void* stream);
int rl_pool_bwd(const rl_pool_desc* d, void* stream);

int rl_rpe_stats_slots(int64_t points);
int rl_rpe_stats(const rl_pool_desc* d, double* stats, void* stream);

int rl_rpe_bn_reduce(const rl_pool_desc* d, const float* G, double* stats, void* stream);
int64_t rl_rpe_wgrad_slab_floats(int64_t points, int d, int stage);
int rl_rpe_wgrad(const rl_pool_desc* d, const float* G, const float* coef, float* slab, int64_t slab_floats,
                 float* GU1, void* stream);

int rl_add_act_fwd(const float* Y1, const float* s1, const float* b1, const float* Y2,
                   const float* s2, const float* b2, int64_t rows, int C, float slope, float* O,
                   void* stream);
int rl_add_act_bwd(float* G, const float* O, int64_t rows, int C, float slope, void* stream);

int rl_rpe_build(const float* xyz, int64_t xyz_bstride, const int32_t* nbr_idx, const float* nbr_d2, int B,
                 int n, int k, float* out, void* stream);
int rl_rpe_build_dist(const float* xyz, int64_t xyz_bstride, const int32_t* nbr_idx, const float* nbr_dist, int B,
                      int n, int k, float* out, void* stream);

typedef struct rl_cloud_job {
    const void* xyz;
    const float* features;
    const int64_t* labels;
    int64_t n_points;
    int32_t xyz_f64;
    int32_t normalization;
    int32_t augment;
    int32_t normal_col;
    double jitter_variance, jitter_limit;
    double scale;
    double R[9];
    double shift[3];
} rl_cloud_job;

int64_t rl_batch_assemble_scratch_doubles(int B, int n);
int64_t rl_batch_assemble_flag_u32(int B, int n, int b);
int rl_batch_assemble(const rl_cloud_job* jobs_dev, int B, int n, int F, const int64_t* indices,
                      const double* noise, double* scratch, float* out_input, int64_t* out_labels,
                      void* stream);
int rl_batch_draw(const rl_cloud_job* jobs_dev, int B, int n, uint64_t seed, int64_t* indices, double* noise, void* stream);

typedef struct rl_head_desc {
    const float* X;
    const float* scale;
    const float* shift;
    int32_t act;
    float slope;
    const float* mean;
    const float* invstd;
    const float* W;
    const float* bias;
    const int64_t* perm;
    const int64_t* labels;
    int32_t B, N, C;
    int32_t loss_kind;
    float alpha, gamma;
    int32_t neglect_background;
    float drop_p;
    const int64_t* drop_key;
    uint64_t drop_seed;
    int64_t drop_first_row;
    double* work;
    float* G;
    double* bn_bwd_stats;
    float* slab;
    int64_t slab_floats;
    float grad_scale;
    int32_t reserved;
    void* drop_mask;
    int64_t perm_bstride;
    const float* class_weight;
    int32_t masked;
} rl_head_desc;
int rl_head_supported(int C, int K);
int rl_head_grid(int64_t rows);
int rl_head_fwd(const rl_head_desc* d, double* out, void* stream);
int rl_head_bwd(const rl_head_desc* d, void* stream);

int rl_scale_mask(float* x, const uint8_t* mask, float scale, int64_t count, void* stream);

int rl_dropout_tick(int64_t* counter, int64_t* key_out, void* stream);
int rl_dropout_fwd(const float* src, const float* scale, const float* shift, int act, float slope, float* dst,
                   int64_t rows, int64_t first_row, int C, const int64_t* key, uint64_t seed, float p, void* stream);
// ... 143 lines not shown
```

Baseline: 1256.

## Feed pool128 weight gradient from concat-gather operand instead of materialized X

The d=128 pool backward kernel no longer writes its concatenated, activated input X to global memory. Instead, the wide weight-gradient kernel rebuilds it on the fly: the first half of K comes from the lazy U operand, and the second half is gathered by neighbour index from a second source, with its own scale, shift and activation folded in. This removes a full P*16*d fp32 write and read-back, at the cost of an index load and scattered gathered reads inside the wgrad kernel. The path is gated by a mode switch and a planner check, and falls back to the materialized X when unsupported.

```diff
diff --git a/3d_recognizer_amd/csrc/gemm.hip b/3d_recognizer_amd/csrc/gemm.hip
--- a/3d_recognizer_amd/csrc/gemm.hip
+++ b/3d_recognizer_amd/csrc/gemm.hip
@@ -256,8 +256,18 @@
 constexpr int WG_T = 64;
 constexpr int WG_S = 80;
 
+struct ConcatSrc {
+    const float* A2;
+    const int32_t* idx;
+    const float* sc2; const float* sh2;
+    long a2_bstride;
+    int lda2, split, act2;
+    float slope2;
+};
+
 struct WgradParams {
     AOperand a;
+    ConcatSrc cat;
     int N;
     const float* dY;
     long lddy, dy_bstride;
@@ -2253,11 +2263,12 @@
     __bf16* Dl = Dh + PW2_RB * RP;
     __bf16* Xh = lds_a;
     __bf16* Xl = Xh + PW2_RB * RP;
-    __shared__ __attribute__((aligned(16))) float lz[2][PW2_T];
+    __shared__ __attribute__((aligned(16))) float lz[3][PW2_T];
     const int tid = threadIdx.x, lane = tid & 63, wave = tid >> 6;
     const int lr = lane & 15, lq = lane >> 4;
     const int N = p.N, K = p.a.K;
     const int n0 = by * PW2_T, k0 = bz * PW2_T;
+    const bool cat = !RB && p.cat.split > 0;
     const int nvalid = min(PW2_T, N - n0), kvalid = min(PW2_T, K - k0);
     const long r_begin = (long)bx * p.rows_per_block;
     const long r_end = min(p.a.M, r_begin + p.rows_per_block);
@@ -2275,10 +2286,25 @@
         ucol[i] = (u & 7) * 16 + (lane & 3) * 4;
         urow[i] = (u >> 3) * 16 + (lane >> 2);
     }
+    const bool gat = cat && k0 + ucol[0] >= p.cat.split;
     if (tid < PW2_T) {
-        const bool in = lazy && tid < kvalid;
-        lz[0][tid] = in ? p.a.lazy.scale[k0 + tid] : 1.f;
-        lz[1][tid] = in ? p.a.lazy.shift[k0 + tid] : 0.f;
+        if (cat) {
+            const bool two = k0 + tid >= p.cat.split;
+            const int c = two ? k0 + tid - p.cat.split : k0 + tid;
+            const float* scp = two ? p.cat.sc2 : p.a.lazy.scale;
+            const float* shp = two ? p.cat.sh2 : p.a.lazy.shift;
+            RlLazy t = p.a.lazy;
+            if (two) { t.scale = p.cat.sc2; t.shift = p.cat.sh2; t.act = p.cat.act2; t.slope = p.cat.slope2; }
+            const bool in = scp != nullptr && tid < kvalid;
+            lz[0][tid] = in ? scp[c] : 1.f;
+            lz[1][tid] = in ? shp[c] : 0.f;
+            lz[2][tid] = rl_eff_slope(t);
+        } else {
+            const bool in = lazy && tid < kvalid;
+            lz[0][tid] = in ? p.a.lazy.scale[k0 + tid] : 1.f;
+            lz[1][tid] = in ? p.a.lazy.shift[k0 + tid] : 0.f;
+            lz[2][tid] = 1.f;
+        }
     }
     const int nh = wave >> 2, kw = wave & 3;
     f32x4 acc[4][2];
@@ -2289,8 +2315,22 @@
     const bool want_bias = p.has_bias && bz == 0;
     f32x4 bs = {0.f, 0.f, 0.f, 0.f};
     float4 rd[2], ra[2];
+    int gi[2] = {0, 0};
+    auto fetch_idx = [&](long r0) {
+#pragma unroll
+        for (int i = 0; i < 2; ++i) {
+            const unsigned R = (unsigned)min(r0 + urow[i], r_end - 1);
+            gi[i] = *reinterpret_cast<const int32_t*>(reinterpret_cast<const char*>(p.cat.idx) + R * 4u);
+        }
+    };
+    int cb = 0, cend = 0;
+    if (cat) {
+        cb = (int)((unsigned)r_begin / (unsigned)p.a.n);
+        cend = (cb + 1) * p.a.n;
+    }
 
     auto fetch = [&](long r0) {
+        if (cat) while ((int)r0 >= cend) { ++cb; cend += p.a.n; }
 #pragma unroll
         for (int i = 0; i < 2; ++i) {
             const long R = r0 + urow[i];
@@ -2307,15 +2347,30 @@
                     }
                     rd[i] = rl_ldx4<RB>(p.dY, off + n0 + ucol[i]);
                 }
-                if (ucol[i] < kvalid) ra[i] = rl_ldx4<RB>(p.a.A, a_row_offset(p.a, R) + k0 + ucol[i]);
-            }
-        }
+                if (ucol[i] < kvalid) {
+                    if (gat) {
+                        int b = cb;
+                        for (int e = cend; (int)R >= e; e += p.a.n) ++b;
+                        const unsigned off = ((unsigned)b * (unsigned)p.cat.a2_bstride + (unsigned)gi[i]) * (unsigned)p.cat.lda2 +
+                                             (unsigned)(k0 + ucol[i] - p.cat.split);
+                        ra[i] = *reinterpret_cast<const float4*>(p.cat.A2 + off);
+                    } else ra[i] = rl_ldx4<RB>(p.a.A, a_row_offset(p.a, R) + k0 + ucol[i]);
+                }
+            }
+        }
+        if (gat) fetch_idx(r0 + PW2_RB);
     };
     auto commit = [&](long r0) {
 #pragma unroll
         for (int i = 0; i < 2; ++i) {
             float4 v = ra[i];
-            if (lazy && r0 + urow[i] < r_end && ucol[i] < kvalid) {
+            if (cat) {
+                if (r0 + urow[i] < r_end && ucol[i] < kvalid) {
+                    const f32x4 x = rl_fold_act4((f32x4){v.x, v.y, v.z, v.w}, *reinterpret_cast<const f32x4*>(&lz[0][ucol[i]]),
+                                                 *reinterpret_cast<const f32x4*>(&lz[1][ucol[i]]), lz[2][ucol[i]]);
+                    v = make_float4(x[0], x[1], x[2], x[3]);
+                }
+            } else if (lazy && r0 + urow[i] < r_end && ucol[i] < kvalid) {
                 const float4 sc = *reinterpret_cast<const float4*>(&lz[0][ucol[i]]);
                 const float4 sh = *reinterpret_cast<const float4*>(&lz[1][ucol[i]]);
                 v.x = actf(v.x * sc.x + sh.x);
@@ -2346,6 +2401,7 @@
         const bf16x4 r1 = __builtin_bit_cast(bf16x4, __builtin_amdgcn_ds_read_tr16_b64_v4i16((__attribute__((address_space(3))) s16x4g*)(q + 4 * RP)));
         return __builtin_shufflevector(r0, r1, 0, 1, 2, 3, 4, 5, 6, 7);
     };
+    if (gat && r_begin < r_end) fetch_idx(r_begin);
     if (r_begin < r_end) fetch(r_begin);
     for (long r0 = r_begin; r0 < r_end; r0 += PW2_RB) {
         __syncthreads();
@@ -2414,13 +2470,17 @@
     int first_block;
     int nsplit;
     unsigned short gy, gz;
-    unsigned char a_contig, dy_contig, has_bias, pad;
+    unsigned char a_contig, dy_contig, has_bias;
+    unsigned char cat;
 };
 constexpr int WB_MAX = 24;
+constexpr int WB_CAT_MAX = 4;
 struct WgradBatch {
     WBItem item[WB_MAX];
+    ConcatSrc cat[WB_CAT_MAX];
     int count, pad;
 };
+static_assert(sizeof(WgradBatch) <= 4096, "the grouped launch carries its layer table in the kernel arguments (4 KB)");
 template <int TERMS>
 __global__ __launch_bounds__(512, 4) void pwgrad128w_batch_kernel(const WgradBatch b) {
     int i = 0;
@@ -2443,6 +2503,8 @@
     p.a.n = it.n; p.a.K = it.K; p.a.M = it.M; p.a.contig = it.a_contig; p.a.vec4 = 1; p.a.vec4p = 1;
     p.N = it.N; p.dY = it.dY; p.lddy = it.lddy; p.dy_bstride = it.dy_bstride; p.rows_per_batch = it.rows_per_batch;
     p.dy_contig = it.dy_contig; p.slab = it.slab; p.rows_per_block = it.rows_per_block; p.has_bias = it.has_bias;
+    p.cat = ConcatSrc{};
+    if (it.cat) p.cat = b.cat[it.cat - 1];
     pwgrad128w_body<TERMS, false>(p, bx, by, bz);
 }
 
@@ -2458,6 +2520,7 @@
     p.a.n = it.n; p.a.K = it.K; p.a.M = it.M; p.a.contig = it.a_contig; p.a.vec4 = 0; p.a.vec4p = 0;
     p.N = it.N; p.dY = it.dY; p.lddy = it.lddy; p.dy_bstride = it.dy_bstride; p.rows_per_batch = it.rows_per_batch;
     p.dy_contig = it.dy_contig; p.slab = it.slab; p.rows_per_block = it.rows_per_block; p.has_bias = it.has_bias;
+    p.cat = ConcatSrc{};
     const int bx = (int)blockIdx.x - it.first_block;
     if (bx >= it.nsplit) return;
     switch (it.gy) {
@@ -2636,7 +2699,18 @@
     return N <= 16 ? swgrad_kernel<KT, 1> : N <= 32 ? swgrad_kernel<KT, 2> : swgrad_kernel<KT, 4>;
 }
 
-WgradPlan plan_wgrad(long M, int N, int K, int a_mode, bool pwgrad, bool rows_bf16) {
+WgradPlan plan_wgrad(long M, int N, int K, int a_mode, bool pwgrad, bool rows_bf16, int cat_split = 0) {
+    if (cat_split != 0) {
+        WgradPlan pl = plan_wgrad(M, N, K, a_mode, pwgrad, rows_bf16);
+        const bool w = pl.fn == (WgradFn)pwgrad128w_kernel<1> || pl.fn == (WgradFn)pwgrad128w_kernel<3>;
+        if (!(w && !rows_bf16 && K == 2 * cat_split && cat_split % 16 == 0)) {
+            pl.fn = nullptr;
+            pl.batch = 0;
+            pl.refusal = "rl_wgrad: a concat-gather A operand (a2_split) needs the wide (128 x 128 tile) kernel outside the fp32 "
+                         "arithmetic mode, fp32 rows, K == 2 * a2_split and a2_split % 16 == 0";
+        }
+        return pl;
+    }
     WgradPlan pl{};
     pl.threads = 256;
     const int terms = wide_gemm_terms();
@@ -2842,17 +2916,32 @@
 static int wgrad_fill(const rl_wgrad_desc* d, WgradParams* pp, WgradPlan* plan) {
     RL_REQUIRE(d != nullptr, RL_ERR_ARGS, "rl_wgrad: null descriptor");
     WgradParams& p = *pp;
+    const int split = d->a2_split;
+    RL_REQUIRE(split == 0 || (split > 0 && split < d->K && d->a_mode == 0), RL_ERR_ARGS,
+               "rl_wgrad: a2_split must lie inside (0, K), on a tensor operand");
     int rc = fill_a(&p.a, "rl_wgrad", d->A, d->lda, d->a_bstride, d->a_mode, d->in_act, d->in_slope,
                     d->in_scale, d->in_shift, d->xyz, d->xyz_bstride, d->nbr_idx, d->nbr_d2, d->nbr_k,
-                    d->B, d->n, d->K);
+                    d->B, d->n, split ? split : d->K);
     if (rc) return rc;
+    p.a.K = d->K;
+    p.cat = ConcatSrc{};
+    if (split) {
+        RL_REQUIRE(d->A2 && d->a2_idx && d->a2_bstride > 0 && (d->a2_scale == nullptr) == (d->a2_shift == nullptr), RL_ERR_ARGS,
+                   "rl_wgrad: incomplete second source (A2, a2_idx, a2_bstride; a2_scale / a2_shift come together)");
+        RL_REQUIRE((((uintptr_t)d->A2) & 15) == 0 && d->lda2 % 4 == 0 && d->lda2 >= d->K - split && d->lda2 < (1l << 31), RL_ERR_ARGS,
+                   "rl_wgrad: A2 must be 16-byte aligned with lda2 a multiple of 4 and >= K - a2_split");
+        RL_REQUIRE((int64_t)d->B * d->a2_bstride * d->lda2 < (1l << 31) && p.a.M < (1l << 30), RL_ERR_ARGS,
+                   "rl_wgrad: a concat-gather operand needs a second source below 2^31 elements and fewer than 2^30 rows");
+        p.cat.A2 = d->A2; p.cat.idx = d->a2_idx; p.cat.sc2 = d->a2_scale; p.cat.sh2 = d->a2_shift;
+        p.cat.a2_bstride = d->a2_bstride; p.cat.lda2 = (int)d->lda2; p.cat.split = split; p.cat.act2 = d->a2_act; p.cat.slope2 = d->a2_slope;
+    }
     RL_REQUIRE(d->N > 0 && d->dY && d->dW && d->slab && d->lddy >= d->N, RL_ERR_ARGS, "rl_wgrad: bad dY/dW/slab");
     p.N = d->N; p.dY = d->dY; p.lddy = d->lddy; p.dy_bstride = d->dy_bstride;
     p.rows_per_batch = (d->a_mode == 1) ? d->n * d->nbr_k : d->n;
     RL_REQUIRE(d->dy_bstride >= p.rows_per_batch, RL_ERR_ARGS, "rl_wgrad: dy_bstride smaller than rows per cloud");
     p.dy_contig = (d->dy_bstride == p.rows_per_batch);
     p.slab = d->slab; p.has_bias = d->dbias != nullptr;
-    const WgradPlan pl = plan_wgrad(p.a.M, d->N, d->K, d->a_mode, pwgrad_ok(p), d->rows_bf16 != 0);
+    const WgradPlan pl = plan_wgrad(p.a.M, d->N, d->K, d->a_mode, pwgrad_ok(p), d->rows_bf16 != 0, split);
     RL_REQUIRE(pl.fn != nullptr, RL_ERR_UNSUPPORTED, "%s", pl.refusal);
     RL_REQUIRE(d->slab_floats >= (int64_t)pl.nsplit * ((int64_t)d->N * d->K + d->N), RL_ERR_ARGS,
                "rl_wgrad: slab too small (%ld floats)", (long)d->slab_floats);
@@ -2876,12 +2965,14 @@
     for (int kind = 1; kind <= 2; ++kind) {
         WgradBatch b;
         b.count = 0; b.pad = 0;
+        for (int c = 0; c < WB_CAT_MAX; ++c) b.cat[c] = ConcatSrc{};
+        int ncat = 0;
         long blocks = 0;
         auto flush = [&]() -> int {
-            if (b.count == 0 || blocks == 0) { b.count = 0; blocks = 0; return RL_OK; }
+            if (b.count == 0 || blocks == 0) { b.count = 0; blocks = 0; ncat = 0; return RL_OK; }
             launch_wgrad_batch(kind, blocks, st, b);
             RL_LAUNCH_CHECK("rl_wgrad_batch");
-            b.count = 0; blocks = 0;
+            b.count = 0; blocks = 0; ncat = 0;
             return RL_OK;
         };
         for (int i = 0; i < count; ++i) {
@@ -2895,6 +2986,10 @@
             RL_REQUIRE(d->defer_reduce, RL_ERR_ARGS, "rl_wgrad_batch: the layers' slabs are summed by rl_wgrad_reduce_batch (defer_reduce must be set)");
             if (pl.batch != kind) continue;
             any[kind] = true;
+            if (p.cat.split > 0 && ncat == WB_CAT_MAX) {
+                rc = flush();
+                if (rc) return rc;
+            }
             WBItem& it = b.item[b.count];
             it.A = p.a.A; it.dY = p.dY; it.sc = p.a.lazy.scale; it.sh = p.a.lazy.shift; it.slab = p.slab;
             it.lda = p.a.lda; it.a_bstride = p.a.a_bstride; it.lddy = p.lddy; it.dy_bstride = p.dy_bstride;
@@ -2912,7 +3007,12 @@
                 it.first_block = (int)blocks;
                 blocks += per > 1 ? (long)((pl.nsplit + 7) / 8 * 8) * per : (long)pl.nsplit;
             }
-            it.a_contig = (unsigned char)p.a.contig; it.dy_contig = (unsigned char)p.dy_contig; it.has_bias = (unsigned char)p.has_bias; it.pad = 0;
+            it.a_contig = (unsigned char)p.a.contig; it.dy_contig = (unsigned char)p.dy_contig; it.has_bias = (unsigned char)p.has_bias;
+            it.cat = 0;
+            if (p.cat.split > 0) {
+                b.cat[ncat] = p.cat;
+                it.cat = (unsigned char)++ncat;
+            }
             RL_REQUIRE(blocks < (1l << 30), RL_ERR_ARGS, "rl_wgrad_batch: too many workgroups");
             if (++b.count == WB_MAX) {
                 rc = flush();
@@ -2943,6 +3043,17 @@
     return RL_OK;
 }
 
+extern "C" int rl_wgrad_plan(const rl_wgrad_desc* d, int32_t* grid_xyz, int32_t* threads, const char** kernel) {
+    WgradParams p;
+    WgradPlan pl;
+    int rc = wgrad_fill(d, &p, &pl);
+    if (rc) return rc;
+    if (grid_xyz) { grid_xyz[0] = (int32_t)pl.grid.x; grid_xyz[1] = (int32_t)pl.grid.y; grid_xyz[2] = (int32_t)pl.grid.z; }
+    if (threads) *threads = pl.threads;
+    if (kernel) *kernel = pl.name;
+    return RL_OK;
+}
+
 extern "C" int rl_wgrad_nsplit(int64_t M, int N, int K) { return plan_wgrad(M, N, K, 0, true, false).nsplit; }
 
 extern "C" int rl_wgrad_reduce_batch(const rl_wgrad_reduce_item* items, int count, void* stream) {
diff --git a/3d_recognizer_amd/csrc/pool.hip b/3d_recognizer_amd/csrc/pool.hip
--- a/3d_recognizer_amd/csrc/pool.hip
+++ b/3d_recognizer_amd/csrc/pool.hip
@@ -1,3 +1,5 @@
+#include <string.h>
+
 #include "rl_common.h"
 #include <stdlib.h>
 
@@ -55,10 +57,7 @@
 __device__ __forceinline__ float sum4(const f32x4 a) { return (a[0] + a[1]) + (a[2] + a[3]); }
 __device__ __forceinline__ f32x4 vbn(const f32x4 raw, float s, float h) { return __builtin_elementwise_fma(raw, splat(s), splat(h)); }
 __device__ __forceinline__ f32x4 vrelu(const f32x4 z) { return __builtin_elementwise_max(z, splat(0.f)); }
-__device__ __forceinline__ float eff_slope(const RlLazy& t) {
-    if (t.scale == nullptr || t.act == RL_ACT_NONE) return 1.f;
-    return t.act == RL_ACT_RELU ? 0.f : t.slope;
-}
+__device__ __forceinline__ float eff_slope(const RlLazy& t) { return rl_eff_slope(t); }
 __device__ __forceinline__ f32x4 vact(const f32x4 z, float e) { return __builtin_elementwise_max(z, z * splat(e)); }
 
 struct PoolParams {
@@ -211,7 +210,7 @@
 #pragma unroll
     for (int c = 0; c < DT; ++c) {
         const int k = 16 * c + 4 * lj;
-        const float4 v = f4(vact(v4(raw[c]) * lf.sc(c) + lf.sh(c), chunk_slope<DT>(c, lj, es_u, es_g)));
+        const float4 v = f4(rl_fold_act4(v4(raw[c]), lf.sc(c), lf.sh(c), chunk_slope<DT>(c, lj, es_u, es_g)));
         xa[c] = v;
         *reinterpret_cast<float4*>(Xs + li * XS + k) = v;
     }
@@ -608,7 +607,7 @@
     }
 }
 
-template <bool GB>
+template <bool GB, bool XO = true>
 __global__ __launch_bounds__(512) void pool128_bwd_kernel(const PoolParams p) {
     __shared__ __attribute__((aligned(16))) float lfm[LFold<8>::LDS_FLOATS];
     constexpr int NW = 8;
@@ -661,12 +660,14 @@
         loads_issued();
         cu = cn;
         idx_cur = idx_nxt; idx_nxt = idx_n2;
-#pragma unroll
-        for (int c = 0; c < DT; ++c) rl_stx4<GB>(p.X_out, (pt * 16 + li) * D + 16 * c + 4 * lj, xa[c]);
+        if constexpr (XO)
+#pragma unroll
+            for (int c = 0; c < DT; ++c) rl_stx4<GB>(p.X_out, (pt * 16 + li) * D + 16 * c + 4 * lj, xa[c]);
         f32x4 a[DT];
 #pragma unroll
         for (int nb = 0; nb < DT; ++nb) a[nb] = (f32x4){0.f, 0.f, 0.f, 0.f};
         tile_gemm_bf<DT>(xa, Wh, Wl, li, lj, a);
+        if constexpr (!XO) __builtin_amdgcn_sched_barrier(0);
         softmax_rows<DT>(a);
         __builtin_amdgcn_wave_barrier();
         f32x4 dx[DT];
@@ -2187,6 +2188,7 @@
     int terms;
     bool rows_bf16, gu_accumulate, fwd_stats2;
     long points;
+    bool skip_x;
 };
 
 typedef void (*PoolFn)();
@@ -2255,6 +2257,7 @@
     }
     const bool gb = f.rows_bf16 && !fwd && f.entry != PE_STATS;
     if (gb && f.terms != 3 && d != 128) { pl.refusal = "bf16 gradient rows need the bf16x3 arithmetic mode"; return pl; }
+    if (f.skip_x && gb) { pl.refusal = "bf16 gradient rows need X_out (the in-place X of the weight gradient is fp32 only)"; return pl; }
     switch (f.entry) {
     case PE_FWD:
         pl.name = virt ? "vpool_fwd_kernel" : d == 16 ? "pool_fwd_kernel<1>" : d == 32 ? "pool_fwd_kernel<2>" : d == 64 ? "pool_fwd_kernel<4>" : "pool_fwd_kernel<8>";
@@ -2264,7 +2267,8 @@
     case PE_BWD:
         pl.name = virt ? "vpool_bwd_kernel" : d == 16 ? "pool_bwd_kernel<1>" : d == 32 ? "pool_bwd_kernel<2>" : d == 64 ? "pool_bwd_kernel<4>" : "pool128_bwd_kernel";
         pl.fn = virt ? by_width<VPoolBwd>(d, f.terms, s2, gb, f.gu_accumulate)
-              : d == 128 ? (gb ? (PoolFn)pool128_bwd_kernel<true> : (PoolFn)pool128_bwd_kernel<false>) : by_width<PoolBwd>(d, f.terms, gb);
+              : d == 128 ? (gb ? (PoolFn)pool128_bwd_kernel<true> : f.skip_x ? (PoolFn)pool128_bwd_kernel<false, false> : (PoolFn)pool128_bwd_kernel<false>)
+              : by_width<PoolBwd>(d, f.terms, gb);
         pl.dw_count = d == 128 ? 0 : d * d;
         break;
     case PE_STATS:
@@ -2390,10 +2394,11 @@
     PoolParams p;
     int rc = fill(&p, d, "rl_pool_bwd", true);
     if (rc) return rc;
-    const PoolPlan pl = plan_pool({PE_BWD, p.d, p.src, rl_wide_terms(), d->rows_bf16 != 0, p.gu_accumulate != 0, false, p.P});
+    const bool skip_x = p.d == 128 && d->x_optional != 0 && d->X_out == nullptr;
+    const PoolPlan pl = plan_pool({PE_BWD, p.d, p.src, rl_wide_terms(), d->rows_bf16 != 0, p.gu_accumulate != 0, false, p.P, skip_x});
     RL_REQUIRE(!pl.refusal, RL_ERR_UNSUPPORTED, "rl_pool_bwd: %s (d %d, u_source %d)", pl.refusal, p.d, p.src);
     if (p.d == 128) {
-        RL_REQUIRE(d->X_out && d->dS_out, RL_ERR_ARGS, "rl_pool_bwd: d = 128 needs X_out and dS_out");
+        RL_REQUIRE((d->X_out || skip_x) && d->dS_out, RL_ERR_ARGS, "rl_pool_bwd: d = 128 needs X_out and dS_out");
         RL_REQUIRE((((uintptr_t)d->X_out | (uintptr_t)d->dS_out) & 15) == 0, RL_ERR_ARGS, "rl_pool_bwd: X_out / dS_out must be 16-byte aligned");
         p.X_out = d->X_out; p.dS_out = d->dS_out;
         return launch_pool(pl, "rl_pool_bwd", stream, nullptr, nullptr, p);
@@ -2402,6 +2407,15 @@
     RL_REQUIRE(d->slab_floats >= (int64_t)pl.grid * p.slab_stride, RL_ERR_ARGS, "rl_pool_bwd: slab too small");
     return launch_pool(pl, "rl_pool_bwd", stream, p.slab, d->dW, p);
 }
+
+static int g_pool128_x_in_place = 1;
+extern "C" int rl_set_pool128_x(const char* mode) {
+    const bool in_place = mode && !strcmp(mode, "in_place"), stored = mode && !strcmp(mode, "stored");
+    RL_REQUIRE(in_place || stored, RL_ERR_ARGS, "rl_set_pool128_x: mode must be \"in_place\" or \"stored\"");
+    g_pool128_x_in_place = in_place ? 1 : 0;
+    return RL_OK;
+}
+extern "C" const char* rl_get_pool128_x(void) { return g_pool128_x_in_place ? "in_place" : "stored"; }
 
 extern "C" int rl_rpe_stats(const rl_pool_desc* d, double* stats, void* stream) {
     PoolParams p;
diff --git a/3d_recognizer_amd/csrc/rl_common.h b/3d_recognizer_amd/csrc/rl_common.h
--- a/3d_recognizer_amd/csrc/rl_common.h
+++ b/3d_recognizer_amd/csrc/rl_common.h
@@ -104,6 +104,17 @@
     return rl_act(raw * t.scale[c] + t.shift[c], t.act, t.slope);
 }
 
+typedef float rl_f32x4 __attribute__((ext_vector_type(4)));
+__device__ __forceinline__ float rl_eff_slope(const RlLazy& t) {
+    if (t.scale == nullptr || t.act == RL_ACT_NONE) return 1.f;
+    return t.act == RL_ACT_RELU ? 0.f : t.slope;
+}
+__device__ __forceinline__ rl_f32x4 rl_fold_act4(const rl_f32x4 raw, const rl_f32x4 scale, const rl_f32x4 shift, const float e) {
+    const rl_f32x4 z = raw * scale + shift;
+    const rl_f32x4 ev = {e, e, e, e};
+    return __builtin_elementwise_max(z, z * ev);
+}
+
 typedef __bf16 rl_bf16x4 __attribute__((ext_vector_type(4)));
 template <bool BF>
 __device__ __forceinline__ float rl_ldx(const float* p, long i) {
diff --git a/3d_recognizer_amd/randlanet/_hip.py b/3d_recognizer_amd/randlanet/_hip.py
--- a/3d_recognizer_amd/randlanet/_hip.py
+++ b/3d_recognizer_amd/randlanet/_hip.py
@@ -62,6 +62,8 @@
         ("dbias", C.c_void_p),
         ("slab", C.c_void_p), ("slab_floats", C.c_int64),
         ("defer_reduce", C.c_int32), ("rows_bf16", C.c_int32),
+        ("a2_split", C.c_int32), ("a2_act", C.c_int32), ("A2", C.c_void_p), ("lda2", C.c_int64), ("a2_bstride", C.c_int64),
+        ("a2_idx", C.c_void_p), ("a2_scale", C.c_void_p), ("a2_shift", C.c_void_p), ("a2_slope", C.c_float),
     ]
 
 
@@ -134,6 +136,7 @@
         ("xyz_width", C.c_int32), ("bn_bwd_stats", C.c_void_p), ("bn_fwd_stats2", C.c_void_p),
         ("rows_bf16", C.c_int32),
         ("pivot_mean1", C.c_void_p), ("pivot_mean2", C.c_void_p),
+        ("x_optional", C.c_int32),
     ]
 
 
@@ -225,6 +228,7 @@
     "rl_set_gemm_ksplit": (_i, [_i]),
     "rl_set_sgemm_grid_div": (_i, [_i]),
     "rl_wgrad": (_i, [C.POINTER(WgradDesc), _vp]),
+    "rl_wgrad_plan": (_i, [C.POINTER(WgradDesc), C.POINTER(C.c_int32), C.POINTER(C.c_int32), C.POINTER(C.c_char_p)]),
     "rl_wgrad_nsplit": (_i, [_l, _i, _i]),
     "rl_wgrad_batchable": (_i, [C.POINTER(WgradDesc)]),
     "rl_wgrad_batch": (_i, [C.POINTER(WgradDesc), _i, _vp]),
@@ -267,6 +271,8 @@
     "rl_rpe_wgrad_slab_floats": (_l, [_l, _i, _i]),
     "rl_rpe_wgrad": (_i, [C.POINTER(PoolDesc), _vp, _vp, _vp, _l, _vp, _vp]),
     "rl_pool_bwd": (_i, [C.POINTER(PoolDesc), _vp]),
+    "rl_set_pool128_x": (_i, [C.c_char_p]),
+    "rl_get_pool128_x": (C.c_char_p, []),
     "rl_attpool_fwd": (_i, [_vp, _vp, _l, _i, _i, _vp, _vp]),
     "rl_attpool_bwd": (_i, [_vp, _vp, _vp, _vp, _l, _i, _i, _vp, _vp, _vp]),
     "rl_add_act_fwd": (_i, [_vp, _vp, _vp, _vp, _vp, _vp, _l, _i, _f, _vp, _vp]),
diff --git a/3d_recognizer_amd/randlanet/_ops.py b/3d_recognizer_amd/randlanet/_ops.py
--- a/3d_recognizer_amd/randlanet/_ops.py
+++ b/3d_recognizer_amd/randlanet/_ops.py
@@ -250,7 +250,51 @@
     return Lazy(out, a.B, a.n * a.K, a.n * a.K, 10)
 
 
+@dataclass
+class ConcatGather:
+    u: Lazy
+    g: Lazy
+    idx: torch.Tensor
+
+    @property
+    def B(self) -> int:
+        return self.u.B
+
+    @property
+    def n(self) -> int:
+        return self.u.n
+
+    @property
+    def C(self) -> int:
+        return self.u.C + self.g.C
+
+    @property
+    def rows(self) -> int:
+        return self.u.rows
+
+
+def set_pool128_x(mode: str) -> None:
+    H.check(H.lib().rl_set_pool128_x(mode.encode()), "rl_set_pool128_x")
+
+
+def get_pool128_x() -> str:
+    return H.lib().rl_get_pool128_x().decode()
+
+
 def _fill_a(d, a):
+    if isinstance(a, ConcatGather):
+        u, g, idx = a.u, a.g, a.idx
+        _dev_check(g.raw, g.scale, g.shift, idx)
+        assert idx.dtype == torch.int32 and idx.numel() == u.rows and u.bstride == u.n and g.B == u.B
+        assert g.raw.dtype == F32 and g.raw.dim() == 2 and g.raw.shape[1] >= g.C
+        assert g.raw.shape[0] >= (g.B - 1) * g.bstride + g.n, "second source rows out of range"
+        M, _ = _fill_a(d, u)
+        d.K = u.C + g.C
+        d.a2_split, d.A2, d.lda2, d.a2_bstride, d.a2_idx = u.C, g.raw.data_ptr(), g.raw.shape[1], g.bstride, idx.data_ptr()
+        if g.scale is not None:
+            assert g.scale.numel() == g.C and g.shift.numel() == g.C
+            d.a2_scale, d.a2_shift, d.a2_act, d.a2_slope = g.scale.data_ptr(), g.shift.data_ptr(), g.act, g.slope
+        return M, u.C + g.C
     if isinstance(a, Rpe):
         _dev_check(a.xyz, a.idx, a.d2)
         assert a.idx.dtype == torch.int32 and a.idx.shape == (a.B, a.n, a.K) and a.d2.shape == a.idx.shape
@@ -431,7 +475,8 @@
     _dev_check(dY, dW, dbias)
     rows_bf16 = dY.dtype == BF16
     assert dY.dtype in (F32, BF16) and dY.dim() == 2 and dY.shape[1] >= N
-    assert isinstance(a, Rpe) or a.raw.dtype == dY.dtype, "A and dY must share their storage type"
+    adt = F32 if isinstance(a, Rpe) else a.u.raw.dtype if isinstance(a, ConcatGather) else a.raw.dtype
+    assert isinstance(a, Rpe) or adt == dY.dtype, "A and dY must share their storage type"
     d.rows_bf16 = int(rows_bf16)
     assert dY.shape[0] >= (d.B - 1) * dy_bstride + rows_per_batch
     assert dW.numel() == K * N and (dbias is None or dbias.numel() == N)
@@ -443,6 +488,8 @@
     d.defer_reduce = 0 if pending is None else 1
     es = 2 if rows_bf16 else 4
     nbytes, flops = es * (M * (K if not isinstance(a, Rpe) else 6) + M * N) + 4 * K * N, 2 * M * K * N
+    if isinstance(a, ConcatGather):
+        nbytes = 4 * (M * a.u.C + a.g.rows * a.g.C + M) + 4 * M * N + 4 * K * N
     kind = H.lib().rl_wgrad_batchable(C.byref(d)) if (batch is not None and pending is not None) else 0
     if kind:
         batch.append((d, nbytes, flops, a, dY, slab, kind))
@@ -456,6 +503,19 @@
         it.slab, it.dW, it.dbias, it.w_ks, it.w_ns = slab.data_ptr(), dW.data_ptr(), H.ptr(dbias), w_ks, w_ns
         it.nsplit, it.N, it.K = H.lib().rl_wgrad_nsplit(M, N, K), N, K
         pending.append((it, slab, dW, dbias))
+
+
+def wgrad_supported(a, dY: torch.Tensor, dy_bstride: int, N: int) -> bool:
+    d = H.WgradDesc()
+    _fill_a(d, a)
+    d.rows_bf16 = int(dY.dtype == BF16)
+    d.N, d.dY, d.lddy, d.dy_bstride = N, dY.data_ptr(), dY.shape[1], dy_bstride
+    d.dW = d.slab = dY.data_ptr()
+    d.slab_floats, d.defer_reduce = 1 << 62, 1
+    rc = H.lib().rl_wgrad_plan(C.byref(d), None, None, None)
+    if rc not in (0, H.ERR_UNSUPPORTED):
+        H.check(rc, "rl_wgrad_plan")
+    return rc == 0
 
 
 def wgrad_batch_flush(batch: list) -> None:
@@ -964,12 +1024,19 @@
     else:
         nbytes = (4 * (2 * P * 16 * h + P * 16 + 2 * P * d) + es * P * 16 * h + 4 * P * 16 * h * (1 + int(gu_accumulate)))
     if d == 128:
-        X = torch.empty((P * 16, d), dtype=rdt, device=W.device)
         dS = torch.empty((P * 16, d), dtype=rdt, device=W.device)
-        pd.X_out, pd.dS_out = X.data_ptr(), dS.data_ptr()
-        with _rec("pool_bwd", (P, 16, d), nbytes + 2 * es * P * 16 * d, 4 * P * 16 * d * d):
+        xop = ConcatGather(u, g, idx) if (rdt == F32 and not virt and get_pool128_x() == "in_place") else None
+        if xop is not None and not wgrad_supported(xop, dS, n * 16, d):
+            xop = None
+        if xop is None:
+            X = torch.empty((P * 16, d), dtype=rdt, device=W.device)
+            pd.X_out, xop = X.data_ptr(), plain(X, u.B, n * 16)
+        else:
+            pd.x_optional = 1
+        pd.dS_out = dS.data_ptr()
+        with _rec("pool_bwd", (P, 16, d), nbytes + (1 + int(pd.x_optional == 0)) * es * P * 16 * d, 4 * P * 16 * d * d):
             H.check(H.lib().rl_pool_bwd(C.byref(pd), _st()), "rl_pool_bwd")
-        wgrad(plain(X, u.B, n * 16), dS, n * 16, d, dW, 1, d, None, pending=pending, batch=batch)
+        wgrad(xop, dS, n * 16, d, dW, 1, d, None, pending=pending, batch=batch)
         return DG
     floats = H.lib().rl_pool_slab_floats(P, d)
     if pending is not None:
diff --git a/include/rl_randlanet.h b/include/rl_randlanet.h
--- a/include/rl_randlanet.h
+++ b/include/rl_randlanet.h
@@ -140,10 +140,19 @@
     int64_t slab_floats;
     int32_t defer_reduce;
     int32_t rows_bf16;
+    int32_t a2_split;
+    int32_t a2_act;
+    const float* A2;
+    int64_t lda2, a2_bstride;
+    const int32_t* a2_idx;
+    const float* a2_scale;
+    const float* a2_shift;
+    float a2_slope;
 } rl_wgrad_desc;
 
 int64_t rl_wgrad_slab_floats(int64_t M, int N, int K);
 int rl_wgrad(const rl_wgrad_desc* d, void* stream);
+int rl_wgrad_plan(const rl_wgrad_desc* d, int32_t* grid_xyz, int32_t* threads, const char** kernel);
 
 typedef struct rl_wgrad_reduce_item {
     const float* slab;
@@ -339,6 +348,7 @@
     int32_t rows_bf16;
     const float* pivot_mean1;
     const float* pivot_mean2;
+    int32_t x_optional;
 } rl_pool_desc;
 
 int rl_pool_supported(int d, int nbr_k);
@@ -348,6 +358,8 @@
 int rl_pool_fwd_slots(int64_t points, int d);
 int rl_pool_fwd(const rl_pool_desc* d, void* stream);
 int rl_pool_bwd(const rl_pool_desc* d, void* stream);
+int rl_set_pool128_x(const char* mode);
+const char* rl_get_pool128_x(void);
 
 int rl_rpe_stats_slots(int64_t points);
 int rl_rpe_stats(const rl_pool_desc* d, double* stats, void* stream);
```

Result: faster. 1277, median of 6 (+1.7%).
